# PKU-EPIC/HOTrack

Measured on AMD Instinct MI355X. Metric: HandTrackNet point-cloud frames/sec (N=1024), higher is better.
Workload: dtype f32; 1 GPU; HandTrackNet forward, batch=64 synthetic 1024-pt clouds per GPU (BASELINE configs[1]); per_gpu_batch=64, global_batch=64, npoints=1024, parallelism=dp1 (independent batches, no collective), world_size=1, resident_batches_rotated=5, dead_attention_elided=True, fused_sa_kernels=True, launch=hipGraph replay, batches_in_flight=4, hip_hw_queues=4, sa_compute_units=256, weights=deterministic random init (no checkpoint available offline)

## Files before the change

hotrack_amd/csrc/capi.hip:

```cpp
#include <stdlib.h>

#include "pn2_common.h"
#include "../../include/pn2_ext.h"

namespace pn2 {
static thread_local int g_last_hip_error = 0;
void set_last_hip_error(int e) { g_last_hip_error = e; }

int fps_dispatch(int b, int n, int m, const float *xyz, float *temp, int *idx, hipStream_t st, int force_threads,
                 const int *skip_flags, int nflags, float *radii);
int fps_tie_check(int b, int n, int m, int m1, const float *xyz, const int *idx, const float *radii, int *flags, hipStream_t st);
bool fps_knn_supported(int n, int nq, int k);
bool ball_tie_supported(long b, long n, long m, long m2);
int ball_tie_dispatch(int b, int n, int m, float radius, int nsample, const float *xyz, int *idx, const int *picks, float *new_xyz_out,
                      float *new_xyz_copy, int copy_ld, int m2, const float *radii, int *flags, hipStream_t st, int *counts);
bool three_nn_interp_supported(long b, long n, long m, long c, long ldp, long ldo);
int three_nn_interp_dispatch(int b, int n, int m, int c, const float *unknown, const float *known, const float *points, int ldp,
                             float *out, int ldo, hipStream_t st);
bool three_nn_interp_rows_supported(long b, long n, long m, long c, long ldp, long ldo);
int three_nn_interp_rows_dispatch(int b, int n, int m, int c, const float *unknown, const float *known, const float *points, int ldp,
                                  float *out, int ldo, const int *row_list, const int *row_counts, hipStream_t st);
int fps_knn_dispatch(int b, int n, int m, const float *xyz, int *idx, float *radii, int nq, int k, int k2, const float *query,
                     int *kidx, int *kidx2, hipStream_t st);
int ball_query_dispatch(int b, int n, int m, float radius, int nsample, const float *new_xyz, const float *xyz,
                        int *idx, hipStream_t st, const int *picks, float *new_xyz_out, float *new_xyz_copy, int copy_ld, int *counts);
int three_nn_dispatch(int b, int n, int m, const float *unknown, const float *known, float *dist2, int *idx,
                      hipStream_t st, bool weights);
int interp_pm_dispatch(int b, int c, int m, int n, const float *points, int ldp, const int *idx, const float *weight,
                       float *out, int ldo, hipStream_t st);
int knn_dispatch(int b, int n, int m, int k, const float *unknown, const float *known, float *dist2, int *idx,
                 hipStream_t st, int k2, int *idx2);
int group_fwd_dispatch(int b, int c, int n, int npoints, int nsample, const float *points, const int *idx,
                       float *out, hipStream_t st);
int group_bwd_dispatch(int b, int c, int n, int npoints, int nsample, const float *grad_out, const int *idx,
                       float *grad_points, hipStream_t st);
int interp_fwd_dispatch(int b, int c, int m, int n, const float *points, const int *idx, const float *weight,
                        float *out, hipStream_t st);
int interp_bwd_dispatch(int b, int c, int n, int m, const float *grad_out, const int *idx, const float *weight,
                        float *grad_points, hipStream_t st);
}

using namespace pn2;

#define PN2_REQ(cond, code) \
    do {                    \
        if (!(cond)) return (code); \
    } while (0)

static inline bool fits_int(long v) { return v >= 0 && v <= 2147483647L; }

extern "C" {

int pn2_abi_version(void) { return 4; }

int pn2_last_hip_error(void) { return g_last_hip_error; }

const char *pn2_strerror(int code) {
    switch (code) {
        case PN2_OK: return "ok";
        case PN2_EINVAL: return "invalid dimension or parameter";
        case PN2_ENULL: return "required pointer is NULL";
        case PN2_ERANGE: return "size outside the supported range";
        case PN2_ESCRATCH: return "this size needs the scratch buffer (temp) to be provided";
        case PN2_ELAUNCH: return "HIP kernel launch failed";
        default: return "unknown error";
    }
}

int pn2_furthest_point_sampling(int b, int n, int m, const float *xyz, float *temp, int *idx, void *stream) {
    PN2_REQ(b >= 0 && n >= 1 && m >= 0, PN2_EINVAL);
    if (b == 0 || m == 0) return PN2_OK;
    PN2_REQ(xyz && idx, PN2_ENULL);
    PN2_REQ(b <= 65535 * 32768L, PN2_ERANGE);
    PN2_REQ(fits_int((long)n * 3), PN2_ERANGE);
    int force = 0;
    if (const char *e = getenv("PN2_FPS_THREADS")) force = atoi(e);
    return fps_dispatch(b, n, m, xyz, temp, idx, (hipStream_t)stream, force, nullptr, 0, nullptr);
}

int pn2x_furthest_point_sampling_radii(int b, int n, int m, const float *xyz, int *idx, float *radii, void *stream) {
    PN2_REQ(b >= 0 && n >= 1 && m >= 0, PN2_EINVAL);
    if (b == 0 || m == 0) return PN2_OK;
    PN2_REQ(xyz && idx && radii, PN2_ENULL);
    PN2_REQ(fits_int((long)n * 3), PN2_ERANGE);
    return fps_dispatch(b, n, m, xyz, nullptr, idx, (hipStream_t)stream, 0, nullptr, 0, radii);
}

int pn2x_fps_radii_knn_supported(int n, int nq, int k) { return fps_knn_supported(n, nq, k) ? 1 : 0; }

int pn2x_fps_radii_knn(int b, int n, int m, const float *xyz, int *idx, float *radii, int nq, int k, int k2, const float *query,
                       int *knn_idx, int *knn_idx2, void *stream) {
    PN2_REQ(b >= 0 && n >= 1 && m >= 1 && nq >= 1 && k >= 1 && k2 >= 0 && k2 <= k, PN2_EINVAL);
    if (b == 0) return PN2_OK;
    PN2_REQ(xyz && idx && radii && query && knn_idx && (k2 == 0 || knn_idx2), PN2_ENULL);
    PN2_REQ(m <= n && fits_int((long)n * 3) && fits_int((long)b * nq * k), PN2_ERANGE);
    return fps_knn_dispatch(b, n, m, xyz, idx, radii, nq, k, k2, query, knn_idx, k2 ? knn_idx2 : nullptr, (hipStream_t)stream);
}

int pn2x_fps_prefix_ties(int b, int n, int m1, int m2, const float *xyz, const int *idx1, const float *radii, int *flags, void *stream) {
    PN2_REQ(b >= 0 && n >= 1 && m1 >= 1 && m2 >= 1 && m2 <= m1, PN2_EINVAL);
    if (b == 0) return PN2_OK;
    PN2_REQ(xyz && idx1 && radii && flags, PN2_ENULL);
    PN2_REQ(fits_int((long)n * 3) && b <= 65535, PN2_ERANGE);
    return fps_tie_check(b, n, m2, m1, xyz, idx1, radii, flags, (hipStream_t)stream);
}

int pn2x_fps_prefix_flags(int n) { return n < 1 ? PN2_EINVAL : (n + 63) / 64; }

int pn2x_furthest_point_sampling_prefix(int b, int n, int m, const float *xyz, const int *flags, int nflags, int *idx, void *stream) {
    PN2_REQ(b >= 0 && n >= 1 && m >= 0 && m <= n && nflags >= 1, PN2_EINVAL);
    if (b == 0 || m == 0) return PN2_OK;
    PN2_REQ(xyz && idx && flags, PN2_ENULL);
    PN2_REQ(fits_int((long)n * 3), PN2_ERANGE);
    return fps_dispatch(b, n, m, xyz, nullptr, idx, (hipStream_t)stream, 0, flags, nflags, nullptr);
}

int pn2_ball_query(int b, int n, int m, float radius, int nsample, const float *new_xyz, const float *xyz,
                   int *idx, void *stream) {
    PN2_REQ(b >= 0 && n >= 1 && m >= 0 && nsample >= 1, PN2_EINVAL);
    PN2_REQ(radius == radius, PN2_EINVAL);
    if (b == 0 || m == 0) return PN2_OK;
    PN2_REQ(new_xyz && xyz && idx, PN2_ENULL);
    PN2_REQ(b <= 65535, PN2_ERANGE);
    PN2_REQ(fits_int((long)n * 3) && fits_int((long)m * nsample), PN2_ERANGE);
    if (n >= 4096 && (long)m * n >= (1L << 22) && radius > 0.f) {
        const long words = pn2x_ball_query_grid_scratch_words(b, n);
        if (words > 0 && words < (1L << 30)) {
            StreamScratch own;
            int *scratch = own.acquire((size_t)words + 4, (hipStream_t)stream);
            if (scratch) {
                unsigned *aligned = reinterpret_cast<unsigned *>(((uintptr_t)scratch + 15) & ~(uintptr_t)15);
                const int rc = ball_query_grid_dispatch(b, n, m, radius, nsample, new_xyz, xyz, idx, aligned, (size_t)words, (hipStream_t)stream);
                if (rc != PN2_ERANGE) return rc;
            }
        }
    }
    return ball_query_dispatch(b, n, m, radius, nsample, new_xyz, xyz, idx, (hipStream_t)stream, nullptr, nullptr, nullptr, 0, nullptr);
}

int pn2x_ball_query_picks(int b, int n, int m, float radius, int nsample, const float *xyz, const int *picks, float *new_xyz,
                           int *idx, float *new_xyz_copy, int copy_ld, void *stream) {
    return pn2x_ball_query_picks_counts(b, n, m, radius, nsample, xyz, picks, new_xyz, idx, new_xyz_copy, copy_ld, nullptr, stream);
}

int pn2x_ball_query_picks_counts(int b, int n, int m, float radius, int nsample, const float *xyz, const int *picks, float *new_xyz,
                                  int *idx, float *new_xyz_copy, int copy_ld, int *counts, void *stream) {
    PN2_REQ(!new_xyz_copy || copy_ld >= 3, PN2_EINVAL);
    PN2_REQ(b >= 0 && n >= 1 && m >= 0 && nsample >= 1, PN2_EINVAL);
    PN2_REQ(radius == radius, PN2_EINVAL);
    if (b == 0 || m == 0) return PN2_OK;
    PN2_REQ(xyz && picks && new_xyz && idx, PN2_ENULL);
    PN2_REQ(b <= 65535, PN2_ERANGE);
    PN2_REQ(fits_int((long)n * 3) && fits_int((long)m * nsample), PN2_ERANGE);
    return ball_query_dispatch(b, n, m, radius, nsample, nullptr, xyz, idx, (hipStream_t)stream, picks, new_xyz, new_xyz_copy, copy_ld, counts);
}

int pn2x_ball_query_picks_ties_supported(int b, int n, int m, int m2) { return ball_tie_supported(b, n, m, m2) ? 1 : 0; }

int pn2x_ball_query_picks_ties(int b, int n, int m, float radius, int nsample, const float *xyz, const int *picks, float *new_xyz,
                               int *idx, float *new_xyz_copy, int copy_ld, int m2, const float *radii, int *flags, void *stream) {
    return pn2x_ball_query_picks_ties_counts(b, n, m, radius, nsample, xyz, picks, new_xyz, idx, new_xyz_copy, copy_ld, m2, radii, flags,
                                             nullptr, stream);
}

int pn2x_ball_query_picks_ties_counts(int b, int n, int m, float radius, int nsample, const float *xyz, const int *picks, float *new_xyz,
                                      int *idx, float *new_xyz_copy, int copy_ld, int m2, const float *radii, int *flags, int *counts,
                                      void *stream) {
    PN2_REQ(!new_xyz_copy || copy_ld >= 3, PN2_EINVAL);
    PN2_REQ(b >= 0 && n >= 1 && m >= 1 && nsample >= 1 && m2 >= 1 && m2 <= m, PN2_EINVAL);
    PN2_REQ(radius == radius, PN2_EINVAL);
    if (b == 0) return PN2_OK;
    PN2_REQ(xyz && picks && new_xyz && idx && radii && flags, PN2_ENULL);
    PN2_REQ(b <= 65535 && fits_int((long)n * 3) && fits_int((long)m * nsample), PN2_ERANGE);
    return ball_tie_dispatch(b, n, m, radius, nsample, xyz, idx, picks, new_xyz, new_xyz_copy, copy_ld, m2, radii, flags, (hipStream_t)stream, counts);
}

int pn2_group_points(int b, int c, int n, int npoints, int nsample, const float *points, const int *idx,
                     float *out, void *stream) {
    PN2_REQ(b >= 0 && c >= 0 && n >= 1 && npoints >= 0 && nsample >= 0, PN2_EINVAL);
    if (b == 0 || c == 0 || npoints == 0 || nsample == 0) return PN2_OK;
    PN2_REQ(points && idx && out, PN2_ENULL);
    PN2_REQ(b <= 65535 && fits_int((long)npoints * nsample), PN2_ERANGE);
    return group_fwd_dispatch(b, c, n, npoints, nsample, points, idx, out, (hipStream_t)stream);
}

int pn2_group_points_grad(int b, int c, int n, int npoints, int nsample, const float *grad_out, const int *idx,
                          float *grad_points, void *stream) {
    PN2_REQ(b >= 0 && c >= 0 && n >= 1 && npoints >= 0 && nsample >= 0, PN2_EINVAL);
    if (b == 0 || c == 0 || npoints == 0 || nsample == 0) return PN2_OK;
    PN2_REQ(grad_out && idx && grad_points, PN2_ENULL);
    PN2_REQ(b <= 65535 && c <= 65535 * 16 && fits_int((long)npoints * nsample), PN2_ERANGE);
    return group_bwd_dispatch(b, c, n, npoints, nsample, grad_out, idx, grad_points, (hipStream_t)stream);
}

int pn2_gather_points(int b, int c, int n, int npoints, const float *points, const int *idx, float *out,
                      void *stream) {
    return pn2_group_points(b, c, n, npoints, 1, points, idx, out, stream);
}

int pn2_gather_points_grad(int b, int c, int n, int npoints, const float *grad_out, const int *idx,
                           float *grad_points, void *stream) {
    return pn2_group_points_grad(b, c, n, npoints, 1, grad_out, idx, grad_points, stream);
}

int pn2_knn(int b, int n, int m, int k, const float *unknown, const float *known, float *dist2, int *idx,
            void *stream) {
    PN2_REQ(b >= 0 && n >= 0 && m >= 0, PN2_EINVAL);
    PN2_REQ(k >= 1, PN2_EINVAL);
    PN2_REQ(k <= PN2_KNN_MAX_K, PN2_ERANGE);
    if (b == 0 || n == 0) return PN2_OK;
    PN2_REQ(unknown && dist2 && idx && (known || m == 0), PN2_ENULL);
    PN2_REQ(b <= 65535 && fits_int((long)n * k) && fits_int((long)m * 3), PN2_ERANGE);
    return knn_dispatch(b, n, m, k, unknown, known, dist2, idx, (hipStream_t)stream, 0, nullptr);
}

int pn2x_knn_indices(int b, int n, int m, int k, int k2, const float *unknown, const float *known, int *idx, int *idx2, void *stream) {
    PN2_REQ(b >= 0 && n >= 0 && m >= 1 && k >= 1 && k2 >= 0 && k2 <= k, PN2_EINVAL);
    PN2_REQ(k <= PN2_KNN_MAX_K, PN2_ERANGE);
    if (b == 0 || n == 0) return PN2_OK;
    PN2_REQ(unknown && known && idx && (idx2 || k2 == 0), PN2_ENULL);
    PN2_REQ(b <= 65535 && fits_int((long)n * k) && fits_int((long)m * 3), PN2_ERANGE);
    return knn_dispatch(b, n, m, k, unknown, known, nullptr, idx, (hipStream_t)stream, k2, k2 > 0 ? idx2 : nullptr);
}

int pn2_three_nn(int b, int n, int m, const float *unknown, const float *known, float *dist2, int *idx,
                 void *stream) {
    PN2_REQ(b >= 0 && n >= 0 && m >= 0, PN2_EINVAL);
    if (b == 0 || n == 0) return PN2_OK;
    PN2_REQ(unknown && dist2 && idx && (known || m == 0), PN2_ENULL);
    PN2_REQ(b <= 65535 && fits_int((long)n * 3) && fits_int((long)m * 3), PN2_ERANGE);
    return three_nn_dispatch(b, n, m, unknown, known, dist2, idx, (hipStream_t)stream, false);
}

int pn2_three_interpolate(int b, int c, int m, int n, const float *points, const int *idx, const float *weight,
                          float *out, void *stream) {
    PN2_REQ(b >= 0 && c >= 0 && m >= 1 && n >= 0, PN2_EINVAL);
    if (b == 0 || c == 0 || n == 0) return PN2_OK;
    PN2_REQ(points && idx && weight && out, PN2_ENULL);
    PN2_REQ(b <= 65535 && fits_int((long)n * 3), PN2_ERANGE);
    return interp_fwd_dispatch(b, c, m, n, points, idx, weight, out, (hipStream_t)stream);
}

int pn2_three_interpolate_grad(int b, int c, int n, int m, const float *grad_out, const int *idx,
                               const float *weight, float *grad_points, void *stream) {
    PN2_REQ(b >= 0 && c >= 0 && m >= 1 && n >= 0, PN2_EINVAL);
    if (b == 0 || c == 0 || n == 0) return PN2_OK;
    PN2_REQ(grad_out && idx && weight && grad_points, PN2_ENULL);
    PN2_REQ(b <= 65535 && c <= 65535 * 16 && fits_int((long)n * 3), PN2_ERANGE);
    return interp_bwd_dispatch(b, c, n, m, grad_out, idx, weight, grad_points, (hipStream_t)stream);
}

int pn2x_three_nn_weights(int b, int n, int m, const float *unknown, const float *known, float *weight, int *idx,
                          void *stream) {
    PN2_REQ(b >= 0 && n >= 0 && m >= 3, PN2_EINVAL);
    if (b == 0 || n == 0) return PN2_OK;
    PN2_REQ(unknown && known && weight && idx, PN2_ENULL);
    PN2_REQ(b <= 65535 && fits_int((long)n * 3) && fits_int((long)m * 3), PN2_ERANGE);
    return three_nn_dispatch(b, n, m, unknown, known, weight, idx, (hipStream_t)stream, true);
}

int pn2x_three_nn_interpolate_pm_supported(int b, int n, int m, int c, int ldp, int ldo) {
    return three_nn_interp_supported(b, n, m, c, ldp, ldo) ? 1 : 0;
}

int pn2x_three_nn_interpolate_pm(int b, int n, int m, int c, const float *unknown, const float *known, const float *points, int ldp,
                                 float *out, int ldo, void *stream) {
    PN2_REQ(b >= 0 && n >= 0 && m >= 3 && c >= 1 && ldp >= c && ldo >= c, PN2_EINVAL);
    if (b == 0 || n == 0) return PN2_OK;
    PN2_REQ(unknown && known && points && out, PN2_ENULL);
    PN2_REQ(b <= 65535 && fits_int((long)n * 3) && fits_int((long)m * 3), PN2_ERANGE);
    return three_nn_interp_dispatch(b, n, m, c, unknown, known, points, ldp, out, ldo, (hipStream_t)stream);
}

int pn2x_three_nn_interpolate_pm_rows_supported(int b, int n, int m, int c, int ldp, int ldo) {
    return three_nn_interp_rows_supported(b, n, m, c, ldp, ldo) ? 1 : 0;
}

int pn2x_three_nn_interpolate_pm_rows(int b, int n, int m, int c, const float *unknown, const float *known, const float *points,
                                      int ldp, float *out, int ldo, const int *row_list, const int *row_counts, void *stream) {
    PN2_REQ(b >= 0 && n >= 0 && m >= 3 && c >= 1 && ldp >= c && ldo >= c, PN2_EINVAL);
    if (b == 0 || n == 0) return PN2_OK;
    PN2_REQ(unknown && known && points && out && row_list && row_counts, PN2_ENULL);
    PN2_REQ(b <= 65535 && fits_int((long)n * 3) && fits_int((long)m * 3), PN2_ERANGE);
    return three_nn_interp_rows_dispatch(b, n, m, c, unknown, known, points, ldp, out, ldo, row_list, row_counts, (hipStream_t)stream);
}

int pn2x_three_interpolate_pm(int b, int c, int m, int n, const float *points, int ldp, const int *idx,
                              const float *weight, float *out, int ldo, void *stream) {
    PN2_REQ(b >= 0 && c >= 0 && m >= 1 && n >= 0 && ldp >= c && ldo >= c, PN2_EINVAL);
    if (b == 0 || c == 0 || n == 0) return PN2_OK;
    PN2_REQ(points && idx && weight && out, PN2_ENULL);
    PN2_REQ(fits_int((long)n * 3), PN2_ERANGE);
    return interp_pm_dispatch(b, c, m, n, points, ldp, idx, weight, out, ldo, (hipStream_t)stream);
}

}
```

hotrack_amd/csrc/nn_search.hip:

```cpp
#include "pn2_common.h"
#include "knn_wave.h"

namespace pn2 {

constexpr int kNnTile = 2048;

template <int THREADS, bool WEIGHTS>
__global__ void __launch_bounds__(THREADS)
three_nn_kernel(int n, int m, const float *__restrict__ unknown_all, const float *__restrict__ known_all,
                float *__restrict__ dist2_all, int *__restrict__ idx_all) {
    extern __shared__ __attribute__((aligned(16))) float4 sk[];
    const int b = blockIdx.y;
    const float *__restrict__ known = known_all + (size_t)b * m * 3;
    const int q = blockIdx.x * THREADS + threadIdx.x;
    const bool active = q < n;
    const float *__restrict__ u = unknown_all + ((size_t)b * n + (active ? q : 0)) * 3;
    const float ux = u[0], uy = u[1], uz = u[2];

    float b1 = __builtin_inff(), b2 = __builtin_inff(), b3 = __builtin_inff();
    int i1 = 0, i2 = 0, i3 = 0;

    for (int t0 = 0; t0 < m; t0 += kNnTile) {
        const int tn = (m - t0) < kNnTile ? (m - t0) : kNnTile;
        if (t0 > 0) __syncthreads();
        for (int p = threadIdx.x; p < tn; p += THREADS) {
            const float *src = known + (size_t)3 * (t0 + p);
            sk[p] = make_float4(src[0], src[1], src[2], 0.f);
        }
        __syncthreads();
#pragma unroll 4
        for (int p = 0; p < tn; ++p) {
            const float4 kp = sk[p];
            const float d = sqdist(ux, uy, uz, kp.x, kp.y, kp.z);
            const int k = t0 + p;
            const bool lt1 = d < b1, lt2 = d < b2, lt3 = d < b3;
            b3 = lt2 ? b2 : (lt3 ? d : b3);
            i3 = lt2 ? i2 : (lt3 ? k : i3);
            b2 = lt1 ? b1 : (lt2 ? d : b2);
            i2 = lt1 ? i1 : (lt2 ? k : i2);
            b1 = lt1 ? d : b1;
            i1 = lt1 ? k : i1;
        }
    }
    if (active) {
        float *od = dist2_all + ((size_t)b * n + q) * 3;
        int *oi = idx_all + ((size_t)b * n + q) * 3;
        if constexpr (WEIGHTS) {
            const float r1 = 1.0f / (__builtin_sqrtf(b1) + 1e-8f), r2 = 1.0f / (__builtin_sqrtf(b2) + 1e-8f),
                        r3 = 1.0f / (__builtin_sqrtf(b3) + 1e-8f);
            const float norm = (r1 + r2) + r3;
            od[0] = r1 / norm; od[1] = r2 / norm; od[2] = r3 / norm;
        } else {
            od[0] = b1; od[1] = b2; od[2] = b3;
        }
        oi[0] = i1; oi[1] = i2; oi[2] = i3;
    }
}

template <bool WEIGHTS>
__global__ void __launch_bounds__(256)
three_nn_split_kernel(int n, int m, const float *__restrict__ unknown_all, const float *__restrict__ known_all,
                      float *__restrict__ dist2_all, int *__restrict__ idx_all) {
    extern __shared__ __attribute__((aligned(16))) float4 sk[];
    __shared__ float sd[3][3][64];
    __shared__ int si[3][3][64];
    const int b = blockIdx.y;
    const float *__restrict__ known = known_all + (size_t)b * m * 3;
    const int ql = threadIdx.x & 63, c = threadIdx.x >> 6;
    const int q = blockIdx.x * 64 + ql;
    const bool active = q < n;
    const float *__restrict__ u = unknown_all + ((size_t)b * n + (active ? q : 0)) * 3;
    const float ux = u[0], uy = u[1], uz = u[2];
    for (int p = threadIdx.x; p < m; p += 256) {
        const float *src = known + (size_t)3 * p;
        sk[p] = make_float4(src[0], src[1], src[2], 0.f);
    }
    __syncthreads();
    float b1 = __builtin_inff(), b2 = __builtin_inff(), b3 = __builtin_inff();
    int i1 = 0, i2 = 0, i3 = 0;
    auto insert = [&](float d, int k) {
        const bool lt1 = d < b1, lt2 = d < b2, lt3 = d < b3;
        b3 = lt2 ? b2 : (lt3 ? d : b3);
        i3 = lt2 ? i2 : (lt3 ? k : i3);
        b2 = lt1 ? b1 : (lt2 ? d : b2);
        i2 = lt1 ? i1 : (lt2 ? k : i2);
        b1 = lt1 ? d : b1;
        i1 = lt1 ? k : i1;
    };
    const int len = (m + 3) / 4, p0 = c * len, p1 = min(m, p0 + len);
#pragma unroll 4
    for (int p = p0; p < p1; ++p) {
        const float4 kp = sk[p];
        insert(sqdist(ux, uy, uz, kp.x, kp.y, kp.z), p);
    }
    if (c > 0) {
        sd[c - 1][0][ql] = b1; sd[c - 1][1][ql] = b2; sd[c - 1][2][ql] = b3;
        si[c - 1][0][ql] = i1; si[c - 1][1][ql] = i2; si[c - 1][2][ql] = i3;
    }
    __syncthreads();
    if (c != 0 || !active) return;
#pragma unroll
    for (int cc = 0; cc < 3; ++cc)
#pragma unroll
        for (int e = 0; e < 3; ++e) insert(sd[cc][e][ql], si[cc][e][ql]);
    float *od = dist2_all + ((size_t)b * n + q) * 3;
    int *oi = idx_all + ((size_t)b * n + q) * 3;
    if constexpr (WEIGHTS) {
        const float r1 = 1.0f / (__builtin_sqrtf(b1) + 1e-8f), r2 = 1.0f / (__builtin_sqrtf(b2) + 1e-8f),
                    r3 = 1.0f / (__builtin_sqrtf(b3) + 1e-8f);
        const float norm = (r1 + r2) + r3;
        od[0] = r1 / norm; od[1] = r2 / norm; od[2] = r3 / norm;
    } else {
        od[0] = b1; od[1] = b2; od[2] = b3;
    }
    oi[0] = i1; oi[1] = i2; oi[2] = i3;
}

template <bool ROWS>
__global__ void __launch_bounds__(256)
three_nn_interp_kernel(int n, int m, int c4, const float *__restrict__ unknown_all, const float *__restrict__ known_all,
                       const float *__restrict__ points_all, int ldp, float *__restrict__ out_all, int ldo,
                       const int *__restrict__ row_list, const int *__restrict__ row_counts) {
    extern __shared__ __attribute__((aligned(16))) float4 sk[];
    __shared__ float sd[3][3][64];
    __shared__ int si[3][3][64];
    __shared__ float fw[3][64];
    __shared__ int fi[3][64];
    __shared__ int fq[ROWS ? 64 : 1];
    const int b = blockIdx.y;
    const float *__restrict__ known = known_all + (size_t)b * m * 3;
    const int ql = threadIdx.x & 63, c = threadIdx.x >> 6;
    int q = blockIdx.x * 64 + ql, nq = n;
    if constexpr (ROWS) {
        nq = row_counts[2 * b + 1];
        nq = nq < 0 ? 0 : (nq > n ? n : nq);
        if ((int)blockIdx.x * 64 >= nq) return;
        q = q < nq ? row_list[(size_t)b * n + q] : -1;
        if ((unsigned)q >= (unsigned)n) q = -1;
    }
    const bool active = ROWS ? q >= 0 : q < n;
    const float *__restrict__ u = unknown_all + ((size_t)b * n + (active ? q : 0)) * 3;
    const float ux = u[0], uy = u[1], uz = u[2];
    for (int p = threadIdx.x; p < m; p += 256) {
        const float *src = known + (size_t)3 * p;
        sk[p] = make_float4(src[0], src[1], src[2], 0.f);
    }
    __syncthreads();
    float b1 = __builtin_inff(), b2 = __builtin_inff(), b3 = __builtin_inff();
    int i1 = 0, i2 = 0, i3 = 0;
    auto insert = [&](float d, int k) {
        const bool lt1 = d < b1, lt2 = d < b2, lt3 = d < b3;
        b3 = lt2 ? b2 : (lt3 ? d : b3);
        i3 = lt2 ? i2 : (lt3 ? k : i3);
        b2 = lt1 ? b1 : (lt2 ? d : b2);
        i2 = lt1 ? i1 : (lt2 ? k : i2);
        b1 = lt1 ? d : b1;
        i1 = lt1 ? k : i1;
    };
    const int len = (m + 3) / 4, p0 = c * len, p1 = min(m, p0 + len);
#pragma unroll 4
    for (int p = p0; p < p1; ++p) {
        const float4 kp = sk[p];
        insert(sqdist(ux, uy, uz, kp.x, kp.y, kp.z), p);
    }
    if (c > 0) {
        sd[c - 1][0][ql] = b1; sd[c - 1][1][ql] = b2; sd[c - 1][2][ql] = b3;
        si[c - 1][0][ql] = i1; si[c - 1][1][ql] = i2; si[c - 1][2][ql] = i3;
    }
    __syncthreads();
    if (c == 0) {
#pragma unroll
        for (int cc = 0; cc < 3; ++cc)
#pragma unroll
            for (int e = 0; e < 3; ++e) insert(sd[cc][e][ql], si[cc][e][ql]);
        const float r1 = 1.0f / (__builtin_sqrtf(b1) + 1e-8f), r2 = 1.0f / (__builtin_sqrtf(b2) + 1e-8f),
                    r3 = 1.0f / (__builtin_sqrtf(b3) + 1e-8f);
        const float norm = (r1 + r2) + r3;
        fw[0][ql] = r1 / norm; fw[1][ql] = r2 / norm; fw[2][ql] = r3 / norm;
        fi[0][ql] = i1; fi[1][ql] = i2; fi[2][ql] = i3;
        if constexpr (ROWS) fq[ql] = q;
    }
    __syncthreads();
    const int rows = min(64, nq - (int)blockIdx.x * 64);
    const float *__restrict__ src = points_all + (size_t)b * m * ldp;
    float *__restrict__ dst = out_all + ((size_t)b * n + (ROWS ? (size_t)0 : (size_t)blockIdx.x * 64)) * ldo;
    for (int e = threadIdx.x; e < rows * c4; e += 256) {
        const int r = e / c4, col = e - r * c4;
        const float w0 = fw[0][r], w1 = fw[1][r], w2 = fw[2][r];
        const float4 a0 = *reinterpret_cast<const float4 *>(src + (size_t)fi[0][r] * ldp + 4 * col);
        const float4 a1 = *reinterpret_cast<const float4 *>(src + (size_t)fi[1][r] * ldp + 4 * col);
        const float4 a2 = *reinterpret_cast<const float4 *>(src + (size_t)fi[2][r] * ldp + 4 * col);
        float4 o;
        o.x = __builtin_fmaf(w2, a2.x, __builtin_fmaf(w0, a0.x, w1 * a1.x));
        o.y = __builtin_fmaf(w2, a2.y, __builtin_fmaf(w0, a0.y, w1 * a1.y));
        o.z = __builtin_fmaf(w2, a2.z, __builtin_fmaf(w0, a0.z, w1 * a1.z));
        o.w = __builtin_fmaf(w2, a2.w, __builtin_fmaf(w0, a0.w, w1 * a1.w));
        if constexpr (ROWS) {
            if (fq[r] >= 0) *reinterpret_cast<float4 *>(dst + (size_t)fq[r] * ldo + 4 * col) = o;
        } else {
            *reinterpret_cast<float4 *>(dst + (size_t)r * ldo + 4 * col) = o;
        }
    }
}

bool three_nn_interp_supported(long b, long n, long m, long c, long ldp, long ldo) {
    return b * n >= 16384 && b * n < 256L * 1024 && m >= 16 && m <= kNnTile && c >= 4 && c % 4 == 0 && ldp % 4 == 0 && ldo % 4 == 0;
}

int three_nn_interp_dispatch(int b, int n, int m, int c, const float *unknown, const float *known, const float *points, int ldp,
                             float *out, int ldo, hipStream_t st) {
    if (b == 0 || n == 0) return PN2_OK;
    if (!three_nn_interp_supported(b, n, m, c, ldp, ldo) || (((uintptr_t)points | (uintptr_t)out) % 16) != 0) return PN2_ERANGE;
    dim3 grid((n + 63) / 64, b);
    hipLaunchKernelGGL(three_nn_interp_kernel<false>, grid, dim3(256), (size_t)m * sizeof(float4), st, n, m, c / 4, unknown, known, points,
                       ldp, out, ldo, nullptr, nullptr);
    return check_launch();
}

bool three_nn_interp_rows_supported(long b, long n, long m, long c, long ldp, long ldo) {
    return b <= 65535 && m >= 3 && m <= kNnTile && c >= 4 && c % 4 == 0 && ldp % 4 == 0 && ldo % 4 == 0;
}

int three_nn_interp_rows_dispatch(int b, int n, int m, int c, const float *unknown, const float *known, const float *points, int ldp,
                                  float *out, int ldo, const int *row_list, const int *row_counts, hipStream_t st) {
    if (b == 0 || n == 0) return PN2_OK;
    if (!three_nn_interp_rows_supported(b, n, m, c, ldp, ldo) || (((uintptr_t)points | (uintptr_t)out) % 16) != 0) return PN2_ERANGE;
    dim3 grid((n + 63) / 64, b);
    hipLaunchKernelGGL(three_nn_interp_kernel<true>, grid, dim3(256), (size_t)m * sizeof(float4), st, n, m, c / 4, unknown, known, points,
                       ldp, out, ldo, row_list, row_counts);
    return check_launch();
}

int three_nn_dispatch(int b, int n, int m, const float *unknown, const float *known, float *dist2,
                      int *idx, hipStream_t st, bool weights) {
    if (b == 0 || n == 0) return PN2_OK;
    if ((long)b * n < 256L * 1024 && m >= 16 && m <= kNnTile) {
        dim3 grid((n + 63) / 64, b);
        const size_t lds_split = (size_t)m * sizeof(float4);
        if (weights) hipLaunchKernelGGL((three_nn_split_kernel<true>), grid, dim3(256), lds_split, st, n, m, unknown, known, dist2, idx);
        else hipLaunchKernelGGL((three_nn_split_kernel<false>), grid, dim3(256), lds_split, st, n, m, unknown, known, dist2, idx);
        return check_launch();
    }
    const int tile_cap = m < kNnTile ? m : kNnTile;
    const size_t lds = (size_t)(tile_cap > 0 ? tile_cap : 1) * sizeof(float4);
    if ((long)b * n < 256L * 1024) {
        dim3 grid((n + 63) / 64, b);
        if (weights) hipLaunchKernelGGL((three_nn_kernel<64, true>), grid, dim3(64), lds, st, n, m, unknown, known, dist2, idx);
        else hipLaunchKernelGGL((three_nn_kernel<64, false>), grid, dim3(64), lds, st, n, m, unknown, known, dist2, idx);
    } else {
        dim3 grid((n + 255) / 256, b);
        if (weights) hipLaunchKernelGGL((three_nn_kernel<256, true>), grid, dim3(256), lds, st, n, m, unknown, known, dist2, idx);
        else hipLaunchKernelGGL((three_nn_kernel<256, false>), grid, dim3(256), lds, st, n, m, unknown, known, dist2, idx);
    }
    return check_launch();
}

template <int P>
__global__ void __launch_bounds__(256)
knn_wave_kernel(int n, int m, int k, const float *__restrict__ unknown_all, const float *__restrict__ known_all,
                float *__restrict__ dist2_all, int *__restrict__ idx_all, int k2, int *__restrict__ idx2_all) {
    const int q = blockIdx.x * 4 + (threadIdx.x >> 6);
    if (q >= n) return;
    knn_wave_body<P>(blockIdx.y, q, n, m, k, unknown_all, known_all, dist2_all, idx_all, k2, idx2_all);
}

template <int NS>
__global__ void __launch_bounds__(256)
knn_stream_kernel(int n, int m, int k, const float *__restrict__ unknown_all, const float *__restrict__ known_all,
                  float *__restrict__ dist2_all, int *__restrict__ idx_all, int k2, int *__restrict__ idx2_all) {
    __shared__ unsigned long long lists[4][64 * NS];
    const int b = blockIdx.y;
    const int lane = threadIdx.x & 63, wv = threadIdx.x >> 6;
    const int q = blockIdx.x * 4 + wv;
    if (q >= n) return;
    volatile unsigned long long *L = lists[wv];
    const float *__restrict__ known = known_all + (size_t)b * m * 3;
    const float *__restrict__ u = unknown_all + ((size_t)b * n + q) * 3;
    const float ux = u[0], uy = u[1], uz = u[2];
#pragma unroll
    for (int s = 0; s < NS; ++s) L[lane + 64 * s] = kInfKey;
    unsigned long long kth = kInfKey;
    for (int base = 0; base < m; base += 64) {
        const int c = base + lane;
        const bool in = c < m;
        const float *src = known + (size_t)3 * (in ? c : 0);
        const float d = sqdist(ux, uy, uz, src[0], src[1], src[2]);
        const unsigned long long key = (in && d < __builtin_inff()) ? (((unsigned long long)(unsigned)f2i(d) << 32) | (unsigned)c) : kInfKey;
        uint64_t pass = __ballot(key < kth);
        while (pass) {
            const int l = __builtin_ctzll(pass);
            pass &= pass - 1;
            const unsigned long long kb = ((unsigned long long)(unsigned)__builtin_amdgcn_readlane((int)(unsigned)(key >> 32), l) << 32) |
                                          (unsigned)__builtin_amdgcn_readlane((int)(unsigned)key, l);
            if (!(kb < kth)) continue;
            unsigned long long cur[NS], prev[NS];
#pragma unroll
            for (int s = 0; s < NS; ++s) {
                const int e = lane + 64 * s;
                cur[s] = L[e];
                prev[s] = e > 0 ? L[e - 1] : 0ull;
            }
#pragma unroll
            for (int s = 0; s < NS; ++s) L[lane + 64 * s] = cur[s] < kb ? cur[s] : (prev[s] < kb ? kb : prev[s]);
            kth = L[k - 1];
            kth = ((unsigned long long)(unsigned)__builtin_amdgcn_readfirstlane((int)(unsigned)(kth >> 32)) << 32) |
                  (unsigned)__builtin_amdgcn_readfirstlane((int)(unsigned)kth);
        }
    }
    float *__restrict__ od = dist2_all ? dist2_all + ((size_t)b * n + q) * k : nullptr;
    int *__restrict__ oi = idx_all + ((size_t)b * n + q) * k;
    int *__restrict__ oi2 = idx2_all ? idx2_all + ((size_t)b * n + q) * k2 : nullptr;
#pragma unroll
    for (int s = 0; s < NS; ++s) {
        const int e = lane + 64 * s;
        if (e < k) {
            const unsigned long long v = L[e];
            if (od) od[e] = i2f((int)(unsigned)(v >> 32));
            oi[e] = (int)(unsigned)v;
            if (oi2 && e < k2) oi2[e] = (int)(unsigned)v;
        }
    }
}

int knn_dispatch(int b, int n, int m, int k, const float *unknown, const float *known, float *dist2,
                 int *idx, hipStream_t st, int k2, int *idx2) {
    if (b == 0 || n == 0) return PN2_OK;
    dim3 grid((n + 3) / 4, b);
#define PN2_KNN_CASE(PP)                                                                                    \
    if (m <= 64 * PP) {                                                                                     \
        hipLaunchKernelGGL(knn_wave_kernel<PP>, grid, dim3(256), 0, st, n, m, k, unknown, known, dist2, idx, k2, idx2); \
        return check_launch();                                                                              \
    }
    PN2_KNN_CASE(1) PN2_KNN_CASE(2) PN2_KNN_CASE(4) PN2_KNN_CASE(8) PN2_KNN_CASE(16) PN2_KNN_CASE(32)
#undef PN2_KNN_CASE
    if (k <= 64) hipLaunchKernelGGL(knn_stream_kernel<1>, grid, dim3(256), 0, st, n, m, k, unknown, known, dist2, idx, k2, idx2);
    else if (k <= 128) hipLaunchKernelGGL(knn_stream_kernel<2>, grid, dim3(256), 0, st, n, m, k, unknown, known, dist2, idx, k2, idx2);
    else hipLaunchKernelGGL(knn_stream_kernel<4>, grid, dim3(256), 0, st, n, m, k, unknown, known, dist2, idx, k2, idx2);
    static_assert(PN2_KNN_MAX_K <= 256, "knn_stream_kernel<4> holds 256 list entries");
    return check_launch();
}

}
```

hotrack_amd/csrc/row_chain.hip:

```cpp
#include "pn2_common.h"
#include "mfma_rows.h"
#include "../../include/pn2_ext.h"

namespace pn2 {
namespace rchain {

using mrows::f32x4;
using mrows::init_bias;
using mrows::mm;
using mrows::relu_to_lds;

constexpr int CH = 128, CC = 384, CQ = 512;
constexpr int KX = 144;
constexpr int XQ = 33;
constexpr int LDX = 152, LDH = 136, LDC = 392;
constexpr int MAXB = 1024;
constexpr int GROUP_COST_SMALL = 31, GROUP_COST_LARGE = 20;

struct ChainArgs {
    int B, N, ldx, ldo;
    const float *x;
    const int *list, *counts;
    const float *wa, *ba, *wb, *bb, *wc, *bc, *wq;
    float *out;
};

struct Smem {
    int *rows;
    int *p_small;
    int *p_large;
    float *r1;
    float *r2;
};

constexpr size_t lds_bytes(int clouds) {
    return (size_t)64 * (LDX + LDC) * sizeof(float) + (size_t)(64 + 2 * (clouds + 1) + 512) * sizeof(int);
}

__device__ __forceinline__ int lookup(const ChainArgs &A, const Smem &S, int seq, int e) {
    const int *P = seq ? S.p_large : S.p_small;
    int lo = 0, hi = A.B;
    while (hi - lo > 1) {
        const int mid = (lo + hi) >> 1;
        if (P[mid] <= e) lo = mid; else hi = mid;
    }
    const int off = seq ? (S.p_small[lo + 1] - S.p_small[lo]) : 0;
    return lo * A.N + A.list[(size_t)lo * A.N + off + (e - P[lo])];
}

template <int MT>
__device__ void tile(const ChainArgs &A, const Smem &S, int seq, int e0, int cnt) {
    const int tid = (int)threadIdx.x, lane = tid & 63, w = tid >> 6;
    constexpr int R = MT * 16;
    if (tid < R) S.rows[tid] = tid < cnt ? lookup(A, S, seq, e0 + tid) : -1;
    __syncthreads();
    for (int i = tid; i < R * (KX / 4); i += 256) {
        const int r = i / (KX / 4), q = i - r * (KX / 4);
        const int g = S.rows[r];
        f32x4 v = {0.f, 0.f, 0.f, 0.f};
        if (g >= 0 && q < XQ) {
            v = *reinterpret_cast<const f32x4 *>(A.x + (size_t)g * A.ldx + 4 * q);
            if (q == XQ - 1) v.w = 0.f;
        }
        *reinterpret_cast<f32x4 *>(S.r1 + r * LDX + 4 * q) = v;
    }
    __syncthreads();
    {
        f32x4 acc[2][MT];
        init_bias(acc, A.ba, 2 * w, lane);
        mm<2, MT, KX / 16, LDX>(acc, A.wa + (size_t)(2 * w) * (KX / 16) * 256, S.r1, lane);
        relu_to_lds(acc, S.r2, LDH, 2 * w, lane);
    }
    __syncthreads();
    {
        f32x4 acc[2][MT];
        init_bias(acc, A.bb, 2 * w, lane);
        mm<2, MT, CH / 16, LDH>(acc, A.wb + (size_t)(2 * w) * (CH / 16) * 256, S.r2, lane);
        relu_to_lds(acc, S.r1, LDH, 2 * w, lane);
    }
    __syncthreads();
#pragma unroll 1
    for (int p = 0; p < 2; ++p) {
        const int nt0 = (p * 4 + w) * 3;
        f32x4 acc[3][MT];
        init_bias(acc, A.bc, nt0, lane);
        mm<3, MT, CH / 16, LDH>(acc, A.wc + (size_t)nt0 * (CH / 16) * 256, S.r1, lane);
        relu_to_lds(acc, S.r2, LDC, nt0, lane);
    }
    __syncthreads();
    const int np = seq ? 1 : 2;
#pragma unroll 1
    for (int p = 0; p < np; ++p) {
        const int nt0 = (seq ? 16 : 0) + (p * 4 + w) * 4;
        f32x4 acc[4][MT];
#pragma unroll
        for (int nt = 0; nt < 4; ++nt)
#pragma unroll
            for (int mt = 0; mt < MT; ++mt) acc[nt][mt] = (f32x4){0.f, 0.f, 0.f, 0.f};
        mm<4, MT, CC / 16, LDC>(acc, A.wq + (size_t)nt0 * (CC / 16) * 256, S.r2, lane);
#pragma unroll
        for (int mt = 0; mt < MT; ++mt) {
            const int g = S.rows[mt * 16 + (lane & 15)];
            if (g < 0) continue;
            float *o = A.out + (size_t)g * A.ldo + nt0 * 16 + 4 * (lane >> 4);
#pragma unroll
            for (int nt = 0; nt < 4; ++nt) *reinterpret_cast<f32x4 *>(o + nt * 16) = acc[nt][mt];
        }
    }
    __syncthreads();
}

__device__ void run_rows(const ChainArgs &A, const Smem &S, int seq, int e_lo, int e_hi) {
    for (int e0 = e_lo; e0 < e_hi; e0 += 64) {
        const int cnt = e_hi - e0 < 64 ? e_hi - e0 : 64;
        switch ((cnt + 15) >> 4) {
            case 1: tile<1>(A, S, seq, e0, cnt); break;
            case 2: tile<2>(A, S, seq, e0, cnt); break;
            case 3: tile<3>(A, S, seq, e0, cnt); break;
            default: tile<4>(A, S, seq, e0, cnt); break;
        }
    }
}

__global__ __launch_bounds__(256, 1) void row_chain_kernel(ChainArgs A) {
    extern __shared__ __attribute__((aligned(16))) float smem[];
    const int tid = (int)threadIdx.x;
    Smem S;
    S.r1 = smem;
    S.r2 = smem + 64 * LDX;
    S.rows = reinterpret_cast<int *>(S.r2 + 64 * LDC);
    S.p_small = S.rows + 64;
    S.p_large = S.p_small + (A.B + 1);
    int *scan = S.p_large + (A.B + 1);
    int carry_s = 0, carry_l = 0;
    if (tid == 0) { S.p_small[0] = 0; S.p_large[0] = 0; }
    for (int base = 0; base < A.B; base += 256) {
        const int b = base + tid;
        int cs = 0, cl = 0;
        if (b < A.B) {
            cs = A.counts[2 * b];
            cl = A.counts[2 * b + 1] - cs;
        }
        for (int d = 1; d < 256; d <<= 1) {
            scan[tid] = cs; scan[256 + tid] = cl;
            __syncthreads();
            if (tid >= d) { cs += scan[tid - d]; cl += scan[256 + tid - d]; }
            __syncthreads();
        }
        if (b < A.B) { S.p_small[b + 1] = carry_s + cs; S.p_large[b + 1] = carry_l + cl; }
        scan[tid] = cs; scan[256 + tid] = cl;
        __syncthreads();
        carry_s += scan[255]; carry_l += scan[511];
        __syncthreads();
    }
    const int n_small = carry_s, n_large = carry_l;
    const long g_small = (n_small + 15) / 16, g_large = (n_large + 15) / 16;
    const long total = GROUP_COST_SMALL * g_small + GROUP_COST_LARGE * g_large;
    const long lo = total * blockIdx.x / gridDim.x, hi = total * (blockIdx.x + 1) / gridDim.x;
    auto first_at = [](long c, long cost) { return c <= 0 ? 0L : (c + cost - 1) / cost; };
    long s0 = first_at(lo, GROUP_COST_SMALL), s1 = first_at(hi, GROUP_COST_SMALL);
    s0 = s0 < g_small ? s0 : g_small; s1 = s1 < g_small ? s1 : g_small;
    const long cs_end = GROUP_COST_SMALL * g_small;
    long l0 = first_at(lo - cs_end, GROUP_COST_LARGE), l1 = first_at(hi - cs_end, GROUP_COST_LARGE);
    l0 = l0 < g_large ? l0 : g_large; l1 = l1 < g_large ? l1 : g_large;
    auto clip = [](long e, int n) { return (int)(e < n ? e : n); };
    run_rows(A, S, 0, clip(16 * s0, n_small), clip(16 * s1, n_small));
    run_rows(A, S, 1, clip(16 * l0, n_large), clip(16 * l1, n_large));
}

constexpr int RL_MAXN = 16384;

__global__ __launch_bounds__(256) void row_lists_kernel(int N, int J, int KL, int KS, const int *__restrict__ gi,
                                                        const int *__restrict__ gis, int *__restrict__ list, int *__restrict__ counts) {
    __shared__ unsigned small[RL_MAXN / 32], any[RL_MAXN / 32];
    __shared__ int scan[2][256];
    const int tid = (int)threadIdx.x, b = (int)blockIdx.x;
    const int NW = (N + 31) >> 5;
    for (int i = tid; i < NW; i += 256) { small[i] = 0u; any[i] = 0u; }
    __syncthreads();
    const int *gl = gi + (size_t)b * J * KL;
    for (int i = tid; i < J * KL; i += 256) {
        const int p = gl[i];
        if (gis == nullptr && (i % KL) < KS && (unsigned)p < (unsigned)N) atomicOr(&small[p >> 5], 1u << (p & 31));
        if ((unsigned)p < (unsigned)N) atomicOr(&any[p >> 5], 1u << (p & 31));
    }
    if (gis != nullptr) {
        const int *gs = gis + (size_t)b * J * KS;
        for (int i = tid; i < J * KS; i += 256) {
            const int p = gs[i];
            if ((unsigned)p < (unsigned)N) {
                atomicOr(&small[p >> 5], 1u << (p & 31));
                atomicOr(&any[p >> 5], 1u << (p & 31));
            }
        }
    }
    __syncthreads();
    const int WPT = (NW + 255) >> 8;
    const int w0 = tid * WPT, w1 = w0 + WPT < NW ? w0 + WPT : NW;
    int cs = 0, co = 0;
    for (int i = w0; i < w1; ++i) {
        cs += __builtin_popcount(small[i]);
        co += __builtin_popcount(any[i] & ~small[i]);
    }
    int is = cs, io = co;
    for (int d = 1; d < 256; d <<= 1) {
        scan[0][tid] = is; scan[1][tid] = io;
        __syncthreads();
        if (tid >= d) { is += scan[0][tid - d]; io += scan[1][tid - d]; }
        __syncthreads();
    }
    scan[0][tid] = is; scan[1][tid] = io;
    __syncthreads();
    const int tot_s = scan[0][255], tot_o = scan[1][255];
    int *dst = list + (size_t)b * N;
    int ps = is - cs, po = tot_s + io - co;
    for (int i = w0; i < w1; ++i) {
        unsigned ms = small[i], mo = any[i] & ~small[i];
        while (ms) { const int k = __builtin_ctz(ms); ms &= ms - 1; dst[ps++] = 32 * i + k; }
        while (mo) { const int k = __builtin_ctz(mo); mo &= mo - 1; dst[po++] = 32 * i + k; }
    }
    if (tid == 0) { counts[2 * b] = tot_s; counts[2 * b + 1] = tot_s + tot_o; }
}

}
}

extern "C" int pn2x_row_lists(int b, int n, int j, int k_large, int k_small, const int *gi, const int *gi_small, int *list,
                              int *counts, void *stream) {
    using namespace pn2;
    if (b < 0 || n < 1 || j < 1 || k_large < 1 || k_small < 1 || k_small > k_large) return PN2_EINVAL;
    if (n > rchain::RL_MAXN || (long)j * k_large > (1L << 24)) return PN2_ERANGE;
    if (b == 0) return PN2_OK;
    if (!gi || !list || !counts) return PN2_ENULL;
    hipLaunchKernelGGL(rchain::row_lists_kernel, dim3(b), dim3(256), 0, (hipStream_t)stream, n, j, k_large, k_small, gi, gi_small,
                       list, counts);
    return check_launch();
}

extern "C" int pn2x_row_chain_supported(int c_in, int c_h, int c_conv, int c_q) {
    return (c_in == 128 && c_h == 128 && c_conv == 384 && c_q == 512) ? 1 : 0;
}

extern "C" int pn2x_row_chain(int b, int n, const float *x, int ldx, const int *list, const int *counts, const float *wa,
                              const float *ba, const float *wb, const float *bb, const float *wc, const float *bc, const float *wq,
                              float *out, int ldo, int grid, void *stream) {
    using namespace pn2;
    using namespace pn2::rchain;
    if (b < 0 || n < 1 || ldx < 132 || ldo < CQ || ldx % 4 || ldo % 4 || grid < 0) return PN2_EINVAL;
    if (b > MAXB || (long)b * n >= (1L << 31) / 2) return PN2_ERANGE;
    if (b == 0) return PN2_OK;
    if (!x || !list || !counts || !wa || !ba || !wb || !bb || !wc || !bc || !wq || !out) return PN2_ENULL;
    if (((uintptr_t)x | (uintptr_t)out | (uintptr_t)wa | (uintptr_t)ba | (uintptr_t)wb | (uintptr_t)bb | (uintptr_t)wc |
         (uintptr_t)bc | (uintptr_t)wq) % 16 != 0)
        return PN2_EINVAL;
    ChainArgs a;
    a.B = b; a.N = n; a.ldx = ldx; a.ldo = ldo; a.x = x; a.list = list; a.counts = counts;
    a.wa = wa; a.ba = ba; a.wb = wb; a.bb = bb; a.wc = wc; a.bc = bc; a.wq = wq; a.out = out;
    const size_t lds = lds_bytes(b);
    static_assert(lds_bytes(MAXB) <= 160 * 1024, "row_chain's LDS at MAXB clouds exceeds a compute unit's 160 KB");
    static PerDeviceOnce raised;
    if (raised.first_use())
        (void)hipFuncSetAttribute((const void *)row_chain_kernel, hipFuncAttributeMaxDynamicSharedMemorySize, (int)lds_bytes(MAXB));
    const int cus = num_compute_units();
    if (grid == 0 || grid > cus) grid = cus;
    hipLaunchKernelGGL(row_chain_kernel, dim3(grid), dim3(256), lds, (hipStream_t)stream, a);
    return check_launch();
}
```

hotrack_amd/ext.py:

```python
from __future__ import annotations

import ctypes
import os

import torch

from . import pointnet2_hip as _native

_lib = _native._lib
_vp, _ci = ctypes.c_void_p, ctypes.c_int
_lib.pn2x_kabsch.argtypes = [_ci, _ci, _ci, _vp, _vp, _vp, _vp, _vp]
_lib.pn2x_kabsch.restype = _ci


def kabsch(x: torch.Tensor, y: torch.Tensor):
    x = x.float().contiguous()
    y = y.float().contiguous()
    if x.dim() == 2:
        x = x.unsqueeze(0)
    B, num, _ = y.shape
    xb = x.shape[0]
    if xb not in (1, B) or x.shape[1] != num:
        raise ValueError(f"kabsch: x {tuple(x.shape)} does not match y {tuple(y.shape)}")
    px = _native._ptr(x, "x", torch.float32, xb * num * 3)
    py = _native._ptr(y, "y", torch.float32, B * num * 3)
    R = torch.empty((B, 3, 3), dtype=torch.float32, device=y.device)
    t = torch.empty((B, 3, 1), dtype=torch.float32, device=y.device)
    with torch.cuda.device(y.device):
        _native._check(_lib.pn2x_kabsch(B, xb, num, px, py, R.data_ptr(), t.data_ptr(), _native._stream(y)), "kabsch")
    return R, t


_lib.pn2x_kabsch_backward.argtypes = [_ci, _ci, _ci, _vp, _vp, _vp, _vp, _vp, _vp, _vp]
_lib.pn2x_kabsch_backward.restype = _ci


def kabsch_backward(x: torch.Tensor, y: torch.Tensor, R: torch.Tensor, grad_R, grad_t) -> torch.Tensor:
    x = x.float().contiguous()
    y = y.float().contiguous()
    if x.dim() == 2:
        x = x.unsqueeze(0)
    B, num, _ = y.shape
    f32 = torch.float32
    gR = None if grad_R is None else _native._ptr(grad_R.contiguous(), "grad_R", f32, B * 9)
    gt = None if grad_t is None else _native._ptr(grad_t.contiguous(), "grad_t", f32, B * 3)
    dy = torch.empty_like(y)
    with torch.cuda.device(y.device):
        _native._check(_lib.pn2x_kabsch_backward(B, x.shape[0], num, _native._ptr(x, "x", f32, x.shape[0] * num * 3),
                                                 _native._ptr(y, "y", f32, B * num * 3), _native._ptr(R.contiguous(), "R", f32, B * 9),
                                                 gR, gt, dy.data_ptr(), _native._stream(y)), "kabsch_backward")
    return dy


class KabschFit(torch.autograd.Function):

    @staticmethod
    def forward(ctx, x, y):
        R, t = kabsch(x, y)
        ctx.save_for_backward(x, y, R)
        return R, t

    @staticmethod
    def backward(ctx, grad_R, grad_t):
        x, y, R = ctx.saved_tensors
        return None, kabsch_backward(x, y, R, grad_R, grad_t)


_cl = ctypes.c_long
_lib.pn2x_sa_mlp_max.argtypes = [_ci] * 7 + [_vp, _ci, _vp, _vp, _vp, _vp, _vp, _ci, _vp, _vp, _vp, _vp, _vp, _vp, _cl, _ci, _ci, _vp]
_lib.pn2x_sa_mlp_max.restype = _ci
_lib.pn2x_sa_mlp_max_supported.argtypes = [_ci] * 4
_lib.pn2x_sa_mlp_max_supported.restype = _ci
_lib.pn2x_three_nn_weights.argtypes = [_ci, _ci, _ci, _vp, _vp, _vp, _vp, _vp]
_lib.pn2x_three_nn_weights.restype = _ci
_lib.pn2x_three_interpolate_pm.argtypes = [_ci, _ci, _ci, _ci, _vp, _ci, _vp, _vp, _vp, _ci, _vp]
_lib.pn2x_three_interpolate_pm.restype = _ci
_lib.pn2x_gather_rows.argtypes = [_ci, _ci, _ci, _ci, _vp, _vp, _vp, _vp]
_lib.pn2x_gather_rows.restype = _ci
_lib.pn2x_bias_act_pm.argtypes = [_cl, _ci, _vp, _ci, _vp, _cl, _ci, _vp]
_lib.pn2x_bias_act_pm.restype = _ci


def sa_mlp_max_supported(k: int, c1: int, c2: int, c3: int) -> bool:
    return bool(_lib.pn2x_sa_mlp_max_supported(k, c1, c2, c3))


def _rows(t: torch.Tensor, name: str, cols: int):
    if not t.is_cuda or t.dtype != torch.float32 or t.dim() != 3:
        raise TypeError(f"{name}: expected a 3-D float32 GPU tensor")
    B, R, C = t.shape
    if C < cols or t.stride(2) != 1 or (R > 1 and B > 1 and t.stride(0) != R * t.stride(1)):
        raise ValueError(f"{name}: unsupported layout shape={tuple(t.shape)} strides={t.stride()}")
    return t.data_ptr(), t.stride(1)


def sa_mlp_max(idx: torch.Tensor, w2, b2, w3, b3, *, a1f=None, xyz=None, cxyz=None, wx=None, b1=None, cadd=None,
               out=None, point_major=False) -> torch.Tensor:
    return _sa_mlp_max(idx, w2, b2, w3, b3, None, a1f, xyz, cxyz, wx, b1, cadd, out, point_major)


_lib.pn2x_sa_mlp_max_classes.argtypes = [_ci] * 7 + [_vp, _ci, _vp, _vp, _vp, _vp, _vp, _ci, _vp, _vp, _vp, _vp, _vp, _vp, _vp, _vp, _cl, _ci, _ci, _vp]
_lib.pn2x_sa_mlp_max_classes.restype = _ci
_lib.pn2x_sa_mlp_max_classes_supported.argtypes = [_ci] * 4
_lib.pn2x_sa_mlp_max_classes_supported.restype = _ci
_lib.pn2x_sa_class_lists.argtypes = [_ci, _ci, _ci, _vp, _vp, _vp, _vp]
_lib.pn2x_sa_class_lists.restype = _ci
_lib.pn2x_sa_class_lists2.argtypes = [_ci, _ci, _ci, _vp, _vp, _vp] * 2 + [_vp]
_lib.pn2x_sa_class_lists2.restype = _ci


def sa_mlp_max_classes_supported(k: int, c1: int, c2: int, c3: int) -> bool:
    return bool(_lib.pn2x_sa_mlp_max_classes_supported(k, c1, c2, c3))


def sa_class_partition(counts: torch.Tensor):
    c = counts.reshape(-1)
    ids = torch.arange(c.numel(), dtype=torch.int32, device=c.device)
    masks = (c > 16, (c > 8) & (c <= 16), c <= 8)
    return torch.cat([ids[m] for m in masks]), torch.stack([m.sum() for m in masks]).to(torch.int32)


def _class_lists_args(counts, n, what):
    if not isinstance(counts, torch.Tensor) or counts.dim() != 2 or counts.dtype != torch.int32 or not counts.is_cuda:
        raise TypeError(f"{what}: counts must be a (B,S) int32 GPU tensor")
    if int(n) < 1:
        raise ValueError(f"{what}: n >= 1")
    B, S = counts.shape
    pc = _native._ptr(counts, "counts", torch.int32, B * S)
    lst = torch.empty((B * S, 4), dtype=torch.int32, device=counts.device)
    sizes = torch.empty(3, dtype=torch.int32, device=counts.device)
    return B, S, int(n), pc, lst, sizes


def sa_class_lists(counts: torch.Tensor, n: int):
    B, S, n, pc, lst, sizes = _class_lists_args(counts, n, "sa_class_lists")
    with torch.cuda.device(counts.device):
        _native._check(_native._call(_lib.pn2x_sa_class_lists, "sa_class_lists2_kernel", None, B, S, n, pc, lst.data_ptr(),
                                     sizes.data_ptr(), _native._stream(counts)), "sa_class_lists")
    return lst, sizes


def sa_class_lists_pair(counts_a: torch.Tensor, n_a: int, counts_b: torch.Tensor, n_b: int):
    a = _class_lists_args(counts_a, n_a, "sa_class_lists_pair")
    b = _class_lists_args(counts_b, n_b, "sa_class_lists_pair")
    if counts_a.device != counts_b.device:
        raise ValueError("sa_class_lists_pair: both problems on one device")
    with torch.cuda.device(counts_a.device):
        _native._check(_native._call(_lib.pn2x_sa_class_lists2, "sa_class_lists2_kernel", None, *a[:4], a[4].data_ptr(), a[5].data_ptr(),
                                     *b[:4], b[4].data_ptr(), b[5].data_ptr(), _native._stream(counts_a)), "sa_class_lists_pair")
    return (a[4], a[5]), (b[4], b[5])


def sa_mlp_max_classes(idx: torch.Tensor, classes, w2, b2, w3, b3, *, a1f=None, xyz=None, cxyz=None, wx=None, b1=None, cadd=None,
                       out=None, point_major=False) -> torch.Tensor:
    if not (isinstance(classes, (tuple, list)) and len(classes) == 2):
        raise TypeError("sa_mlp_max_classes: classes must be the (list, sizes) pair of sa_class_lists")
    return _sa_mlp_max(idx, w2, b2, w3, b3, classes, a1f, xyz, cxyz, wx, b1, cadd, out, point_major)


def _sa_mlp_max(idx, w2, b2, w3, b3, classes, a1f, xyz, cxyz, wx, b1, cadd, out, point_major, record=False):
    B, S, K = idx.shape
    C1, C2, C3 = w2.shape[1], w2.shape[0], w3.shape[0]
    f32 = torch.float32
    N = a1f.shape[1] if a1f is not None else xyz.shape[1]
    pa, lda = (None, 0) if a1f is None else _rows(a1f, "a1f", C1)
    pc, ldc = (None, 0) if cadd is None else _rows(cadd, "cadd", C1)
    px = None if xyz is None else _native._ptr(xyz, "xyz", f32, B * N * 3)
    pcx = None if cxyz is None else _native._ptr(cxyz, "cxyz", f32, B * S * 3)
    pwx = None if wx is None else _native._ptr(wx, "wx", f32, C1 * 3)
    pb1 = None if b1 is None else _native._ptr(b1, "b1", f32, C1)
    pi = _native._ptr(idx, "idx", torch.int32, B * S * K)
    pw2, pb2 = _native._ptr(w2, "w2", f32, C2 * C1), _native._ptr(b2, "b2", f32, C2)
    pw3, pb3 = _native._ptr(w3, "w3", f32, C3 * C2), _native._ptr(b3, "b3", f32, C3)
    if out is None:
        out = torch.empty((B, S, C3) if point_major else (B, C3, S), dtype=f32, device=idx.device)
        ob, os_, oc = (S * C3, C3, 1) if point_major else (C3 * S, 1, S)
        po = out.data_ptr()
    else:
        po, ld = _rows(out, "out", C3)
        ob, os_, oc = out.stride(0), ld, 1
    if record:
        return _SaProblem(N, S, K, pa, lda, px, pcx, pwx, pb1, pc, ldc, pi, pw2, pb2, pw3, pb3, po, ob, os_, oc)
    if classes is not None:
        lst, sizes = classes
        pl = _native._ptr(lst, "classes list", torch.int32, B * S * 4)
        ps = _native._ptr(sizes, "classes sizes", torch.int32, 3)
        if lst.device != idx.device or sizes.device != idx.device:
            raise ValueError("sa_mlp_max_classes: classes on another device than idx")
        with torch.cuda.device(idx.device):
            _native._check(_native._call(_lib.pn2x_sa_mlp_max_classes, "sa_mlp_max_classes_kernel", None, B, N, S, K, C1, C2, C3, pa, lda,
                                         px, pcx, pwx, pb1, pc, ldc, pi, pl, ps, pw2, pb2, pw3, pb3, po, ob, os_, oc,
                                         _native._stream(idx)), "sa_mlp_max_classes")
        return out
    with torch.cuda.device(idx.device):
        _native._check(_native._call(_lib.pn2x_sa_mlp_max, "sa_mlp_max_kernel", None, B, N, S, K, C1, C2, C3, pa, lda, px, pcx,
                                     pwx, pb1, pc, ldc, pi, pw2, pb2, pw3, pb3, po, ob, os_, oc, _native._stream(idx)),
                       "sa_mlp_max")
    return out


class _SaProblem(ctypes.Structure):
    _fields_ = [("n", _ci), ("s", _ci), ("k", _ci), ("a1f", _vp), ("a1f_ld", _ci), ("xyz", _vp), ("cxyz", _vp), ("wx", _vp),
                ("b1", _vp), ("cadd", _vp), ("cadd_ld", _ci), ("idx", _vp), ("w2", _vp), ("b2", _vp), ("w3", _vp), ("b3", _vp),
                ("out", _vp), ("out_b", _cl), ("out_s", _ci), ("out_c", _ci)]


_lib.pn2x_sa_mlp_max_pair.argtypes = [_ci] * 4 + [ctypes.POINTER(_SaProblem)] * 2 + [_vp]
_lib.pn2x_sa_mlp_max_pair.restype = _ci
_lib.pn2x_sa_mlp_max_pair_supported.argtypes = [_ci] * 5
_lib.pn2x_sa_mlp_max_pair_supported.restype = _ci


def sa_mlp_max_pair(p0: dict, p1: dict) -> None:
    keys = ("idx", "w2", "b2", "w3", "b3", "a1f", "xyz", "cxyz", "wx", "b1", "cadd", "out")
    a = [{k: p.get(k) for k in keys} for p in (p0, p1)]
    C1, C2, C3 = a[0]["w2"].shape[1], a[0]["w2"].shape[0], a[0]["w3"].shape[0]
    same = all(tuple(a[1][k].shape) == tuple(a[0][k].shape) for k in ("w2", "w3"))
    modes = [(p["a1f"] is not None, p["xyz"] is not None, p["cadd"] is not None) for p in a]
    if not (same and modes[0] == modes[1] and modes[0][0] and modes[0][1]
            and _lib.pn2x_sa_mlp_max_pair_supported(a[0]["idx"].shape[2], a[1]["idx"].shape[2], C1, C2, C3)):
        for p in a:
            sa_mlp_max(p["idx"], p["w2"], p["b2"], p["w3"], p["b3"], a1f=p["a1f"], xyz=p["xyz"], cxyz=p["cxyz"], wx=p["wx"], b1=p["b1"],
                       cadd=p["cadd"], out=p["out"])
        return
    B = a[0]["idx"].shape[0]
    if a[0]["out"] is None or a[1]["out"] is None:
        raise TypeError("sa_mlp_max_pair: out is required")
    q0, q1 = (_sa_mlp_max(classes=None, point_major=False, record=True, **p) for p in a)
    with torch.cuda.device(a[0]["idx"].device):
        _native._check(_native._call(_lib.pn2x_sa_mlp_max_pair, "sa_mlp_max_pair_kernel", None, B, C1, C2, C3, ctypes.byref(q0),
                                     ctypes.byref(q1), _native._stream(a[0]["idx"])), "sa_mlp_max_pair")


_lib.pn2x_mlp2_rows.argtypes = [_cl] + [_ci] * 3 + [_vp, _ci, _vp, _vp, _vp, _vp, _vp, _vp, _ci, _vp]
_lib.pn2x_mlp2_rows.restype = _ci
_lib.pn2x_mlp2_rows_supported.argtypes = [_ci] * 3
_lib.pn2x_mlp2_rows_supported.restype = _ci


_lib.pn2x_sa_set_compute_units.argtypes = [_ci]
_lib.pn2x_sa_set_compute_units.restype = _ci


def sa_set_compute_units(n: int) -> None:
    _native._check(_lib.pn2x_sa_set_compute_units(int(n)), "sa_set_compute_units")


def mlp2_rows_supported(c1: int, c2: int, c3: int) -> bool:
    return bool(_lib.pn2x_mlp2_rows_supported(c1, c2, c3))


def mlp2_rows(x: torch.Tensor, w2, b2, w3, b3, out: torch.Tensor = None, w2e=None) -> torch.Tensor:
    if x.dim() != 2 or not x.is_cuda or x.dtype != torch.float32 or x.stride(1) != 1:
        raise TypeError("mlp2_rows: x must be a 2-D float32 GPU tensor with a contiguous last dimension")
    R = x.shape[0]
    C1, C2, C3 = w2.shape[1], w2.shape[0], w3.shape[0]
    f32 = torch.float32
    ldx = x.stride(0) if R > 1 else x.shape[1]
    if x.shape[1] < C1 + (3 if w2e is not None else 0) or (w2e is not None and ldx < C1 + 4):
        raise ValueError("mlp2_rows: x has too few columns")
    if out is None:
        out = torch.empty((R, C3), dtype=f32, device=x.device)
    if out.dim() != 2 or out.shape[0] != R or out.shape[1] < C3 or out.stride(1) != 1 or out.dtype != f32 or out.device != x.device:
        raise ValueError("mlp2_rows: out must be (rows, >= c3) float32 on the same device")
    if (R > 1 and out.stride(0) % 4) or out.data_ptr() % 16:
        raise ValueError("mlp2_rows: out needs a row stride that is a multiple of 4 floats and a 16-byte aligned first element")
    with torch.cuda.device(x.device):
        _native._check(_native._call(_lib.pn2x_mlp2_rows, "mlp2_rows_kernel", None, R, C1, C2, C3, x.data_ptr(), ldx,
                                     _native._ptr(w2, "w2", f32, C2 * C1), None if w2e is None else _native._ptr(w2e, "w2e", f32, C2 * 3),
                                     _native._ptr(b2, "b2", f32, C2), _native._ptr(w3, "w3", f32, C3 * C2),
                                     _native._ptr(b3, "b3", f32, C3), out.data_ptr(), out.stride(0) if R > 1 else out.shape[1], _native._stream(x)),
                       "mlp2_rows")
    return out


def three_nn_weights(unknown: torch.Tensor, known: torch.Tensor):
    B, n, _ = unknown.shape
    m = known.shape[1]
    f32 = torch.float32
    w = torch.empty((B, n, 3), dtype=f32, device=unknown.device)
    idx = torch.empty((B, n, 3), dtype=torch.int32, device=unknown.device)
    with torch.cuda.device(unknown.device):
        _native._check(_lib.pn2x_three_nn_weights(B, n, m, _native._ptr(unknown, "unknown", f32, B * n * 3),
                                                  _native._ptr(known, "known", f32, B * m * 3), w.data_ptr(), idx.data_ptr(),
                                                  _native._stream(unknown)), "three_nn_weights")
    return w, idx


def three_interpolate_pm(points: torch.Tensor, idx: torch.Tensor, weight: torch.Tensor, out: torch.Tensor) -> torch.Tensor:
    B, M, C = points.shape
    n = idx.shape[1]
    pp, ldp = _rows(points, "points", C)
    po, ldo = _rows(out, "out", C)
    with torch.cuda.device(points.device):
        _native._check(_lib.pn2x_three_interpolate_pm(B, C, M, n, pp, ldp, _native._ptr(idx, "idx", torch.int32, B * n * 3),
                                                      _native._ptr(weight, "weight", torch.float32, B * n * 3), po, ldo,
                                                      _native._stream(points)), "three_interpolate_pm")
    return out


_lib.pn2x_three_nn_interpolate_pm.argtypes = [_ci, _ci, _ci, _ci, _vp, _vp, _vp, _ci, _vp, _ci, _vp]
_lib.pn2x_three_nn_interpolate_pm.restype = _ci
_lib.pn2x_three_nn_interpolate_pm_supported.argtypes = [_ci] * 6
_lib.pn2x_three_nn_interpolate_pm_supported.restype = _ci
_lib.pn2x_three_nn_interpolate_pm_rows.argtypes = [_ci, _ci, _ci, _ci, _vp, _vp, _vp, _ci, _vp, _ci, _vp, _vp, _vp]
_lib.pn2x_three_nn_interpolate_pm_rows.restype = _ci
_lib.pn2x_three_nn_interpolate_pm_rows_supported.argtypes = [_ci] * 6
_lib.pn2x_three_nn_interpolate_pm_rows_supported.restype = _ci


def three_nn_interpolate_pm(unknown: torch.Tensor, known: torch.Tensor, points: torch.Tensor, out: torch.Tensor, rows=None) -> torch.Tensor:
    if rows is not None:
        if not (isinstance(rows, (tuple, list)) and len(rows) == 2 and all(isinstance(t, torch.Tensor) for t in rows)):
            raise TypeError("three_nn_interpolate_pm: rows must be the (list, counts) pair of row_lists")
        if rows[0].dtype != torch.int32 or rows[1].dtype != torch.int32:
            raise TypeError("three_nn_interpolate_pm: rows must be int32 tensors")
        if tuple(rows[0].shape) != tuple(unknown.shape[:2]) or tuple(rows[1].shape) != (unknown.shape[0], 2):
            raise ValueError("three_nn_interpolate_pm: rows must be list (B,n) and counts (B,2)")
    B, n, _ = unknown.shape
    m, C = known.shape[1], points.shape[2]
    pp, ldp = _rows(points, "points", C)
    po, ldo = _rows(out, "out", C)
    f32 = torch.float32
    if rows is not None:
        if not (_lib.pn2x_three_nn_interpolate_pm_rows_supported(B, n, m, C, ldp, ldo) and pp % 16 == 0 and po % 16 == 0):
            raise ValueError("three_nn_interpolate_pm: rows needs 3 <= m <= 2048 known points, C and the row strides multiples of 4 "
                             "and 16-byte aligned points / out")
        if rows[0].device != points.device or rows[1].device != points.device:
            raise ValueError("three_nn_interpolate_pm: rows on another device than points")
        with torch.cuda.device(points.device):
            _native._check(_native._call(_lib.pn2x_three_nn_interpolate_pm_rows, "three_nn_interp_kernel", None, B, n, m, C,
                                         _native._ptr(unknown, "unknown", f32, B * n * 3), _native._ptr(known, "known", f32, B * m * 3),
                                         pp, ldp, po, ldo, _native._ptr(rows[0], "rows list", torch.int32, B * n),
                                         _native._ptr(rows[1], "rows counts", torch.int32, B * 2), _native._stream(points)),
                           "three_nn_interpolate_pm")
        return out
    if _lib.pn2x_three_nn_interpolate_pm_supported(B, n, m, C, ldp, ldo) and pp % 16 == 0 and po % 16 == 0:
        with torch.cuda.device(points.device):
            _native._check(_native._call(_lib.pn2x_three_nn_interpolate_pm, "three_nn_interp_kernel", None, B, n, m, C,
                                         _native._ptr(unknown, "unknown", f32, B * n * 3), _native._ptr(known, "known", f32, B * m * 3),
                                         pp, ldp, po, ldo, _native._stream(points)), "three_nn_interpolate_pm")
        return out
    w, i3 = three_nn_weights(unknown, known)
    return three_interpolate_pm(points, i3, w, out)


def gather_rows(src: torch.Tensor, idx: torch.Tensor) -> torch.Tensor:
    B, N, C = src.shape
    M = idx.shape[1]
    out = torch.empty((B, M, C), dtype=torch.float32, device=src.device)
    with torch.cuda.device(src.device):
        _native._check(_lib.pn2x_gather_rows(B, N, M, C, _native._ptr(src, "src", torch.float32, B * N * C),
                                             _native._ptr(idx, "idx", torch.int32, B * M), out.data_ptr(),
                                             _native._stream(src)), "gather_rows")
    return out


def bias_act_pm_(y: torch.Tensor, bias: torch.Tensor, rows_per_bias: int, relu: bool = True) -> torch.Tensor:
    B, R, C = y.shape
    py, ldy = _rows(y, "y", C)
    with torch.cuda.device(y.device):
        _native._check(_lib.pn2x_bias_act_pm(B * R, C, py, ldy, _native._ptr(bias.contiguous(), "bias", torch.float32, bias.numel()),
                                             rows_per_bias, 1 if relu else 0, _native._stream(y)), "bias_act_pm")
    return y


_lib.pn2x_bias_act.argtypes = [_ci, _ci, _ci, _vp, _vp, _ci, _vp]
_lib.pn2x_bias_act.restype = _ci


def bias_act_(y: torch.Tensor, bias: torch.Tensor, relu: bool = True) -> torch.Tensor:
    B, C, N = y.shape
    py = _native._ptr(y, "y", torch.float32, B * C * N)
    pb = _native._ptr(bias, "bias", torch.float32, C)
    with torch.cuda.device(y.device):
        _native._check(_lib.pn2x_bias_act(B, C, N, py, pb, 1 if relu else 0, _native._stream(y)), "bias_act")
    return y


_lib.pn2x_max_rows.argtypes = [_ci, _ci, _ci, _vp, _vp, _vp]
_lib.pn2x_max_rows.restype = _ci


def max_rows(x: torch.Tensor) -> torch.Tensor:
    B, R, C = x.shape
    out = torch.empty((B, C), dtype=torch.float32, device=x.device)
    with torch.cuda.device(x.device):
        _native._check(_lib.pn2x_max_rows(B, R, C, _native._ptr(x, "x", torch.float32, B * R * C), out.data_ptr(),
                                          _native._stream(x)), "max_rows")
    return out


_lib.pn2x_hand_frame.argtypes = [_ci] * 5 + [_vp] * 4 + [ctypes.c_float] + [_vp] * 5 + [_ci, _vp, _vp]
_lib.pn2x_hand_frame.restype = _ci


def _xyz_cols(t: torch.Tensor, name: str, B: int, R: int):
    if not t.is_cuda or t.dtype != torch.float32 or tuple(t.shape) != (B, R, 3) or t.stride(2) != 1 or \
            (B > 1 and t.stride(0) != R * t.stride(1)):
        raise ValueError(f"{name}: expected a (B,{R},3) float32 column block with uniform row stride, got {tuple(t.shape)} {t.stride()}")
    return t.data_ptr(), t.stride(1)


def hand_frame(palm_template: torch.Tensor, kp: torch.Tensor, palm_idx: torch.Tensor, points: torch.Tensor, scale: float,
               xyz2_copy: torch.Tensor = None, nonfinite: torch.Tensor = None):
    if palm_template.dim() == 2:
        palm_template = palm_template.unsqueeze(0)
    palm_template, kp, points = palm_template.float().contiguous(), kp.float().contiguous(), points.float().contiguous()
    B, N, _ = points.shape
    J = kp.shape[1]
    xb, num = palm_template.shape[0], palm_template.shape[1]
    f32 = torch.float32
    R = torch.empty((B, 3, 3), dtype=f32, device=points.device)
    t = torch.empty((B, 3, 1), dtype=f32, device=points.device)
    xyz2 = torch.empty((B, N, 3), dtype=f32, device=points.device)
    xyz1 = torch.empty((B, J, 3), dtype=f32, device=points.device)
    pc, ldc = (None, 0) if xyz2_copy is None else _xyz_cols(xyz2_copy, "xyz2_copy", B, N)
    with torch.cuda.device(points.device):
        _native._check(_lib.pn2x_hand_frame(B, xb, num, N, J, _native._ptr(palm_template, "palm_template", f32, xb * num * 3),
                                             _native._ptr(kp, "kp", f32, B * J * 3), _native._ptr(palm_idx, "palm_idx", torch.int32, num),
                                             _native._ptr(points, "points", f32, B * N * 3), float(scale), R.data_ptr(), t.data_ptr(),
                                             xyz2.data_ptr(), xyz1.data_ptr(), pc, ldc,
                                             None if nonfinite is None else _native._ptr(nonfinite, "nonfinite", torch.int32, B),
                                             _native._stream(points)), "hand_frame")
    return R, t, xyz2, xyz1


_cf = ctypes.c_float
_lib.pn2x_add_layernorm.argtypes = [_cl, _ci, _vp, _vp, _vp, _vp, _vp, _cf, _vp, _vp, _cf, _vp, _vp]
_lib.pn2x_add_layernorm.restype = _ci
_lib.pn2x_pose_head.argtypes = [_ci, _ci, _ci, _vp, _vp, _vp, _vp, _vp, _vp, _cf, _vp, _vp, _vp, _vp]
_lib.pn2x_pose_head.restype = _ci


def add_layernorm(x: torch.Tensor, ln1, y: torch.Tensor = None, bias: torch.Tensor = None, ln2=None) -> torch.Tensor:
    rows, C = x.shape
    f32 = torch.float32
    px = _native._ptr(x, "x", f32, rows * C)
    py = None if y is None else _native._ptr(y, "y", f32, rows * C)
    pb = None if bias is None else _native._ptr(bias, "bias", f32, C)
    for ln in (ln1, ln2):
        if ln is not None and (tuple(ln.normalized_shape) != (C,) or ln.weight is None or ln.bias is None):
            raise ValueError("add_layernorm: LayerNorm over the last dimension with affine parameters expected")
    g1, b1 = _native._ptr(ln1.weight, "ln1.weight", f32, C), _native._ptr(ln1.bias, "ln1.bias", f32, C)
    g2 = b2 = None
    eps2 = 0.0
    if ln2 is not None:
        g2, b2, eps2 = _native._ptr(ln2.weight, "ln2.weight", f32, C), _native._ptr(ln2.bias, "ln2.bias", f32, C), ln2.eps
    out = torch.empty_like(x)
    with torch.cuda.device(x.device):
        _native._check(_lib.pn2x_add_layernorm(rows, C, px, py, pb, g1, b1, ln1.eps, g2, b2, eps2, out.data_ptr(), _native._stream(x)),
                       "add_layernorm")
    return out


_lib.pn2x_perm_sum_rows.argtypes = [_ci, _ci, _ci, _ci, _vp, _ci, _vp, _vp, _vp]
_lib.pn2x_perm_sum_rows.restype = _ci
_lib.pn2x_add_layernorm_perm.argtypes = [_ci, _ci, _ci, _ci, _vp, _ci, _vp, _vp, _vp, _vp, _cf, _vp, _vp, _cf, _vp, _vp]
_lib.pn2x_add_layernorm_perm.restype = _ci
_lib.pn2x_add_layernorm_perm_any_slots.argtypes = _lib.pn2x_add_layernorm_perm.argtypes
_lib.pn2x_add_layernorm_perm_any_slots.restype = _ci


def _perm_args(z: torch.Tensor, perm: torch.Tensor, c: int, name: str):
    if not z.is_cuda or z.dtype != torch.float32 or z.dim() != 2 or z.stride(1) != 1:
        raise TypeError(f"{name}: z must be 2-D float32 GPU rows with a contiguous last dimension")
    if perm.is_cuda or perm.dtype != torch.int32 or perm.dim() != 2 or not perm.is_contiguous():
        raise TypeError(f"{name}: perm must be a contiguous (J, re) int32 CPU tensor (the library reads it on the host)")
    J, re = perm.shape
    if z.shape[0] % J or z.shape[1] < re * c:
        raise ValueError(f"{name}: z {tuple(z.shape)} does not hold whole groups of {J} tokens with {re} slots of {c} channels")
    return z.shape[0] // J, J, re, z.stride(0)


def perm_sum_rows(z: torch.Tensor, perm: torch.Tensor, c: int) -> torch.Tensor:
    B, J, re, ldz = _perm_args(z, perm, c, "perm_sum_rows")
    out = torch.empty((B, J, c), dtype=torch.float32, device=z.device)
    with torch.cuda.device(z.device):
        _native._check(_lib.pn2x_perm_sum_rows(B, J, re, c, z.data_ptr(), ldz, perm.data_ptr(), out.data_ptr(), _native._stream(z)),
                       "perm_sum_rows")
    return out


def add_layernorm_perm(z: torch.Tensor, perm: torch.Tensor, ln1, bias: torch.Tensor = None, ln2=None, fixed_slots: bool = True) -> torch.Tensor:
    C = int(ln1.normalized_shape[-1])
    f32 = torch.float32
    for ln in (ln1, ln2):
        if ln is not None and (tuple(ln.normalized_shape) != (C,) or ln.weight is None or ln.bias is None):
            raise ValueError("add_layernorm_perm: LayerNorm over the last dimension with affine parameters expected")
    B, J, re, ldz = _perm_args(z, perm, C, "add_layernorm_perm")
    pb = None if bias is None else _native._ptr(bias, "bias", f32, C)
    g1, b1 = _native._ptr(ln1.weight, "ln1.weight", f32, C), _native._ptr(ln1.bias, "ln1.bias", f32, C)
    g2 = b2 = None
    eps2 = 0.0
    if ln2 is not None:
        g2, b2, eps2 = _native._ptr(ln2.weight, "ln2.weight", f32, C), _native._ptr(ln2.bias, "ln2.bias", f32, C), ln2.eps
    out = torch.empty((B * J, C), dtype=f32, device=z.device)
    with torch.cuda.device(z.device):
        args = (B, J, re, C, z.data_ptr(), ldz, perm.data_ptr(), pb, g1, b1, ln1.eps, g2, b2, eps2, out.data_ptr(), _native._stream(z))
        _native._check(_lib.pn2x_add_layernorm_perm(*args) if fixed_slots else _lib.pn2x_add_layernorm_perm_any_slots(*args),
                       "add_layernorm_perm")
    return out


def pose_head(h: torch.Tensor, w: torch.Tensor, bias: torch.Tensor, xyz1: torch.Tensor, R: torch.Tensor, t: torch.Tensor, scale: float,
              nonfinite: torch.Tensor = None):
    B, J, _ = xyz1.shape
    C = h.shape[1]
    f32 = torch.float32
    ptrs = (_native._ptr(h, "h", f32, B * J * C), _native._ptr(w, "w", f32, 3 * C), _native._ptr(bias, "bias", f32, 3),
            _native._ptr(xyz1, "xyz1", f32, B * J * 3), _native._ptr(R, "R", f32, B * 9), _native._ptr(t, "t", f32, B * 3))
    kp_hand = torch.empty((B, J, 3), dtype=f32, device=h.device)
    kp_cam = torch.empty((B, J, 3), dtype=f32, device=h.device)
    with torch.cuda.device(h.device):
        _native._check(_lib.pn2x_pose_head(B, J, C, *ptrs, float(scale), kp_hand.data_ptr(), kp_cam.data_ptr(),
                                            None if nonfinite is None else _native._ptr(nonfinite, "nonfinite", torch.int32, B),
                                            _native._stream(h)), "pose_head")
    return kp_hand, kp_cam


_lib.pn2x_linear_small.argtypes = [_ci, _ci, _ci, _vp, _ci, _vp, _ci, _vp, _ci, _vp, _ci, _vp]
_lib.pn2x_linear_small.restype = _ci
LINEAR_SMALL_MAX_ROWS = 512
LINEAR_SMALL_MAX_K, LINEAR_SMALL_MAX_N = 384, 512


def linear(x: torch.Tensor, w: torch.Tensor, bias: torch.Tensor = None, relu: bool = False) -> torch.Tensor:
    M, K = x.shape
    N = w.shape[0]
    if (M > LINEAR_SMALL_MAX_ROWS or M < 2 or K > LINEAR_SMALL_MAX_K or N > LINEAR_SMALL_MAX_N or not x.is_cuda or x.dtype != torch.float32 or w.dtype != torch.float32 or x.stride(1) != 1
            or w.stride(1) != 1 or (bias is not None and not bias.is_contiguous()) or torch.is_grad_enabled() and (x.requires_grad or w.requires_grad)):
        if relu and bias is not None:
            return torch._addmm_activation(bias, x, w.t())
        y = torch.nn.functional.linear(x, w, bias)
        return torch.relu_(y) if relu else y
    y = torch.empty((M, N), dtype=torch.float32, device=x.device)
    with torch.cuda.device(x.device):
        _native._check(_lib.pn2x_linear_small(M, K, N, x.data_ptr(), x.stride(0), w.data_ptr(), w.stride(0),
                                              None if bias is None else bias.data_ptr(), 1 if relu else 0, y.data_ptr(), N,
                                              _native._stream(x)), "linear_small")
    return y


_lib.pn2x_ln_linear_small.argtypes = [_ci, _ci, _ci, _vp, _vp, _vp, _vp, _vp, _cf, _vp, _vp, _cf, _vp, _vp, _ci, _vp, _ci, _vp, _ci, _vp]
_lib.pn2x_ln_linear_small.restype = _ci
LN_LINEAR_MAX_ROWS = 256


def ln_linear_supported(rows: int, c: int) -> bool:
    return 0 < rows <= LN_LINEAR_MAX_ROWS and c <= 384


def ln_linear(x: torch.Tensor, ln1, w: torch.Tensor, bias: torch.Tensor = None, relu: bool = False, y: torch.Tensor = None,
              ybias: torch.Tensor = None, ln2=None):
    rows, C = x.shape
    N = w.shape[0]
    f32 = torch.float32
    for ln in (ln1, ln2):
        if ln is not None and (tuple(ln.normalized_shape) != (C,) or ln.weight is None or ln.bias is None):
            raise ValueError("ln_linear: LayerNorm over the last dimension with affine parameters expected")
    if x.dtype != f32 or not x.is_cuda or not x.is_contiguous() or w.dtype != f32 or w.stride(1) != 1 or w.shape[1] != C:
        raise TypeError("ln_linear: contiguous float32 GPU rows and a (N, C) float32 weight expected")
    if y is not None and (y.shape != x.shape or not y.is_contiguous() or y.dtype != f32):
        raise TypeError("ln_linear: y must match x")
    xn = torch.empty_like(x)
    out = torch.empty((rows, N), dtype=f32, device=x.device)
    with torch.cuda.device(x.device):
        _native._check(_lib.pn2x_ln_linear_small(
            rows, C, N, x.data_ptr(), None if y is None else y.data_ptr(), None if ybias is None else _native._ptr(ybias, "ybias", f32, C),
            _native._ptr(ln1.weight, "ln1.weight", f32, C), _native._ptr(ln1.bias, "ln1.bias", f32, C), ln1.eps,
            None if ln2 is None else _native._ptr(ln2.weight, "ln2.weight", f32, C), None if ln2 is None else _native._ptr(ln2.bias, "ln2.bias", f32, C),
            0.0 if ln2 is None else ln2.eps, xn.data_ptr(), w.data_ptr(), w.stride(0), None if bias is None else _native._ptr(bias, "bias", f32, N),
            1 if relu else 0, out.data_ptr(), N, _native._stream(x)), "ln_linear_small")
    return xn, out


_lib.pn2x_knn_indices.argtypes = [_ci, _ci, _ci, _ci, _ci, _vp, _vp, _vp, _vp, _vp]
_lib.pn2x_knn_indices.restype = _ci


def knn_indices(k: int, unknown: torch.Tensor, known: torch.Tensor, k2: int = 0):
    B, n, _ = unknown.shape
    m = known.shape[1]
    pu, pk = _native._ptr(unknown, "unknown", torch.float32, B * n * 3), _native._ptr(known, "known", torch.float32, B * m * 3)
    idx = torch.empty((B, n, k), dtype=torch.int32, device=unknown.device)
    idx2 = torch.empty((B, n, k2), dtype=torch.int32, device=unknown.device) if k2 else None
    with torch.cuda.device(unknown.device):
        _native._check(_lib.pn2x_knn_indices(B, n, m, k, k2, pu, pk, idx.data_ptr(), None if idx2 is None else idx2.data_ptr(),
                                             _native._stream(unknown)), "knn_indices")
    return (idx, idx2) if k2 else idx


_lib.pn2x_furthest_point_sampling_radii.argtypes = [_ci, _ci, _ci, _vp, _vp, _vp, _vp]
_lib.pn2x_furthest_point_sampling_radii.restype = _ci
_lib.pn2x_fps_radii_knn.argtypes = [_ci, _ci, _ci, _vp, _vp, _vp, _ci, _ci, _ci, _vp, _vp, _vp, _vp]
_lib.pn2x_fps_radii_knn.restype = _ci
_lib.pn2x_fps_radii_knn_supported.argtypes = [_ci, _ci, _ci]
_lib.pn2x_fps_radii_knn_supported.restype = _ci
_lib.pn2x_fps_prefix_ties.argtypes = [_ci, _ci, _ci, _ci, _vp, _vp, _vp, _vp, _vp]
_lib.pn2x_fps_prefix_ties.restype = _ci
_lib.pn2x_fps_prefix_flags.argtypes = [_ci]
_lib.pn2x_fps_prefix_flags.restype = _ci
_lib.pn2x_furthest_point_sampling_prefix.argtypes = [_ci, _ci, _ci, _vp, _vp, _ci, _vp, _vp]
_lib.pn2x_furthest_point_sampling_prefix.restype = _ci


_lib.pn2x_ball_query_picks.argtypes = [_ci, _ci, _ci, ctypes.c_float, _ci, _vp, _vp, _vp, _vp, _vp, _ci, _vp]
_lib.pn2x_ball_query_picks.restype = _ci
_lib.pn2x_ball_query_picks_counts.argtypes = [_ci, _ci, _ci, ctypes.c_float, _ci, _vp, _vp, _vp, _vp, _vp, _ci, _vp, _vp]
_lib.pn2x_ball_query_picks_counts.restype = _ci


def ball_query_picks(radius: float, nsample: int, xyz: torch.Tensor, picks: torch.Tensor, xyz_copy: torch.Tensor = None,
                     counts: bool = False):
    B, N, _ = xyz.shape
    S = picks.shape[1]
    px = _native._ptr(xyz, "xyz", torch.float32, B * N * 3)
    pp = _native._ptr(picks, "picks", torch.int32, B * S)
    idx = torch.empty((B, S, nsample), dtype=torch.int32, device=xyz.device)
    new_xyz = torch.empty((B, S, 3), dtype=torch.float32, device=xyz.device)
    pc, ldc = (None, 0) if xyz_copy is None else _xyz_cols(xyz_copy, "xyz_copy", B, S)
    with torch.cuda.device(xyz.device):
        if counts:
            cnt = torch.empty((B, S), dtype=torch.int32, device=xyz.device)
            _native._check(_lib.pn2x_ball_query_picks_counts(B, N, S, float(radius), nsample, px, pp, new_xyz.data_ptr(), idx.data_ptr(),
                                                              pc, ldc, cnt.data_ptr(), _native._stream(xyz)), "ball_query_picks")
            return idx, new_xyz, cnt
        _native._check(_lib.pn2x_ball_query_picks(B, N, S, float(radius), nsample, px, pp, new_xyz.data_ptr(), idx.data_ptr(),
                                                   pc, ldc, _native._stream(xyz)), "ball_query_picks")
    return idx, new_xyz


FPS_KNN_COLAUNCH = True
BALL_TIE_COLAUNCH = True
_lib.pn2x_ball_query_picks_ties.argtypes = [_ci, _ci, _ci, ctypes.c_float, _ci, _vp, _vp, _vp, _vp, _vp, _ci, _ci, _vp, _vp, _vp]
_lib.pn2x_ball_query_picks_ties.restype = _ci
_lib.pn2x_ball_query_picks_ties_counts.argtypes = [_ci, _ci, _ci, ctypes.c_float, _ci, _vp, _vp, _vp, _vp, _vp, _ci, _ci, _vp, _vp, _vp, _vp]
_lib.pn2x_ball_query_picks_ties_counts.restype = _ci
_lib.pn2x_ball_query_picks_ties_supported.argtypes = [_ci] * 4
_lib.pn2x_ball_query_picks_ties_supported.restype = _ci


def fps_two_level(xyz: torch.Tensor, m1: int, m2: int, query=None, knn=None, query_counts: bool = False):
    from . import pointnet2_utils as ops
    B, N, _ = xyz.shape
    if not 1 <= m2 <= m1:
        raise ValueError("fps_two_level: need 1 <= m2 <= m1")
    xyz = xyz.contiguous()

    def knn_alone():
        r = knn_indices(knn[1], knn[0], xyz, k2=knn[2])
        return r if knn[2] else (r, None)
    if m2 > 1024 or N > 16384:
        i1 = ops.furthest_point_sample(xyz, m1)
        l1 = gather_rows(xyz, i1)
        i2 = ops.furthest_point_sample(l1, m2)
        if query is not None and query_counts:
            raise ValueError("fps_two_level: query_counts needs m2 <= 1024 and N <= 16384")
        res = (i1, l1, i2) if query is None else (i1, l1, i2, ops.ball_query(query[0], query[1], xyz, l1))
        return res if knn is None else res + (knn_alone(),)
    px = _native._ptr(xyz, "xyz", torch.float32, B * N * 3)
    nf = _lib.pn2x_fps_prefix_flags(N)
    i1 = torch.empty((B, m1), dtype=torch.int32, device=xyz.device)
    radii = torch.empty((B, m1), dtype=torch.float32, device=xyz.device)
    flags = torch.empty((B, nf), dtype=torch.int32, device=xyz.device)
    i2 = torch.empty((B, m2), dtype=torch.int32, device=xyz.device)
    if query_counts and query is None:
        raise ValueError("fps_two_level: query_counts without query")
    cnt1 = torch.empty((B, m1), dtype=torch.int32, device=xyz.device) if query_counts else None
    with torch.cuda.device(xyz.device):
        st = _native._stream(xyz)
        lists = None
        if knn is not None and FPS_KNN_COLAUNCH and _lib.pn2x_fps_radii_knn_supported(N, knn[0].shape[1], knn[1]):
            pts, k, k2 = knn
            nq = pts.shape[1]
            gi = torch.empty((B, nq, k), dtype=torch.int32, device=xyz.device)
            gi2 = torch.empty((B, nq, k2), dtype=torch.int32, device=xyz.device) if k2 else None
            _native._check(_native._call(_lib.pn2x_fps_radii_knn, "fps_knn_kernel", None, B, N, m1, px, i1.data_ptr(), radii.data_ptr(),
                                         nq, k, k2, _native._ptr(pts, "knn points", torch.float32, B * nq * 3), gi.data_ptr(),
                                         None if gi2 is None else gi2.data_ptr(), st), "fps_two_level/1+knn")
            lists = (gi, gi2)
        else:
            _native._check(_native._call(_lib.pn2x_furthest_point_sampling_radii, "fps_kernel", None, B, N, m1, px, i1.data_ptr(),
                                         radii.data_ptr(), st), "fps_two_level/1")
        if query is not None and BALL_TIE_COLAUNCH and _lib.pn2x_ball_query_picks_ties_supported(B, N, m1, m2):
            idx1 = torch.empty((B, m1, query[1]), dtype=torch.int32, device=xyz.device)
            l1 = torch.empty((B, m1, 3), dtype=torch.float32, device=xyz.device)
            if query_counts:
                _native._check(_native._call(_lib.pn2x_ball_query_picks_ties_counts, "ball_tie_kernel", None, B, N, m1, float(query[0]), query[1],
                                             px, i1.data_ptr(), l1.data_ptr(), idx1.data_ptr(), None, 0, m2, radii.data_ptr(),
                                             flags.data_ptr(), cnt1.data_ptr(), st), "fps_two_level/query+ties")
            else:
                _native._check(_native._call(_lib.pn2x_ball_query_picks_ties, "ball_tie_kernel", None, B, N, m1, float(query[0]), query[1], px,
                                             i1.data_ptr(), l1.data_ptr(), idx1.data_ptr(), None, 0, m2, radii.data_ptr(), flags.data_ptr(), st),
                               "fps_two_level/query+ties")
        else:
            if query is None:
                l1 = gather_rows(xyz, i1)
            elif query_counts:
                idx1, l1, cnt1 = ball_query_picks(query[0], query[1], xyz, i1, counts=True)
            else:
                idx1, l1 = ball_query_picks(query[0], query[1], xyz, i1)
            _native._check(_lib.pn2x_fps_prefix_ties(B, N, m1, m2, px, i1.data_ptr(), radii.data_ptr(), flags.data_ptr(), st), "fps_two_level/ties")
        _native._check(_native._call(_lib.pn2x_furthest_point_sampling_prefix, "fps_prefix_kernel", None, B, m1, m2, l1.data_ptr(),
                                     flags.data_ptr(), nf, i2.data_ptr(), st), "fps_two_level/2")
    res = (i1, l1, i2) if query is None else (i1, l1, i2, idx1)
    if query_counts:
        res = res + (cnt1,)
    if knn is None:
        return res
    return res + (lists if lists is not None else knn_alone(),)


_lib.pn2x_hand_losses.argtypes = [_ci, _ci, _vp, _vp, _vp, _vp, _vp, _vp, ctypes.c_float, _vp, _vp, _vp, _vp, _vp]
_lib.pn2x_hand_losses.restype = _ci
_lib.pn2x_hand_losses_backward.argtypes = [_ci, _ci, _vp, ctypes.c_float, _vp, _vp, _vp, _vp, _vp, _vp, _vp]
_lib.pn2x_hand_losses_backward.restype = _ci
HAND_LOSS_NAMES = ("hand_pred_kp_loss", "hand_pred_r_loss", "hand_pred_t_loss", "hand_pred_kp_diff", "hand_init_kp_diff",
                   "hand_init_r_diff", "hand_init_t_diff", "hand_pred_r_diff", "hand_pred_t_diff")


class HandLosses(torch.autograd.Function):

    @staticmethod
    def forward(ctx, pred_hf, init_hf, gt_kp, pred_kp, R, t, scale, palm, weights=None):
        f32 = torch.float32
        B = pred_hf.shape[0]
        ctx.set_materialize_grads(False)
        pred_hf = pred_hf.contiguous()
        palm = palm.contiguous().float()
        if palm.dim() == 2:
            palm = palm.unsqueeze(0)
        args = [x.detach().contiguous().float() for x in (init_hf, gt_kp, pred_kp, R, t)]
        out = torch.empty(10, dtype=f32, device=pred_hf.device)
        saved = torch.empty((B, 87), dtype=f32, device=pred_hf.device)
        wptr = None if weights is None else _native._ptr(weights, "weights", f32, 9)
        with torch.cuda.device(pred_hf.device):
            _native._check(_lib.pn2x_hand_losses(B, palm.shape[0], _native._ptr(pred_hf, "pred_hf", f32, B * 63), _native._ptr(args[0], "init_hf", f32, B * 63),
                                                  _native._ptr(args[1], "gt_kp", f32, B * 63), _native._ptr(args[2], "pred_kp", f32, B * 63),
                                                  _native._ptr(args[3], "R", f32, B * 9), _native._ptr(args[4], "t", f32, B * 3), float(scale),
                                                  _native._ptr(palm, "palm", f32, palm.shape[0] * 18), out.data_ptr(), saved.data_ptr(), wptr,
                                                  _native._stream(pred_hf)), "hand_losses")
        ctx.save_for_backward(pred_hf, palm, saved, *([weights] if weights is not None else []))
        ctx.scale = float(scale)
        ctx.set_materialize_grads(False)
        if weights is None:
            return out[:9]
        return out[:9], out[9]

    @staticmethod
    def backward(ctx, grad, grad_total=None):
        pred_hf, palm, saved = ctx.saved_tensors[:3]
        weights = ctx.saved_tensors[3] if len(ctx.saved_tensors) > 3 else None
        B = pred_hf.shape[0]
        if grad is None and grad_total is None:
            return (None,) * 9
        g3 = None if grad is None else grad[:3].contiguous().float()
        gt = None if grad_total is None else grad_total.contiguous().float()
        d = torch.empty_like(pred_hf)
        with torch.cuda.device(pred_hf.device):
            _native._check(_lib.pn2x_hand_losses_backward(B, palm.shape[0], pred_hf.data_ptr(), ctx.scale, palm.data_ptr(), saved.data_ptr(),
                                                           None if g3 is None else g3.data_ptr(), None if gt is None else gt.data_ptr(),
                                                           None if weights is None else weights.data_ptr(), d.data_ptr(),
                                                           _native._stream(pred_hf)), "hand_losses_backward")
        return d, None, None, None, None, None, None, None, None


_lib.pn2x_copy_multi_max.argtypes = []
_lib.pn2x_copy_multi_max.restype = _ci
_lib.pn2x_copy_multi.argtypes = [_ci, ctypes.POINTER(_vp), ctypes.POINTER(_vp), ctypes.POINTER(ctypes.c_long), _vp]
_lib.pn2x_copy_multi.restype = _ci


def copy_multi(dsts, srcs) -> None:
    n = len(dsts)
    if n == 0:
        return
    cap = int(_lib.pn2x_copy_multi_max())
    dev = dsts[0].device
    for d, s_ in zip(dsts, srcs):
        if (not d.is_cuda or d.device != dev or s_.device != dev or d.dtype != s_.dtype or d.shape != s_.shape
                or not d.is_contiguous() or not s_.is_contiguous()):
            raise ValueError("copy_multi: same-shaped contiguous tensors of one dtype on one GPU")
    with torch.cuda.device(dev):
        for i0 in range(0, n, cap):
            k = min(cap, n - i0)
            D, S, Bn = (_vp * k)(), (_vp * k)(), (ctypes.c_long * k)()
            for j in range(k):
                D[j], S[j], Bn[j] = dsts[i0 + j].data_ptr(), srcs[i0 + j].data_ptr(), dsts[i0 + j].numel() * dsts[i0 + j].element_size()
            _native._check(_lib.pn2x_copy_multi(k, D, S, Bn, _native._stream(dsts[0])), "copy_multi")


_lib.pn2x_row_lists.argtypes = [_ci] * 5 + [_vp] * 5
_lib.pn2x_row_lists.restype = _ci
_lib.pn2x_row_chain_supported.argtypes = [_ci] * 4
_lib.pn2x_row_chain_supported.restype = _ci
_lib.pn2x_row_chain.argtypes = [_ci, _ci, _vp, _ci, _vp, _vp] + [_vp] * 7 + [_vp, _ci, _ci, _vp]
_lib.pn2x_row_chain.restype = _ci
ROW_CHAIN_MAX_B = 1024


def row_lists(gi: torch.Tensor, gi_small, n: int):
    if gi.dim() != 3 or gi.dtype != torch.int32 or not gi.is_cuda:
        raise TypeError("row_lists: gi must be a (B,J,K) int32 GPU tensor")
    gi = gi.contiguous()
    B, J, KL = gi.shape
    if gi_small is not None:
        if gi_small.dim() != 3 or gi_small.shape[:2] != (B, J) or gi_small.dtype != torch.int32 or gi_small.device != gi.device:
            raise ValueError("row_lists: gi_small must be (B,J,K2) int32 on gi's device")
        gi_small = gi_small.contiguous()
    KS = gi_small.shape[2] if gi_small is not None else KL
    lst = torch.empty((B, n), dtype=torch.int32, device=gi.device)
    counts = torch.empty((B, 2), dtype=torch.int32, device=gi.device)
    with torch.cuda.device(gi.device):
        _native._check(_native._call(_lib.pn2x_row_lists, "row_lists_kernel", None, B, n, J, KL, KS, gi.data_ptr(),
                                     None if gi_small is None else gi_small.data_ptr(), lst.data_ptr(), counts.data_ptr(),
                                     _native._stream(gi)), "row_lists")
    return lst, counts


def row_chain_supported(c_in: int, c_h: int, c_conv: int, c_q: int) -> bool:
    return bool(_lib.pn2x_row_chain_supported(c_in, c_h, c_conv, c_q))


def row_chain_pack(W: torch.Tensor) -> torch.Tensor:
    n_out, k = W.shape
    kp = (k + 15) // 16 * 16
    Wp = torch.zeros((n_out, kp), dtype=torch.float32, device=W.device)
    Wp[:, :k] = W
    return Wp.view(n_out // 16, 16, kp // 16, 4, 4).permute(0, 2, 3, 1, 4).contiguous()


def row_chain(x: torch.Tensor, lst: torch.Tensor, counts: torch.Tensor, wa, ba, wb, bb, wc, bc, wq, out: torch.Tensor = None,
              grid: int = 0) -> torch.Tensor:
    if x.dim() != 3 or not x.is_cuda or x.dtype != torch.float32 or x.stride(2) != 1 or x.stride(0) != x.shape[1] * x.stride(1):
        raise TypeError("row_chain: x must be a (B,N,C) float32 GPU tensor with contiguous rows")
    B, N, _ = x.shape
    f32 = torch.float32
    if out is None:
        out = torch.empty((B, N, 512), dtype=f32, device=x.device)
    if out.shape[:2] != (B, N) or out.shape[2] < 512 or out.stride(2) != 1 or out.stride(0) != N * out.stride(1) or out.dtype != f32:
        raise ValueError("row_chain: out must be (B,N,>=512) float32 with contiguous rows")
    if lst.shape != (B, N) or counts.shape != (B, 2) or lst.dtype != torch.int32 or counts.dtype != torch.int32:
        raise ValueError("row_chain: list (B,N) / counts (B,2) int32 from row_lists")
    with torch.cuda.device(x.device):
        _native._check(_native._call(_lib.pn2x_row_chain, "row_chain_kernel", None, B, N, x.data_ptr(), x.stride(1), lst.data_ptr(),
                                     counts.data_ptr(), _native._ptr(wa, "wa", f32, 128 * 144), _native._ptr(ba, "ba", f32, 128),
                                     _native._ptr(wb, "wb", f32, 128 * 128), _native._ptr(bb, "bb", f32, 128),
                                     _native._ptr(wc, "wc", f32, 384 * 128), _native._ptr(bc, "bc", f32, 384),
                                     _native._ptr(wq, "wq", f32, 512 * 384), out.data_ptr(), out.stride(1), int(grid),
                                     _native._stream(x)), "row_chain")
    return out


_lib.pn2x_sa3_chain_supported.argtypes = [_ci] * 5
_lib.pn2x_sa3_chain_supported.restype = _ci
_lib.pn2x_sa3_chain.argtypes = [_ci, _ci, _vp, _ci] + [_vp] * 7 + [_vp]
_lib.pn2x_sa3_chain.restype = _ci
_lib.pn2x_fp3_chain_supported.argtypes = [_ci] * 5
_lib.pn2x_fp3_chain_supported.restype = _ci
_lib.pn2x_fp3_chain.argtypes = [_ci, _ci, _vp, _ci] + [_vp] * 6 + [_vp, _ci, _vp]
_lib.pn2x_fp3_chain.restype = _ci
MID_CHAIN_TILE = 32


def sa3_chain_supported(s: int, c_in: int, c1: int, c2: int, c3: int) -> bool:
    return bool(_lib.pn2x_sa3_chain_supported(s, c_in, c1, c2, c3))


def fp3_chain_supported(s: int, c_l2: int, c_l3: int, c1: int, c2: int) -> bool:
    return bool(_lib.pn2x_fp3_chain_supported(s, c_l2, c_l3, c1, c2))


def _chain_rows(x: torch.Tensor, name: str, min_cols: int):
    if x.dim() != 3 or not x.is_cuda or x.dtype != torch.float32 or x.stride(2) != 1 or x.shape[2] < min_cols or \
            x.stride(0) != x.shape[1] * x.stride(1):
        raise TypeError(f"{name}: expected a (B,S,>={min_cols}) float32 GPU tensor with contiguous rows, got {tuple(x.shape)} {x.stride()}")
    return x.shape[0], x.shape[1]


def sa3_chain(x: torch.Tensor, w1, b1, w2, b2, w3, b3, part: torch.Tensor = None) -> torch.Tensor:
    B, S = _chain_rows(x, "sa3_chain", 132)
    T = MID_CHAIN_TILE
    if S % T:
        raise ValueError(f"sa3_chain: S = {S} is not a multiple of {T}")
    f32 = torch.float32
    if part is None:
        part = torch.empty((B, S // T, 512), dtype=f32, device=x.device)
    if tuple(part.shape) != (B, S // T, 512) or not part.is_contiguous() or part.dtype != f32:
        raise ValueError(f"sa3_chain: part must be a contiguous (B, S/{T}, 512) float32 tensor")
    with torch.cuda.device(x.device):
        _native._check(_native._call(_lib.pn2x_sa3_chain, "sa3_chain_kernel", None, B, S, x.data_ptr(), x.stride(1),
                                     _native._ptr(w1, "w1", f32, 128 * 144), _native._ptr(b1, "b1", f32, 128),
                                     _native._ptr(w2, "w2", f32, 128 * 128), _native._ptr(b2, "b2", f32, 128),
                                     _native._ptr(w3, "w3", f32, 512 * 128), _native._ptr(b3, "b3", f32, 512), part.data_ptr(),
                                     _native._stream(x)), "sa3_chain")
    return part


def fp3_chain(x: torch.Tensor, part: torch.Tensor, wgt, bg, wa, wf, bf, out: torch.Tensor = None) -> torch.Tensor:
    B, S = _chain_rows(x, "fp3_chain", 128)
    T = MID_CHAIN_TILE
    if S % T:
        raise ValueError(f"fp3_chain: S = {S} is not a multiple of {T}")
    f32 = torch.float32
    if out is None:
        out = torch.empty((B, S, 256), dtype=f32, device=x.device)
    _chain_rows(out, "fp3_chain: out", 256)
    if out.shape[:2] != (B, S):
        raise ValueError("fp3_chain: out must be (B,S,>=256)")
    if tuple(part.shape) != (B, S // T, 512) or not part.is_contiguous() or part.dtype != f32:
        raise ValueError(f"fp3_chain: part must be a contiguous (B, S/{T}, 512) float32 tensor")
    if tuple(wgt.shape) != (512, 256):
        raise ValueError("fp3_chain: wgt must be Wg^T, (512, 256)")
    with torch.cuda.device(x.device):
        _native._check(_native._call(_lib.pn2x_fp3_chain, "fp3_chain_kernel", None, B, S, x.data_ptr(), x.stride(1), part.data_ptr(),
                                     _native._ptr(wgt, "wgt", f32, 512 * 256), _native._ptr(bg, "bg", f32, 256),
                                     _native._ptr(wa, "wa", f32, 256 * 128), _native._ptr(wf, "wf", f32, 256 * 256),
                                     _native._ptr(bf, "bf", f32, 256), out.data_ptr(), out.stride(1), _native._stream(x)), "fp3_chain")
    return out


_lib.pn2x_hand_shape_opt_supported.argtypes = [_ci] * 3
_lib.pn2x_hand_shape_opt_supported.restype = _ci
_lib.pn2x_hand_shape_opt.argtypes = [_ci] * 4 + [_vp] * 5 + [ctypes.c_double, ctypes.c_double, _vp, _vp, _vp]
_lib.pn2x_hand_shape_opt.restype = _ci


def hand_shape_opt_supported(p: int, d: int, t: int) -> bool:
    return bool(_lib.pn2x_hand_shape_opt_supported(p, d, t))


def hand_shape_opt(k0: torch.Tensor, k: torch.Tensor, pre: torch.Tensor, targets: torch.Tensor, initial_scale: torch.Tensor,
                   scaling_coefficient2: float, beta: float, iterations: int, out: torch.Tensor = None, trace: bool = False):
    P, D = pre.shape
    T = targets.shape[0]
    f32 = torch.float32
    if tuple(k.shape) != (D, 21, 3) or tuple(k0.shape) != (21, 3) or targets.dim() != 2 or targets.shape[1] != 15:
        raise ValueError(f"hand_shape_opt: k0 {tuple(k0.shape)}, k {tuple(k.shape)}, pre {tuple(pre.shape)}, targets "
                         f"{tuple(targets.shape)} do not fit together")
    if not hand_shape_opt_supported(P, D, T):
        raise ValueError(f"hand_shape_opt: P = {P}, D = {D}, T = {T} outside 1..8192, 1..16, 1..1024")
    if out is None:
        out = (torch.empty if iterations > 0 else torch.zeros)(D, dtype=f32, device=pre.device)
    tr = torch.empty((iterations, 3 + D), dtype=f32, device=pre.device) if trace else None
    with torch.cuda.device(pre.device):
        _native._check(_native._call(_lib.pn2x_hand_shape_opt, "hand_shape_kernel", None, P, D, T, int(iterations),
                                     _native._ptr(k0, "k0", f32, 63), _native._ptr(k, "k", f32, D * 63),
                                     _native._ptr(pre, "pre", f32, P * D), _native._ptr(targets, "targets", f32, T * 15),
                                     _native._ptr(initial_scale, "initial_scale", f32, D), float(scaling_coefficient2), float(beta),
                                     _native._ptr(out, "out", f32, D), None if tr is None else tr.data_ptr(),
                                     _native._stream(pre)), "hand_shape_opt")
        if iterations == 0:
            out.zero_()
    return out, tr


_lib.pn2x_iknet_supported.argtypes = [_ci] * 5
_lib.pn2x_iknet_supported.restype = _ci
_lib.pn2x_iknet_work_floats.argtypes = []
_lib.pn2x_iknet_work_floats.restype = _cl
_lib.pn2x_iknet_forward.argtypes = [_ci, _ci] + [_vp] * 14
_lib.pn2x_iknet_forward.restype = _ci
IKNET_MAX_ROWS = 16


def iknet_supported(m: int, k_in: int = 126, hidden: int = 1024, layers: int = 6, n_out: int = 60) -> bool:
    return bool(_lib.pn2x_iknet_supported(m, k_in, hidden, layers, n_out))


def iknet_forward(kp: torch.Tensor, R: torch.Tensor, t: torch.Tensor, w1, b1, wh, bh, wo, bo, camera: bool = False):
    M = kp.shape[0]
    if not iknet_supported(M):
        raise ValueError(f"iknet_forward: {M} rows outside 1..{IKNET_MAX_ROWS}")
    f32 = torch.float32
    dev = kp.device
    work = torch.empty(int(_lib.pn2x_iknet_work_floats()), dtype=f32, device=dev)
    raw = torch.empty((M, 60), dtype=f32, device=dev)
    theta = torch.empty((M, 45), dtype=f32, device=dev)
    kp_hf = torch.empty((M, 3, 21), dtype=f32, device=dev)
    with torch.cuda.device(dev):
        _native._check(_native._call(_lib.pn2x_iknet_forward, "iknet_forward", None, M, 1 if camera else 0,
                                     _native._ptr(kp, "kp", f32, M * 63), _native._ptr(R, "R", f32, M * 9),
                                     _native._ptr(t, "t", f32, M * 3), _native._ptr(w1, "w1", f32, 1024 * 128),
                                     _native._ptr(b1, "b1", f32, 1024), _native._ptr(wh, "wh", f32, 5 * 1024 * 1024),
                                     _native._ptr(bh, "bh", f32, 5 * 1024), _native._ptr(wo, "wo", f32, 60 * 1024),
                                     _native._ptr(bo, "bo", f32, 60), work.data_ptr(), kp_hf.data_ptr(), raw.data_ptr(),
                                     theta.data_ptr(), _native._stream(kp)), "iknet_forward")
    return raw, theta, kp_hf


_cf, _cd = ctypes.c_float, ctypes.c_double
HAND_POSE_STATE_FLOATS = 90
HAND_POSE_TRACE_FLOATS = 19
HAND_POSE_WEIGHTS = ("sil_loss", "penetrate_sum_loss", "vis_regu_loss", "invis_regu_loss", "temporal_smooth", "attraction_loss")
HAND_POSE_MANO_ENTRIES = ("posedirs", "pose_mean", "kp_vertex", "centre_root")


class _HandPoseSetup(ctypes.Structure):
    _WEIGHTS = ("w_sil", "w_pen", "w_vis", "w_invis", "w_temporal", "w_attr")
    _fields_ = ([(n, _vp) for n in ("parents", "pose_block", "skin_pack", "skin_w", "comps", "pre", "posedirs", "pose_mean", "kp_vertex")] +
                [(n, _ci) for n in ("p", "v", "j", "k", "vol_f16", "res", "centre_root", "reserved")] +
                [(n, _cf) for n in ("theta_scale", "voxel_scale") + _WEIGHTS])


class _HandPoseProblem(ctypes.Structure):
    _fields_ = ([(n, _vp) for n in ("state", "work", "rest_joints", "rest_verts", "pred_kp", "last_kp", "vis_mask", "obj_r", "obj_t",
                                    "vol", "mask", "trace")] +
                [("h", _ci), ("w", _ci), ("fx", _cf), ("fy", _cf), ("cx", _cf), ("cy", _cf), ("active", _ci), ("reserved", _ci)])


_HP_SETUP, _HP_PROBLEM = ctypes.POINTER(_HandPoseSetup), ctypes.POINTER(_HandPoseProblem)
_lib.pn2x_hand_pose_opt_supported.argtypes = [_ci] * 6
_lib.pn2x_hand_pose_opt_supported.restype = _ci
_lib.pn2x_hand_pose_opt_work_floats.argtypes = [_ci]
_lib.pn2x_hand_pose_opt_work_floats.restype = _cl
_lib.pn2x_hand_pose_mano_work_floats.argtypes = [_ci, _ci]
_lib.pn2x_hand_pose_mano_work_floats.restype = _cl
_lib.pn2x_hand_pose_opt_batch_work_floats.argtypes = [_ci, _ci]
_lib.pn2x_hand_pose_opt_batch_work_floats.restype = _cl
_lib.pn2x_hand_pose_energy.argtypes = [_HP_SETUP, _HP_PROBLEM, _vp, _vp, _vp, _vp, _vp]
_lib.pn2x_hand_pose_energy.restype = _ci
_lib.pn2x_hand_pose_opt.argtypes = [_HP_SETUP, _HP_PROBLEM, _vp, _ci, _cd, _cd, _vp]
_lib.pn2x_hand_pose_opt.restype = _ci
_lib.pn2x_hand_pose_problems_fill.argtypes = [_vp, _ci, _HP_PROBLEM, _vp]
_lib.pn2x_hand_pose_problems_fill.restype = _ci
_lib.pn2x_hand_pose_opt_batch.argtypes = [_HP_SETUP, _ci, _ci, _vp, _ci, _cd, _cd, _vp]
_lib.pn2x_hand_pose_opt_batch.restype = _ci
_lib.pn2x_hand_pose_mano_batch_work_floats.argtypes = [_ci, _ci, _ci]
_lib.pn2x_hand_pose_mano_batch_work_floats.restype = _cl
_lib.pn2x_hand_pose_mano_opt_batch.argtypes = [_HP_SETUP, _ci, _ci, _vp, _vp, _ci, _cd, _cd, _vp]
_lib.pn2x_hand_pose_mano_opt_batch.restype = _ci


def hand_pose_opt_supported(p: int, v: int, j: int, k: int, d_pose: int = 10, res: int = 151) -> bool:
    return bool(_lib.pn2x_hand_pose_opt_supported(int(p), int(v), int(j), int(k), int(d_pose), int(res)))


def hand_pose_model(tables: dict, device) -> dict:
    f32, i32 = torch.float32, torch.int32
    idx = tables["skin_idx"].long()
    V, K = idx.shape
    pack = torch.zeros(V, dtype=torch.long)
    for k in range(K):
        pack |= idx[:, k] << (5 * k)
    offs = [int(o) for o in tables["finger_offsets"]]
    for f in range(5):
        pack[tables["tips"][offs[f]:offs[f + 1]].long().unique()] |= 1 << (20 + f)
    m = {"V": V, "K": K, "J": int(tables["parents"].numel()),
         "parents": tables["parents"].to(device, i32).contiguous(), "pose_block": tables["pose_block"].to(device, i32).contiguous(),
         "rest_joints": tables["rest_joints"].to(device, f32).contiguous(), "rest_verts": tables["rest_verts"].to(device, f32).contiguous(),
         "skin_pack": pack.to(device, i32).contiguous(), "skin_w": tables["skin_w"].to(device, f32).contiguous(),
         "comps": tables["comps"].to(device, f32).contiguous(), "fingers_ok": all(offs[f + 1] > offs[f] for f in range(5))}
    m["mano"] = any(k in tables for k in HAND_POSE_MANO_ENTRIES)
    if m["mano"]:
        J = m["J"]
        kpv = tables["kp_vertex"].long() if "kp_vertex" in tables else torch.full((J,), -1, dtype=torch.long)
        owners = [(j, int(v)) for j, v in enumerate(kpv) if int(v) >= 0]
        m["mano_ok"] = len({v for _, v in owners}) == len(owners) and all(0 < j < 32 and v < V for j, v in owners)
        if m["mano_ok"]:
            for j, v in owners:
                pack[v] |= j << 25
            m["skin_pack"] = pack.to(device, i32).contiguous()
        rows = (3 * V + 15) // 16 * 16
        pd = torch.zeros(rows, 136, dtype=f32)
        if "posedirs" in tables:
            pd[:3 * V, :135] = tables["posedirs"].to(f32).reshape(3 * V, 135)
        m["posedirs_pack"] = pd.to(device).contiguous()
        m["pose_mean"] = (tables["pose_mean"].to(f32) if "pose_mean" in tables else torch.zeros(45)).to(device).contiguous()
        m["kp_vertex"] = kpv.to(device, i32).contiguous()
        m["centre_root"] = 1 if tables.get("centre_root", False) else 0
    if "shape_joints" in tables:
        D = tables["shape_joints"].shape[0]
        m["shape_joints"] = tables["shape_joints"].to(device, f32).reshape(D, -1).contiguous()
        m["shape_verts"] = tables["shape_verts"].to(device, f32).reshape(D, -1).contiguous()
    return m


def hand_pose_rest(model: dict, beta: torch.Tensor = None):
    if beta is None or "shape_joints" not in model:
        return model["rest_joints"], model["rest_verts"]
    b = beta.to(model["rest_joints"]).reshape(1, -1)
    return ((model["rest_joints"] + (b @ model["shape_joints"]).view(-1, 3)).contiguous(),
            (model["rest_verts"] + (b @ model["shape_verts"]).view(-1, 3)).contiguous())


def _hand_pose_setup(model, pre, theta_scale, volume, voxel_scale, weights, posedirs=None) -> _HandPoseSetup:
    f32, i32 = torch.float32, torch.int32
    mano = bool(model.get("mano", False))
    if mano and not model.get("mano_ok", False):
        raise ValueError("hand_pose_mano: one vertex serves two keypoints (kp_vertex)")
    V, K, J = model["V"], model["K"], model["J"]
    if pre is not None and (pre.dim() != 2 or pre.shape[1] != 16):
        raise ValueError(f"hand_pose: pre {tuple(pre.shape)} is not (P, 16)")
    P = 0 if pre is None else pre.shape[0]
    if volume.dim() != 3 or len(set(volume.shape)) != 1 or volume.dtype not in (torch.float16, f32):
        raise ValueError(f"hand_pose: volume {tuple(volume.shape)} {volume.dtype} is not a cubic fp16 / fp32 volume")
    res = volume.shape[0]
    if not hand_pose_opt_supported(1 if pre is None else P, V, J, K, 10, res):
        raise ValueError(f"hand_pose: P = {P}, V = {V}, J = {J}, K = {K}, res = {res} outside 1..8192, 1..1024, 21, 1..4, odd <= 1024")
    s = _HandPoseSetup(p=P, v=V, j=J, k=K, vol_f16=1 if volume.dtype == torch.float16 else 0, res=res,
                       theta_scale=float(theta_scale), voxel_scale=float(voxel_scale))
    s.parents, s.pose_block = _native._ptr(model["parents"], "parents", i32, J), _native._ptr(model["pose_block"], "pose_block", i32, J)
    s.skin_pack, s.skin_w = _native._ptr(model["skin_pack"], "skin_pack", i32, V), _native._ptr(model["skin_w"], "skin_w", f32, V * K)
    s.comps, s.pre = _native._ptr(model["comps"], "comps", f32, 45 * 45), None if pre is None else _native._ptr(pre, "pre", f32, P * 16)
    for field, key in zip(_HandPoseSetup._WEIGHTS, HAND_POSE_WEIGHTS) if weights is not None else ():
        setattr(s, field, float(weights[key]))
    if mano:
        s.posedirs = _native._ptr(model["posedirs_pack"] if posedirs is None else posedirs, "posedirs", f32, (3 * V + 15) // 16 * 16 * 136)
        s.pose_mean, s.kp_vertex = _native._ptr(model["pose_mean"], "pose_mean", f32, 45), _native._ptr(model["kp_vertex"], "kp_vertex", i32, J)
        s.centre_root = int(model["centre_root"])
    return s


def _hand_pose_frame(model, state, work, trace, rest, pred_kp, last_kp, vis_mask, obj_r, obj_t, volume, mask, proj) -> _HandPoseProblem:
    f32, u8 = torch.float32, torch.uint8
    V, J = model["V"], model["J"]
    if mask.dim() != 2:
        raise ValueError(f"hand_pose: mask {tuple(mask.shape)} is not (h, w)")
    h, w = mask.shape
    rest_j, rest_v = rest
    r = _HandPoseProblem(state=state, work=work, trace=trace, h=h, w=w, fx=float(proj["fx"]), fy=float(proj["fy"]), cx=float(proj["cx"]),
                         cy=float(proj["cy"]), active=1)
    r.rest_joints, r.rest_verts = _native._ptr(rest_j, "rest_joints", f32, J * 3), _native._ptr(rest_v, "rest_verts", f32, V * 3)
    r.pred_kp = _native._ptr(pred_kp, "pred_kp", f32, J * 3)
    r.last_kp = None if last_kp is None else _native._ptr(last_kp, "last_kp", f32, J * 3)
    r.vis_mask, r.obj_r, r.obj_t = _native._ptr(vis_mask, "vis_mask", u8, J), _native._ptr(obj_r, "obj_r", f32, 9), _native._ptr(obj_t, "obj_t", f32, 3)
    r.vol, r.mask = _native._ptr(volume, "volume", volume.dtype, volume.shape[0] ** 3), _native._ptr(mask, "mask", u8, h * w)
    return r


def hand_pose_mano_workspace(p: int, v: int, device) -> torch.Tensor:
    return torch.empty(int(_lib.pn2x_hand_pose_mano_work_floats(int(p), int(v))), dtype=torch.float32, device=device)


def _hand_pose_single(setup, model, offsets, state, trace, rest, pred_kp, last_kp, vis_mask, obj_r, obj_t, volume, mask, proj):
    f32, dev = torch.float32, model["rest_joints"].device
    work = torch.empty(int(_lib.pn2x_hand_pose_opt_work_floats(setup.p)), dtype=f32, device=dev)
    off_ptr = None
    if model.get("mano", False):
        if offsets is None:
            offsets = hand_pose_mano_workspace(setup.p, setup.v, dev)
        off_ptr = _native._ptr(offsets, "offsets", f32, int(_lib.pn2x_hand_pose_mano_work_floats(setup.p, setup.v)))
    frame = _hand_pose_frame(model, _native._ptr(state, "state", f32, HAND_POSE_STATE_FLOATS), work.data_ptr(),
                             None if trace is None else trace.data_ptr(), rest, pred_kp, last_kp, vis_mask, obj_r, obj_t, volume, mask, proj)
    return frame, off_ptr, (work, offsets)


def hand_pose_energy(model, rest, theta_scale, pre, state, pred_kp, last_kp, vis_mask, obj_r, obj_t, volume, voxel_scale, mask, proj,
                     weights, with_geometry: bool = False, *, offsets: torch.Tensor = None, posedirs: torch.Tensor = None):
    setup = _hand_pose_setup(model, pre, theta_scale, volume, voxel_scale, weights, posedirs)
    frame, off_ptr, keep = _hand_pose_single(setup, model, offsets, state, None, rest, pred_kp, last_kp, vis_mask, obj_r, obj_t, volume, mask, proj)
    f32, dev, P = torch.float32, pre.device, setup.p
    energy = torch.empty(P, dtype=f32, device=dev)
    verts = torch.empty((P, model["V"], 3), dtype=f32, device=dev) if with_geometry else None
# ... 393 lines not shown
```

include/pn2_ext.h:

```cpp
#ifndef PN2_EXT_H
#define PN2_EXT_H

#include "pn2_hip.h"

#ifdef __cplusplus
extern "C" {
#endif

int pn2x_kabsch(int b, int xb, int num, const float *x, const float *y, float *R, float *t, void *stream);
int pn2x_kabsch_backward(int b, int xb, int num, const float *x, const float *y, const float *R, const float *grad_R,
                         const float *grad_t, float *grad_y, void *stream);

int pn2x_hand_frame(int b, int xb, int num, int n, int j, const float *palm_template, const float *kp,
                    const int *palm_idx, const float *points, float scale, float *R, float *t, float *xyz2,
                    float *xyz1, float *xyz2_copy, int copy_ld, int *nonfinite, void *stream);

int pn2x_sa_mlp_max(int b, int n, int s, int k, int c1, int c2, int c3, const float *a1f, int a1f_ld,
                    const float *xyz, const float *cxyz, const float *wx, const float *b1, const float *cadd,
                    int cadd_ld, const int *idx,
                    const float *w2, const float *b2, const float *w3, const float *b3, float *out,
                    long out_b, int out_s, int out_c, void *stream);
int pn2x_sa_mlp_max_supported(int k, int c1, int c2, int c3);

int pn2x_sa_class_lists(int b, int s, int n, const int *counts, int *list, int *sizes, void *stream);
int pn2x_sa_class_lists2(int b0, int s0, int n0, const int *counts0, int *list0, int *sizes0, int b1, int s1, int n1,
                         const int *counts1, int *list1, int *sizes1, void *stream);
int pn2x_sa_mlp_max_classes_supported(int k, int c1, int c2, int c3);
int pn2x_sa_mlp_max_classes(int b, int n, int s, int k, int c1, int c2, int c3, const float *a1f, int a1f_ld,
                            const float *xyz, const float *cxyz, const float *wx, const float *b1, const float *cadd,
                            int cadd_ld, const int *idx, const int *cls_list, const int *cls_sizes,
                            const float *w2, const float *b2, const float *w3, const float *b3, float *out,
                            long out_b, int out_s, int out_c, void *stream);

int pn2x_bias_act(int b, int c, int n, float *y, const float *bias, int relu, void *stream);

int pn2x_three_nn_weights(int b, int n, int m, const float *unknown, const float *known, float *weight, int *idx,
                          void *stream);

int pn2x_three_nn_interpolate_pm_supported(int b, int n, int m, int c, int ldp, int ldo);
int pn2x_three_nn_interpolate_pm(int b, int n, int m, int c, const float *unknown, const float *known, const float *points, int ldp,
                                 float *out, int ldo, void *stream);
int pn2x_three_interpolate_pm(int b, int c, int m, int n, const float *points, int ldp, const int *idx,
                              const float *weight, float *out, int ldo, void *stream);
int pn2x_three_nn_interpolate_pm_rows_supported(int b, int n, int m, int c, int ldp, int ldo);
int pn2x_three_nn_interpolate_pm_rows(int b, int n, int m, int c, const float *unknown, const float *known, const float *points,
                                      int ldp, float *out, int ldo, const int *row_list, const int *row_counts, void *stream);

int pn2x_furthest_point_sampling_radii(int b, int n, int m, const float *xyz, int *idx, float *radii, void *stream);
int pn2x_fps_radii_knn_supported(int n, int nq, int k);
int pn2x_fps_radii_knn(int b, int n, int m, const float *xyz, int *idx, float *radii, int nq, int k, int k2, const float *query,
                       int *knn_idx, int *knn_idx2, void *stream);
int pn2x_fps_prefix_ties(int b, int n, int m1, int m2, const float *xyz, const int *idx1, const float *radii, int *flags, void *stream);
int pn2x_ball_query_picks_ties_supported(int b, int n, int m, int m2);
int pn2x_ball_query_picks_ties(int b, int n, int m, float radius, int nsample, const float *xyz, const int *picks, float *new_xyz,
                               int *idx, float *new_xyz_copy, int copy_ld, int m2, const float *radii, int *flags, void *stream);
int pn2x_fps_prefix_flags(int n);
int pn2x_furthest_point_sampling_prefix(int b, int n, int m, const float *xyz, const int *flags, int nflags, int *idx, void *stream);

int pn2x_knn_indices(int b, int n, int m, int k, int k2, const float *unknown, const float *known, int *idx, int *idx2, void *stream);

int pn2x_ball_query_picks(int b, int n, int m, float radius, int nsample, const float *xyz, const int *picks, float *new_xyz,
                          int *idx, float *new_xyz_copy, int copy_ld, void *stream);
int pn2x_ball_query_picks_counts(int b, int n, int m, float radius, int nsample, const float *xyz, const int *picks, float *new_xyz,
                                 int *idx, float *new_xyz_copy, int copy_ld, int *counts, void *stream);
int pn2x_ball_query_picks_ties_counts(int b, int n, int m, float radius, int nsample, const float *xyz, const int *picks, float *new_xyz,
                                      int *idx, float *new_xyz_copy, int copy_ld, int m2, const float *radii, int *flags, int *counts,
                                      void *stream);

long pn2x_ball_query_grid_scratch_words(int b, int n);
int pn2x_ball_query_grid(int b, int n, int m, float radius, int nsample, const float *new_xyz, const float *xyz, int *idx,
                         void *scratch, long scratch_words, void *stream);

int pn2x_gather_rows(int b, int n, int m, int c, const float *src, const int *idx, float *out, void *stream);

int pn2x_bias_act_pm(long rows, int c, float *y, int ldy, const float *bias, long rows_per_bias, int relu, void *stream);

int pn2x_max_rows(int b, int r, int c, const float *x, float *out, void *stream);

int pn2x_copy_multi_max(void);
int pn2x_copy_multi(int n, void *const *dst, const void *const *src, const long *bytes, void *stream);

int pn2x_add_layernorm(long rows, int c, const float *x, const float *y, const float *bias, const float *g1,
                       const float *b1, float eps1, const float *g2, const float *b2, float eps2, float *out, void *stream);

int pn2x_perm_sum_rows(int b, int j, int re, int c, const float *z, int ldz, const int *perm, float *out, void *stream);
int pn2x_add_layernorm_perm(int b, int j, int re, int c, const float *z, int ldz, const int *perm, const float *bias,
                            const float *g1, const float *b1, float eps1, const float *g2, const float *b2, float eps2,
                            float *out, void *stream);
int pn2x_add_layernorm_perm_any_slots(int b, int j, int re, int c, const float *z, int ldz, const int *perm, const float *bias,
                                      const float *g1, const float *b1, float eps1, const float *g2, const float *b2, float eps2,
                                      float *out, void *stream);

int pn2x_pose_head(int b, int j, int c, const float *h, const float *w, const float *bias, const float *xyz1,
                   const float *R, const float *t, float scale, float *kp_hand, float *kp_cam, const int *nonfinite,
                   void *stream);

typedef struct pn2x_sa_problem {
    int n, s, k;
    const float *a1f;
    int a1f_ld;
    const float *xyz, *cxyz, *wx, *b1, *cadd;
    int cadd_ld;
    const int *idx;
    const float *w2, *b2, *w3, *b3;
    float *out;
    long out_b;
    int out_s, out_c;
} pn2x_sa_problem;
int pn2x_sa_set_compute_units(int n);
int pn2x_mlp2_rows_supported(int c1, int c2, int c3);
int pn2x_mlp2_rows(long rows, int c1, int c2, int c3, const float *x, int ldx, const float *w2, const float *w2e, const float *b2,
                   const float *w3, const float *b3, float *out, int ldo, void *stream);
int pn2x_sa_mlp_max_pair_supported(int k0, int k1, int c1, int c2, int c3);
int pn2x_sa_mlp_max_pair(int b, int c1, int c2, int c3, const pn2x_sa_problem *p0, const pn2x_sa_problem *p1, void *stream);

int pn2x_row_lists(int b, int n, int j, int k_large, int k_small, const int *gi, const int *gi_small, int *list, int *counts,
                   void *stream);
int pn2x_row_chain_supported(int c_in, int c_h, int c_conv, int c_q);
int pn2x_row_chain(int b, int n, const float *x, int ldx, const int *list, const int *counts, const float *wa, const float *ba,
                   const float *wb, const float *bb, const float *wc, const float *bc, const float *wq, float *out, int ldo,
                   int grid, void *stream);

int pn2x_sa3_chain_supported(int s, int c_in, int c1, int c2, int c3);
int pn2x_sa3_chain(int b, int s, const float *x, int ldx, const float *w1, const float *b1, const float *w2, const float *b2,
                   const float *w3, const float *b3, float *part, void *stream);
int pn2x_fp3_chain_supported(int s, int c_l2, int c_l3, int c1, int c2);
int pn2x_fp3_chain(int b, int s, const float *x, int ldx, const float *part, const float *wgt, const float *bg, const float *wa,
                   const float *wf, const float *bf, float *out, int ldo, void *stream);

int pn2x_hand_shape_opt_supported(int p, int d, int t);
int pn2x_hand_shape_opt(int p, int d, int t, int iterations, const float *k0, const float *k, const float *pre,
                        const float *targets, const float *initial_scale, double scaling_coefficient2, double beta, float *out,
                        float *trace, void *stream);

typedef struct pn2x_hand_pose_setup {
    const int *parents, *pose_block, *skin_pack;
    const float *skin_w, *comps, *pre, *posedirs, *pose_mean;
    const int *kp_vertex;
    int p, v, j, k, vol_f16, res, centre_root, reserved;
    float theta_scale, voxel_scale, w_sil, w_pen, w_vis, w_invis, w_temporal, w_attr;
} pn2x_hand_pose_setup;
typedef struct pn2x_hand_pose_problem {
    float *state, *work;
    const float *rest_joints, *rest_verts, *pred_kp, *last_kp;
    const unsigned char *vis_mask;
    const float *obj_r, *obj_t;
    const void *vol;
    const unsigned char *mask;
    float *trace;
    int h, w;
    float fx, fy, cx, cy;
    int active, reserved;
} pn2x_hand_pose_problem;
int pn2x_hand_pose_opt_supported(int p, int v, int j, int k, int d_pose, int res);
long pn2x_hand_pose_opt_work_floats(int p);
long pn2x_hand_pose_mano_work_floats(int p, int v);
long pn2x_hand_pose_opt_batch_work_floats(int p, int s);
int pn2x_hand_pose_energy(const pn2x_hand_pose_setup *setup, const pn2x_hand_pose_problem *frame, float *offsets, float *energy,
                          float *out_verts, float *out_kp, void *stream);
int pn2x_hand_pose_opt(const pn2x_hand_pose_setup *setup, const pn2x_hand_pose_problem *frame, float *offsets, int iterations,
                       double scaling_coefficient2, double beta, void *stream);
int pn2x_hand_pose_problems_fill(pn2x_hand_pose_problem *problems, int s, const pn2x_hand_pose_problem *host, void *stream);
int pn2x_hand_pose_opt_batch(const pn2x_hand_pose_setup *setup, int s, int active, const pn2x_hand_pose_problem *problems,
                             int iterations, double scaling_coefficient2, double beta, void *stream);
long pn2x_hand_pose_mano_batch_work_floats(int p, int v, int s);
int pn2x_hand_pose_mano_opt_batch(const pn2x_hand_pose_setup *setup, int s, int active, const pn2x_hand_pose_problem *problems,
                                  float *offsets, int iterations, double scaling_coefficient2, double beta, void *stream);

int pn2x_iknet_supported(int m, int k_in, int hidden, int layers, int n_out);
long pn2x_iknet_work_floats(void);
int pn2x_iknet_forward(int m, int frame, const float *kp, const float *R, const float *t, const float *w1, const float *b1,
                       const float *wh, const float *bh, const float *wo, const float *bo, float *work, float *kp_hf,
                       float *raw_quat, float *theta, void *stream);

int pn2x_bn_sums_doubles(int c);
int pn2x_bn_stats(long rows, int c, const float *y, int ldy, double *sums, void *stream);
int pn2x_bn_relu_apply(long rows, int c, const float *y, int ldy, const double *sums, const float *gamma, const float *beta,
                       const float *conv_bias, float eps, float momentum, float *running_mean, float *running_var,
                       long long *num_batches_tracked, float *save_mean, float *save_invstd, float *h, int ldh, int relu,
                       void *stream);
int pn2x_bn_relu_bwd(long rows, int c, const float *dh, int ldd, const float *y, int ldy, const float *mean,
                     const float *invstd, const float *gamma, const float *beta, int relu, double *sums, float *dy, int ldo,
                     float *dgamma, float *dbeta, float *dbias, void *stream);
int pn2x_sa_layer1(int b, int n, int s, int k, int c1, const float *a1f, int a1f_ld, const float *xyz, const float *cxyz,
                   const float *wx, int wx_ld, const float *cadd, int cadd_ld, const int *idx, float *out, float *rel_out,
                   void *stream);
typedef struct pn2x_sa_layer1_stats_problem {
    const float *a1f, *wx, *cadd;
    const int *idx;
    float *out, *rel_out;
    double *sums;
    int k, c1, a1f_ld, wx_ld, cadd_ld, reserved;
} pn2x_sa_layer1_stats_problem;
int pn2x_sa_layer1_stats(const pn2x_sa_layer1_stats_problem *problems, int count, int b, int n, int s, const float *xyz,
                         const float *cxyz, void *stream);
int pn2x_scatter_add_rows(int b, int n, int m, int c, const float *dout, int ldo, const int *idx, float *din, int ldi,
                          void *stream);
int pn2x_three_interpolate_pm_grad(int b, int c, int m, int n, const float *dout, int ldo, const int *idx,
                                   const float *weight, float *dpoints, int ldp, void *stream);

int pn2x_inverse_index(int b, int n_dst, int l, const int *idx, int *offsets, int *order, void *stream);
typedef struct pn2x_rows_segment_sum_problem {
    const float *dout;
    const int *offsets, *order;
    const float *weight;
    float *din;
    int m_src, t, c, ldo, ldi, reserved;
} pn2x_rows_segment_sum_problem;
int pn2x_rows_segment_sum(const pn2x_rows_segment_sum_problem *problems, int count, int b, int n_dst, int accumulate, void *stream);

long pn2x_scatter_cm_scratch_ints(int t, int b, int n_dst, int m_src);
int pn2x_scatter_cm(int t, int b, int c, int n_dst, int m_src, const float *grad_out, const int *idx, const float *weight,
                    float *grad_points, int *scratch, long scratch_ints, void *stream);

typedef struct pn2x_bn_relu_max_problem {
    const float *y;
    const double *sums;
    const float *gamma, *beta, *conv_bias;
    float *running_mean, *running_var;
    long long *num_batches_tracked;
    float *save_mean, *save_invstd, *out;
    int *arg;
    long groups;
    int k, c, ldy, ldo;
    float eps, momentum;
} pn2x_bn_relu_max_problem;
int pn2x_bn_relu_max(const pn2x_bn_relu_max_problem *problems, int count, void *stream);
int pn2x_bn_relu_max_bwd(long groups, int k, int c, const float *dout, const int *arg, const float *y, int ldy, const float *mean,
                         const float *invstd, const float *gamma, const float *beta, double *sums, float *dy, int ldo, float *dgamma,
                         float *dbeta, float *dbias, void *stream);

int pn2x_bn_bwd_reduce(long rows, int c, const float *dh, int ldd, const int *arg, int k, const float *y, int ldy, const float *mean,
                       const float *invstd, const float *gamma, const float *beta, int relu, double *sums, float *g_out, int ldg,
                       void *stream);
typedef struct pn2x_bn_bwd_reduce_routed_problem {
    const float *dout;
    const int *arg;
    const float *y, *mean, *invstd, *gamma, *beta;
    double *sums;
    long groups;
    int k, c, ldd, lda, ldy, reserved;
} pn2x_bn_bwd_reduce_routed_problem;
int pn2x_bn_bwd_reduce_routed(const pn2x_bn_bwd_reduce_routed_problem *problems, int count, void *stream);
long pn2x_rows_outer3_scratch_floats(long rows, int c);
int pn2x_rows_outer3(long rows, int c, const float *dy, int ldy, const float *rel, float *out, float *scratch, long scratch_floats,
                     void *stream);
int pn2x_bn_bwd_apply(long rows, int c, const float *g, int ldg, const float *y, int ldy, const float *mean, const float *invstd,
                      const float *gamma, const float *beta, int relu, const double *sums, float *dy, int ldo, float *dgamma,
                      float *dbeta, float *dbias, void *stream);

long pn2x_bn_bwd_apply_rel_scratch_floats(long rows, int c);
typedef struct pn2x_bn_bwd_apply_rel_problem {
    const float *g, *y, *mean, *invstd, *gamma, *beta;
    const double *sums;
    float *dy, *dgamma, *dbeta, *dbias;
    const float *rel;
    float *scratch, *dwx;
    long rows, scratch_floats;
    int c, ldg, ldy, relu, ldo, reserved;
} pn2x_bn_bwd_apply_rel_problem;
int pn2x_bn_bwd_apply_rel(const pn2x_bn_bwd_apply_rel_problem *problems, int count, void *stream);

int pn2x_tg_supported(int c_in, int c_out);
int pn2x_tg_fwd(long rows, int k, int n, const float *x, int ldx, const float *w, int ldw, float *y, int ldy, const double *sums_in,
                const float *gamma, const float *beta, const float *conv_bias, float eps, float momentum, float *running_mean,
                float *running_var, long long *num_batches_tracked, float *save_mean, float *save_invstd, double *sums_out,
                void *stream);
int pn2x_tg_dgrad(long rows, int kd, int n, int gmode, const float *g, int ldg, const int *arg, int kmax, const float *yi, int ldyi,
                  const float *mean_i, const float *invstd_i, const float *gamma_i, const float *beta_i, const double *sums_bwd_i,
                  const float *w, int ldw, const float *yp, int ldyp, const float *mean_p, const float *invstd_p,
                  const float *gamma_p, const float *beta_p, float *gp, int ldgp, double *sums_bwd_p, void *stream);
long pn2x_tg_wgrad_partial_floats(long rows, int n, int k);
int pn2x_tg_wgrad(long rows, int n, int k, int gmode, const float *g, int ldg, const int *arg, int kmax, const float *yi, int ldyi,
                  const float *mean_i, const float *invstd_i, const float *gamma_i, const float *beta_i, const double *sums_bwd_i,
                  const float *yp, int ldyp, const float *mean_p, const float *invstd_p, const float *gamma_p, const float *beta_p,
                  float *partial, long partial_floats, float *dw, float *dgamma, float *dbeta, float *dbias, int *n_partials,
                  void *stream);

int pn2x_hand_losses(int b, int pb, const float *pred_hf, const float *init_hf, const float *gt_kp, const float *pred_kp, const float *R,
                     const float *t, float scale, const float *palm, float *out, float *saved, const float *weights, void *stream);
int pn2x_hand_losses_backward(int b, int pb, const float *pred_hf, float scale, const float *palm, const float *saved, const float *grad3,
                              const float *grad_total, const float *weights, float *d_pred_hf, void *stream);

int pn2x_tail_ln_fwd(long rows, int c, const float *x, const float *y, const float *bias, float p, int site, const long long *seed_in,
                     long long *seed_dev, long long *seed_out, const float *ga, const float *ba, float eps_a, const float *gb,
                     const float *bb, float eps_b, float *out, float *stats, void *stream);
int pn2x_tail_ln_bwd(long rows, int c, const float *x, const float *y, const float *bias, float p, int site, const long long *seed_in,
                     const float *ga, const float *ba, float eps_a, const float *gb, const float *bb, float eps_b, const float *stats,
                     const float *dout, float *dx, float *dy, float *dga, float *dba, float *dgb, float *dbb, float *dbias,
                     void *stream);
int pn2x_tail_relu_drop_fwd(long rows, int c, const float *z, const float *bias, float p, int site, const long long *seed_in,
                            float *out, void *stream);
int pn2x_tail_relu_drop_bwd(long rows, int c, const float *z, const float *bias, float p, int site, const long long *seed_in,
                            const float *dh, float *dz, float *dbias, void *stream);
int pn2x_tail_pose_head_fwd(int b, int j, int c, const float *h, const float *w, const float *bias, const float *xyz1, const float *R,
                            const float *t, const float *scale, int scale_stride, float *kp_hand, float *kp_cam, void *stream);
int pn2x_tail_pose_head_bwd(int b, int j, int c, const float *h, const float *w, const float *g_hand, const float *g_cam, const float *R,
                            const float *scale, int scale_stride, float *dh, float *dw, float *dbias, void *stream);

int pn2x_adam_multi(int n, void *const *p, const void *const *g, void *const *m, void *const *v, void *const *step, const long *numel,
                    double lr, double beta1, double beta2, double eps, double weight_decay, int advance, void *stream);
int pn2x_adam_advance(float *steps, int n, void *stream);
int pn2x_tg_reduce_multi(int count, const float *const *partial, const int *n_partials, const int *numel, float *const *dw,
                         const double *const *sums_bwd, const int *channels, const int *sums_ld, float *const *dgamma,
                         float *const *dbeta, float *const *dbias, void *stream);
typedef struct pn2x_tg_fwd2_problem {
    const float *x, *w;
    float *y;
    const double *sums_in;
    const float *gamma, *beta, *conv_bias;
    float *running_mean, *running_var;
    long long *num_batches_tracked;
    float *save_mean, *save_invstd;
    double *sums_out;
    long rows;
    int k, n, ldx, ldw, ldy;
    float eps, momentum;
    int reserved;
} pn2x_tg_fwd2_problem;
int pn2x_tg_fwd2_supported(int c_in, int c_out);
int pn2x_tg_fwd2_pair_supported(int c_in, int c_out);
int pn2x_tg_fwd2(const pn2x_tg_fwd2_problem *problems, int count, void *stream);

typedef struct pn2x_tg_bwd_slice_problem {
    const float *g;
    const int *arg;
    const float *yi, *mean_i, *invstd_i, *gamma_i, *beta_i;
    const double *sums_bwd_i;
    const float *w, *yp, *mean_p, *invstd_p, *gamma_p, *beta_p;
    float *gp;
    double *sums_bwd_p;
    float *partial, *dw;
    const float *g_add;
    long rows, partial_floats;
    int n, k, gmode, ldg, ldarg, kmax, ldyi, sums_ld, ldw, ldyp, ldgp, ldga, raw_out, reserved;
} pn2x_tg_bwd_slice_problem;
int pn2x_tg_bwd_pair_supported(int c_in, int c_out);
int pn2x_tg_bwd_slice(const pn2x_tg_bwd_slice_problem *problems, int count, int *n_partials, void *stream);
int pn2x_tg_bwd_supported(int c_in, int c_out);
int pn2x_tg_bwd_partials(long rows, int c_out, int c_in);
int pn2x_tg_bwd_set_variant(int v2);

int pn2x_wgrad_multi_max(void);
long pn2x_wgrad_multi_scratch_floats(int count, const int *rows, const int *n, const int *k);
int pn2x_wgrad_multi(int count, const float *const *g, const int *ldg, const float *const *x, const int *ldx, const int *rows,
                     const int *n, const int *k, float *const *dw, const int *lddw, float *scratch, long scratch_floats, void *stream);

int pn2x_linear_small(int m, int k, int n, const float *x, int ldx, const float *w, int ldw, const float *bias, int relu, float *y,
                      int ldy, void *stream);

int pn2x_ln_linear_small(int m, int k, int n, const float *xa, const float *ya, const float *ybias, const float *g1, const float *b1,
                         float eps1, const float *g2, const float *b2, float eps2, float *xout, const float *w, int ldw,
                         const float *bias, int relu, float *y, int ldy, void *stream);

long pn2x_posed_chamfer_partial_floats(int n, int m, int t);
int pn2x_posed_chamfer(int n, int m, int t, const float *a, const float *b, const float *ra, const float *ta, const float *rb,
                       const float *tb, float *partial, long partial_floats, float *out, void *stream);
int pn2x_obj_pose_metrics(int t, const float *gt_r, const float *gt_t, const float *pred_r, const float *pred_t, int axis,
                          int up_and_down_sym, float *out, void *stream);

int pn2x_hand_seq_metrics(int f, int s, int j, int mode, const float *pred_hf, const float *init_hf, const float *gt_kp,
                          const float *pred_kp, const float *rc, const float *tc, const float *scale, const float *palm,
                          const int *seq_off, const float *pose_r, const float *pose_t, const float *gt_r, const float *gt_t,
                          const float *theta, const float *theta_gt, float *rows, float *seq, void *stream);

int pn2x_hand_interaction_metrics(const pn2x_hand_pose_setup *model, int f, int s, int g, const float *global_r, const float *global_t,
                                  const float *theta, const float *obj_r, const float *obj_t, const float *pred_kp,
                                  const float *rest_joints, const float *rest_verts, const int *rest_of, const void *const *vols,
                                  const int *seq_off, float contact_threshold, float *rows, float *seq, float *out_verts,
                                  float *out_kp, void *stream);

struct pn2x_depth_frame {
    const void *depth;
    const unsigned char *seg;
    const float *intrinsics;
    const float *centre[2];
    float *clouds;
    int *counts;
    unsigned char *background;
    int *work;
    double depth_scale;
    int b, h, w, hs, ws, c, cap, depth_u16, flip_yz, reserved;
    int channel[2], value[2];
    float radius[2];
};
typedef struct pn2x_depth_frame pn2x_depth_frame;
int pn2x_depth_frame_supported(int h, int w, int hs, int ws, int c, int cap);
long pn2x_depth_frame_work_ints(int b, int h, int w);
int pn2x_depth_frame_clouds(const pn2x_depth_frame *frames, void *stream);

#define PN2X_CLOUD_NORMALS_MAX_B 65535
#define PN2X_CLOUD_NORMALS_MAX_N 2048
#define PN2X_CLOUD_NORMALS_MAX_K 64
void pn2x_cloud_normals_limits(int *max_b, int *max_n, int *max_k);
int pn2x_cloud_normals(int b, int n, int k, int orient, const float *points, const unsigned char *valid, const float *viewpoint,
                       float *normals, float *variation, void *stream);

#ifdef __cplusplus
}
#endif
#endif
```

network/models/fast_eval.py:

```python
from __future__ import annotations

import torch
import torch.nn.functional as F



def _lin_relu(x2d: torch.Tensor, W: torch.Tensor, b: torch.Tensor) -> torch.Tensor:
    from hotrack_amd import ext
    return ext.linear(x2d, W, b, relu=True)


def _lin(x2d: torch.Tensor, W: torch.Tensor, b: torch.Tensor = None) -> torch.Tensor:
    from hotrack_amd import ext
    return ext.linear(x2d, W, b)


class FastEval:
    MAX_POINTS = 16384
    fold_rearrange = True
    fold_r2 = True

    def __init__(self, net):
        self.net = net
        self._shapes_seen = set()
        self._key = None
        self.P = None
        self._consts = {}
        self._idents = {}
        self.row_chain = True
        self.sa_classes = True

    def _palm_idx(self, device):
        key = ("palm", str(device))
        if key not in self._consts:
            self._consts[key] = torch.tensor([0, 1, 5, 9, 13, 17], dtype=torch.int32, device=device)
        return self._consts[key]

    def _scale(self, device):
        key = ("scale", str(device))
        if key not in self._consts:
            self._consts[key] = 0.2 * torch.ones(1, dtype=torch.float32, device=device)
        return self._consts[key]

    def _versions(self):
        return tuple((t._version, t.data_ptr(), t.device) for t in list(self.net.parameters()) + list(self.net.buffers()))

    @staticmethod
    def supported(net) -> bool:
        from hotrack_amd import ext
        bh = net.bhand
        if net.handframe != "kp" or not net.elide_dead_attention:
            return False

        def scales_ok(mod, n_scales):
            if len(mod.conv_blocks) != n_scales or len(mod.nsample_list) != n_scales:
                return False
            for convs, K in zip(mod.conv_blocks, mod.nsample_list):
                if len(convs) != 3 or not ext.sa_mlp_max_supported(int(K), *(int(c.weight.shape[0]) for c in convs)):
                    return False
            return True

        if not (scales_ok(bh.sa1, 1) and scales_ok(bh.sa2, 1) and scales_ok(net.q1, 2) and scales_ok(net.q2, 2)):
            return False
        if getattr(bh.sa1, "knn", False) or getattr(bh.sa2, "knn", False) or not (net.q1.knn and net.q2.knn):
            return False
        if bh.in_dim != 0 or not bh.sa3.group_all:
            return False
        if list(net.q1.nsample_list) != list(net.q2.nsample_list):
            return False
        w = [tuple(int(c.weight.shape[0]) for c in convs) for mod in (net.q1, net.q2) for convs in mod.conv_blocks]
        return len(set(w)) == 1

    def prepare(self, force: bool = False):
        key = self._versions()
        if not force and self._key == key:
            return self.P
        with torch.no_grad():
            ts = [t for t in list(self.net.parameters()) + list(self.net.buffers()) if t.is_floating_point()]
            self.finite_weights = bool(torch.stack([torch.isfinite(t).all() for t in ts]).all().item()) if ts else True
        if not self.finite_weights:
            self.P, self._key = None, key
            return None
        from hotrack_amd import gemm_tuning
        from hotrack_amd.fused import fold_conv_bn as fold
        gemm_tuning.enable()
        net, bh = self.net, self.net.bhand
        P = {}

        def msg(mod, i):
            return [fold(c, n) for c, n in zip(mod.conv_blocks[i], mod.bn_blocks[i])]

        (W1, b1), l2, l3 = msg(bh.sa1, 0)
        P["sa1"] = dict(wx=W1.contiguous(), b1=b1, l2=l2, l3=l3)
        (W1, b1), l2, l3 = msg(bh.sa2, 0)
        D = W1.shape[1] - 3
        P["sa2"] = dict(w1f=W1[:, :D].contiguous(), wx=W1[:, D:].contiguous(), b1=b1, l2=l2, l3=l3)
        sa3 = [fold(c, n) for c, n in zip(bh.sa3.mlp_convs, bh.sa3.mlp_bns)]
        W = sa3[0][0]
        sa3[0] = (torch.cat([W[:, 3:], W[:, :3]], dim=1).contiguous(), sa3[0][1])
        P["sa3"] = sa3
        fp3 = [fold(c, n) for c, n in zip(bh.fp3.mlp_convs, bh.fp3.mlp_bns)]
        c_l2 = bh.sa2.out_channel
        P["fp3"] = dict(wa=fp3[0][0][:, :c_l2].contiguous(), wb=fp3[0][0][:, c_l2:].contiguous(), b=fp3[0][1], rest=fp3[1:])
        P["fp2"] = [fold(c, n) for c, n in zip(bh.fp2.mlp_convs, bh.fp2.mlp_bns)]
        fp1 = [fold(c, n) for c, n in zip(bh.fp1.mlp_convs, bh.fp1.mlp_bns)]
        W = fp1[0][0]
        fp1[0] = (torch.cat([W[:, 3:], W[:, :3]], dim=1).contiguous(), fp1[0][1])
        P["fp1"] = fp1
        import os
        from hotrack_amd import ext
        P["fp1_fused"] = None
        c_in = fp1[0][0].shape[1] - 3
        if os.environ.get("HOTRACK_MLP2", "1") != "0" and len(fp1) == 2 and c_in == P["fp2"][-1][0].shape[0] and ext.mlp2_rows_supported(c_in, fp1[0][0].shape[0], fp1[1][0].shape[0]):
            P["fp1_fused"] = dict(w2=fp1[0][0][:, :c_in].contiguous(), w2e=fp1[0][0][:, c_in:].contiguous(), b2=fp1[0][1],
                                  w3=fp1[1][0].contiguous(), b3=fp1[1][1])
        P["conv1"] = fold(bh.conv1, bh.bn1)
        C = bh.out_dim
        wq, q = [], {}
        for name, mod in (("q1", net.q1), ("q2", net.q2)):
            for i in range(2):
                (W1, b1), l2, l3 = msg(mod, i)
                wq.append(W1[:, :C])
                q[(name, i)] = dict(wx=W1[:, C:C + 3].contiguous(), b1=b1, l2=l2, l3=l3, K=mod.nsample_list[i],
                                    wc=W1[:, C + 3:] if W1.shape[1] > C + 3 else None)
        P["q"] = q
        Ks = [q[("q1", i)]["K"] for i in range(2)]
        i_s = Ks.index(min(Ks))
        P["wq_order"] = (i_s, 1 - i_s)
        P["wq"] = torch.cat([torch.cat([wq[i], wq[2 + i]], dim=0) for i in P["wq_order"]], dim=0)
        P["row_chain"] = None
        Wc = P["conv1"][0]
        if (len(fp1) == 2 and c_in == P["fp2"][-1][0].shape[0] and Ks[0] != Ks[1] and fp1[0][0].shape[1] == c_in + 3
                and ext.row_chain_supported(c_in, fp1[0][0].shape[0], Wc.shape[0], 4 * wq[0].shape[0])
                and fp1[1][0].shape == (c_in, c_in) and Wc.shape[1] == c_in and C == Wc.shape[0]):
            P["row_chain"] = dict(wa=ext.row_chain_pack(fp1[0][0]), ba=fp1[0][1].contiguous(),
                                  wb=ext.row_chain_pack(fp1[1][0]), bb=fp1[1][1].contiguous(),
                                  wc=ext.row_chain_pack(Wc), bc=P["conv1"][1].contiguous(), wq=ext.row_chain_pack(P["wq"]))
        P["mid_chain"] = None
        S2 = bh.sa2.npoint
        pf = P["fp3"]
        if (len(sa3) == 3 and len(pf["rest"]) == 1 and sa3[0][0].shape[1] == c_l2 + 3
                and ext.sa3_chain_supported(S2, c_l2, sa3[0][0].shape[0], sa3[1][0].shape[0], sa3[2][0].shape[0])
                and sa3[1][0].shape[1] == sa3[0][0].shape[0] and sa3[2][0].shape[1] == sa3[1][0].shape[0]
                and ext.fp3_chain_supported(S2, pf["wa"].shape[1], pf["wb"].shape[1], pf["wa"].shape[0], pf["rest"][0][0].shape[0])
                and pf["wb"].shape[1] == sa3[2][0].shape[0] and pf["rest"][0][0].shape[1] == pf["wa"].shape[0]):
            P["mid_chain"] = dict(sa3=[t for W, b in sa3 for t in (ext.row_chain_pack(W), b.contiguous())],
                                  wgt=pf["wb"].t().contiguous(), bg=pf["b"].contiguous(), wa=ext.row_chain_pack(pf["wa"]),
                                  wf=ext.row_chain_pack(pf["rest"][0][0]), bf=pf["rest"][0][1].contiguous())
        P["wc2"] = torch.cat([q[("q2", 0)]["wc"], q[("q2", 1)]["wc"]], dim=0).contiguous()
        P["head_w"] = net.final_mlp[2].weight.detach().squeeze(-1).contiguous()
        P["r1"] = (net.r1.linear.weight.detach().squeeze(-1), net.r1.linear.bias.detach(), net.r1._perm.t().contiguous())
        P["r2"] = (net.r2.linear.weight.detach().squeeze(-1), net.r2.linear.bias.detach(), net.r2._perm.t().contiguous())
        Wr1, br1, perm1 = P["r1"]
        Wr2, _, perm2 = P["r2"]
        re1, re2 = perm1.shape[1], perm2.shape[1]
        wc2 = P["wc2"].double()
        P["r1c"] = torch.cat([wc2 @ w for w in Wr1.double().chunk(re1, dim=1)], dim=0).float().contiguous()
        cb = (wc2 @ br1.double()).float()
        c1 = q[("q2", 0)]["b1"].shape[0]
        for i in range(2):
            q[("q2", i)]["b1r"] = (q[("q2", i)]["b1"] + cb[i * c1:(i + 1) * c1]).contiguous()
        P["r2s"] = torch.cat(Wr2.chunk(re2, dim=1), dim=0).contiguous()
        P["perm_host"] = (perm1.to("cpu", torch.int32).contiguous(), perm2.to("cpu", torch.int32).contiguous())
        self.P, self._key = P, key
        return P

    def _large_batch(self, B, N) -> bool:
        from hotrack_amd import ext
        return self.row_chain and B * N >= 32768 and B <= ext.ROW_CHAIN_MAX_B

    def _perm_idx(self, perm, B):
        key = ("perm", B, str(perm.device))
        if key not in self._idents:
            self._idents[key] = perm.reshape(1, -1).to(torch.int32).expand(B, -1).contiguous()
        return self._idents[key]

    @staticmethod
    def _q_scales(ext, name, plan, q, xyz1, c1q, a_col, cadd, out, c_q, b1="b1"):
        probs = []
        for i, (idx, a, nb_xyz) in enumerate(plan):
            p = q[(name, i)]
            probs.append(dict(idx=idx, w2=p["l2"][0], b2=p["l2"][1], w3=p["l3"][0], b3=p["l3"][1], a1f=a[:, :, a_col:a_col + c1q],
                              xyz=nb_xyz, cxyz=xyz1, wx=p["wx"], b1=p[b1],
                              cadd=None if cadd is None else cadd[:, :, i * c1q:(i + 1) * c1q], out=out[:, :, i * c_q:(i + 1) * c_q]))
        if len(probs) == 2:
            ext.sa_mlp_max_pair(*probs)
        else:
            for p in probs:
                ext.sa_mlp_max(p.pop("idx"), p.pop("w2"), p.pop("b2"), p.pop("w3"), p.pop("b3"), **p)

    def forward(self, input, flag_dict):
        from hotrack_amd import gemm_tuning
        shape = tuple(input["hand_points"].shape[:2])
        first = shape not in self._shapes_seen
        self._shapes_seen.add(shape)
        with gemm_tuning.scope(tune=first):
            return self._forward(input, flag_dict)

    def _forward(self, input, flag_dict):
        G = self._geometry(input, flag_dict)
        return None if G is None else self._dense(G, flag_dict)

    def _geometry(self, input, flag_dict):
        from hotrack_amd import ext
        net = self.net
        P = self.prepare()
        if P is None:
            return None
        dev = net.device
        if flag_dict["track_flag"]:
            palm = input["pred_palm_template"]
        else:
            palm = input["gt_hand_pose"]["palm_template"]
        palm = palm.to(dev).float()
        kp = input["jittered_hand_kp"].to(dev).float()
        pts = input["hand_points"].to(dev).float()
        B, N, _ = pts.shape
        J = kp.shape[1]
        f32 = dict(dtype=torch.float32, device=pts.device)

        if net.handframe != "kp":
            raise NotImplementedError("fast path covers handframe='kp' (HandTrackNet's configuration)")
        if kp.shape[1] != 21:
            raise NotImplementedError("fast path covers the 21-keypoint hand")
        palm_idx = self._palm_idx(pts.device)
        c_i = P["fp2"][-1][0].shape[0]
        fp1_in = torch.empty((B, N, c_i + 4), **f32)
        nonfinite = torch.empty(B, dtype=torch.int32, device=pts.device)
        R, t, xyz2, xyz1 = ext.hand_frame(palm.contiguous(), kp.contiguous(), palm_idx, pts.contiguous(), 0.2,
                                          xyz2_copy=fp1_in[:, :, c_i:c_i + 3], nonfinite=nonfinite)
        scale = self._scale(pts.device)
        canon = {"scale": scale, "rotation": R, "translation": t}
        tt = t.transpose(1, 2)

        bh = net.bhand
        p = P["sa1"]
        S1, K1 = bh.sa1.npoint, bh.sa1.nsample_list[0]
        qK = [P["q"][("q1", i)]["K"] for i in range(2)]
        knn_req = (xyz1, max(qK), min(qK) if min(qK) < max(qK) else 0)
        classes = self.sa_classes and self._large_batch(B, N) and all(
            ext.sa_mlp_max_classes_supported(int(m.nsample_list[0]), *(int(c.weight.shape[0]) for c in m.conv_blocks[0]))
            for m in (bh.sa1, bh.sa2))
        cnt1 = None
        if classes:
            _, l1_xyz, i_l2, idx1, cnt1, knn_lists = ext.fps_two_level(xyz2, S1, bh.sa2.npoint, query=(bh.sa1.radius_list[0], K1),
                                                                       knn=knn_req, query_counts=True)
        else:
            _, l1_xyz, i_l2, idx1, knn_lists = ext.fps_two_level(xyz2, S1, bh.sa2.npoint, query=(bh.sa1.radius_list[0], K1), knn=knn_req)
        return dict(cnt1=cnt1, P=P, pts=pts, B=B, N=N, J=J, c_i=c_i, fp1_in=fp1_in, nonfinite=nonfinite, R=R, t=t, xyz2=xyz2, xyz1=xyz1,
                    canon=canon, S1=S1, K1=K1, l1_xyz=l1_xyz, i_l2=i_l2, idx1=idx1, knn_lists=knn_lists)

    def _dense(self, G, flag_dict):
        from hotrack_amd import ext
        from hotrack_amd import pointnet2_utils as ops
        net, bh = self.net, self.net.bhand
        P, pts, B, N, J, c_i, fp1_in, nonfinite = G["P"], G["pts"], G["B"], G["N"], G["J"], G["c_i"], G["fp1_in"], G["nonfinite"]
        R, t, xyz2, xyz1, canon, S1, K1 = G["R"], G["t"], G["xyz2"], G["xyz1"], G["canon"], G["S1"], G["K1"]
        l1_xyz, i_l2, idx1, knn_lists = G["l1_xyz"], G["i_l2"], G["idx1"], G["knn_lists"]
        f32 = dict(dtype=torch.float32, device=pts.device)
        dev = net.device
        p = P["sa1"]
        c_l1 = p["l3"][0].shape[0]
        fp2_w = P["fp2"][0][0].shape[1]
        fp2_in = torch.empty((B, S1, fp2_w), **f32)
        l1_feat = fp2_in[:, :, :c_l1]
        cnt1 = G["cnt1"]
        p2 = P["sa2"]
        S2, K2 = bh.sa2.npoint, bh.sa2.nsample_list[0]
        c_l2 = p2["l3"][0].shape[0]
        sa3_in = torch.empty((B, S2, c_l2 + 4), **f32)
        if cnt1 is not None:
            idx2, l2_xyz, cnt2 = ext.ball_query_picks(bh.sa2.radius_list[0], K2, l1_xyz, i_l2, xyz_copy=sa3_in[:, :, c_l2:c_l2 + 3], counts=True)
            cls1, cls2 = ext.sa_class_lists_pair(cnt1, N, cnt2, S1)
            ext.sa_mlp_max_classes(idx1, cls1, *p["l2"], *p["l3"], xyz=xyz2, cxyz=l1_xyz, wx=p["wx"], b1=p["b1"], out=l1_feat)
        else:
            ext.sa_mlp_max(idx1, *p["l2"], *p["l3"], xyz=xyz2, cxyz=l1_xyz, wx=p["wx"], b1=p["b1"], out=l1_feat)
            idx2, l2_xyz = ext.ball_query_picks(bh.sa2.radius_list[0], K2, l1_xyz, i_l2, xyz_copy=sa3_in[:, :, c_l2:c_l2 + 3])

        p = p2
        a1f = _lin(l1_feat.reshape(B * S1, c_l1), p["w1f"]).view(B, S1, -1)
        l2_feat = sa3_in[:, :, :c_l2]
        if cnt1 is not None:
            ext.sa_mlp_max_classes(idx2, cls2, *p["l2"], *p["l3"], a1f=a1f, xyz=l1_xyz, cxyz=l2_xyz, wx=p["wx"], b1=p["b1"], out=l2_feat)
        else:
            ext.sa_mlp_max(idx2, *p["l2"], *p["l3"], a1f=a1f, xyz=l1_xyz, cxyz=l2_xyz, wx=p["wx"], b1=p["b1"], out=l2_feat)

        large = self._large_batch(B, N)
        mc = P["mid_chain"]
        if large and mc is not None:
            part = ext.sa3_chain(sa3_in, *mc["sa3"])
            l2_out = ext.fp3_chain(sa3_in, part, mc["wgt"], mc["bg"], mc["wa"], mc["wf"], mc["bf"])
        else:
            x = sa3_in.view(B * S2, c_l2 + 4)[:, :c_l2 + 3]
            for W, b in P["sa3"]:
                x = _lin_relu(x, W, b)
            l3 = ext.max_rows(x.view(B, S2, -1))

            p = P["fp3"]
            g = _lin(l3, p["wb"], p["b"])
            if B == 1:
                h = _lin_relu(sa3_in.view(S2, c_l2 + 4)[:, :c_l2], p["wa"], g.view(-1)).view(B, S2, -1)
            else:
                h = _lin(sa3_in.view(B * S2, c_l2 + 4)[:, :c_l2], p["wa"]).view(B, S2, -1)
                ext.bias_act_pm_(h, g, rows_per_bias=S2, relu=True)
            x = h.view(B * S2, -1)
            for W, b in p["rest"]:
                x = _lin_relu(x, W, b)
            l2_out = x.view(B, S2, -1)

        ext.three_nn_interpolate_pm(l1_xyz, l2_xyz, l2_out, fp2_in[:, :, c_l1:])
        x = fp2_in.view(B * S1, fp2_w)
        for W, b in P["fp2"]:
            x = _lin_relu(x, W, b)
        l1_out = x.view(B, S1, -1)

        assert c_i == l1_out.shape[2]
        q = P["q"]
        Ks = [q[("q1", i)]["K"] for i in range(2)]
        kmin, kmax = min(Ks), max(Ks)
        gi, gi_small = knn_lists
        c_q = q[("q1", 0)]["l3"][0].shape[0]
        c1q = q[("q1", 0)]["l2"][0].shape[1]
        rc = P["row_chain"]
        if large and rc is not None and gi_small is not None:
            lst, counts = ext.row_lists(gi, gi_small, N)
            ext.three_nn_interpolate_pm(xyz2, l1_xyz, l1_out, fp1_in[:, :, :c_i], rows=(lst, counts))
            a_all = torch.empty((B, N, 4 * c1q), **f32)
            ext.row_chain(fp1_in, lst, counts, rc["wa"], rc["ba"], rc["wb"], rc["bb"], rc["wc"], rc["bc"], rc["wq"], out=a_all)
        else:
            ext.three_nn_interpolate_pm(xyz2, l1_xyz, l1_out, fp1_in[:, :, :c_i])
            f = P["fp1_fused"]
            if f is not None:
                x = ext.mlp2_rows(fp1_in.view(B * N, c_i + 4), f["w2"], f["b2"], f["w3"], f["b3"], w2e=f["w2e"])
            else:
                x = fp1_in.view(B * N, c_i + 4)[:, :c_i + 3]
                for W, b in P["fp1"]:
                    x = _lin_relu(x, W, b)
            src2 = _lin_relu(x, *P["conv1"])
            a_all = _lin(src2, P["wq"]).view(B, N, -1)
        plan = []
        for i, K in enumerate(Ks):
            j = P["wq_order"].index(i)
            idx = gi if K == kmax else (gi_small if K == kmin and gi_small is not None else gi[:, :, :K].contiguous())
            plan.append((idx, a_all[:, :, 2 * c1q * j:2 * c1q * (j + 1)], xyz2))
        f11 = torch.empty((B, J, 2 * c_q), **f32)
        self._q_scales(ext, "q1", plan, q, xyz1, c1q, 0, None, f11, c_q)
        fold = self.fold_rearrange
        f13 = torch.empty((B, J, 2 * c_q), **f32)
        if fold:
            cadd = ext.perm_sum_rows(_lin(f11.view(B * J, -1), P["r1c"]), P["perm_host"][0], 2 * c1q)
            self._q_scales(ext, "q2", plan, q, xyz1, c1q, c1q, cadd, f13, c_q, b1="b1r")
        else:
            Wr, br, perm = P["r1"]
            f12 = _lin(ext.gather_rows(f11, self._perm_idx(perm, B)).view(B * J, -1), Wr, br)
            cadd = _lin(f12, P["wc2"]).view(B, J, -1)
            self._q_scales(ext, "q2", plan, q, xyz1, c1q, c1q, cadd, f13, c_q)
        Wr, br, perm = P["r2"]
        small = ext.ln_linear_supported(B * J, Wr.shape[0])
        fold2 = fold and self.fold_r2 and not small
        if fold2:
            z14 = _lin(f13.view(B * J, -1), P["r2s"])
        else:
            f14 = _lin(ext.gather_rows(f13, self._perm_idx(perm, B)).view(B * J, -1), Wr, br)

        s11, c11, c3 = net.transt.s11, net.transt.c11, net.c3
        wf, bf = net.final_mlp[0].weight.squeeze(-1), net.final_mlp[0].bias
        if small:
            x, hdn = ext.ln_linear(f14, s11.norm1, c11.linear1.weight, c11.linear1.bias, relu=True, ln2=c11.norm1)
            y = _lin(hdn, c11.linear2.weight)
            x, hdn = ext.ln_linear(x, c11.norm2, c3.linear1.weight, c3.linear1.bias, relu=True, y=y, ybias=c11.linear2.bias, ln2=c3.norm1)
            y = _lin(hdn, c3.linear2.weight)
            x, hdn = ext.ln_linear(x, c3.norm2, wf, bf, relu=True, y=y, ybias=c3.linear2.bias)
        else:
            if fold2:
                x = ext.add_layernorm_perm(z14, P["perm_host"][1], s11.norm1, bias=br, ln2=c11.norm1)
            else:
                x = ext.add_layernorm(f14, s11.norm1, ln2=c11.norm1)
            for blk, nxt in ((c11, c3.norm1), (c3, None)):
                hdn = _lin_relu(x, blk.linear1.weight, blk.linear1.bias)
                x = ext.add_layernorm(x, blk.norm2, y=_lin(hdn, blk.linear2.weight), bias=blk.linear2.bias, ln2=nxt)
            hdn = _lin_relu(x, wf, bf)
        pred_hf, pred_kp = ext.pose_head(hdn, P["head_w"], net.final_mlp[2].bias, xyz1, R, t, 0.2, nonfinite=nonfinite)

        ret = {"canon_pose": canon}
        ret["pred_kp_handframe"] = pred_hf.transpose(1, 2)
        ret["init_kp_handframe"] = xyz1.transpose(1, 2)
        ret["points_handframe"] = xyz2.transpose(1, 2)
        ret["pred_kp"] = pred_kp
        if flag_dict.get("IKNet_flag", False):
            d4, _ = ops.knn(4, ret["pred_kp"].contiguous(), pts.contiguous())
            d4 = d4.mean(dim=-1)
            d4[:, 0] -= 0.01
            d4[:, 1] -= 0.01
            ret["pred_kp_vis_mask"] = (d4 < 0.02).bool()
        return ret
```

Measured before the change: 101,200 frames/s.

## Fold fp1 first linear layer through three-NN interpolation into coarse level

Because interpolation is linear, the first fp1 layer's feature part is applied to the S1 coarse points before interpolation. The interpolate kernel then adds the xyz contribution and bias, applies ReLU, and writes h1 directly. A new row_chain3 kernel starts from h1 and skips the first matmul stage. This moves a per-point 132→128 GEMM onto S1 (fewer) points, at the cost of an extra small GEMM launch and an epilogue in the interpolation kernel.

```diff
diff --git a/hotrack_amd/csrc/capi.hip b/hotrack_amd/csrc/capi.hip
--- a/hotrack_amd/csrc/capi.hip
+++ b/hotrack_amd/csrc/capi.hip
@@ -20,6 +20,10 @@
 bool three_nn_interp_rows_supported(long b, long n, long m, long c, long ldp, long ldo);
 int three_nn_interp_rows_dispatch(int b, int n, int m, int c, const float *unknown, const float *known, const float *points, int ldp,
                                   float *out, int ldo, const int *row_list, const int *row_counts, hipStream_t st);
+bool three_nn_interp_rows_act_supported(long b, long n, long m, long c, long ldp, long ldo);
+int three_nn_interp_rows_act_dispatch(int b, int n, int m, int c, const float *unknown, const float *known, const float *points, int ldp,
+                                      float *out, int ldo, const int *row_list, const int *row_counts, const float *wx,
+                                      const float *bias, int relu, hipStream_t st);
 int fps_knn_dispatch(int b, int n, int m, const float *xyz, int *idx, float *radii, int nq, int k, int k2, const float *query,
                      int *kidx, int *kidx2, hipStream_t st);
 int ball_query_dispatch(int b, int n, int m, float radius, int nsample, const float *new_xyz, const float *xyz,
@@ -285,6 +289,22 @@
     return three_nn_interp_rows_dispatch(b, n, m, c, unknown, known, points, ldp, out, ldo, row_list, row_counts, (hipStream_t)stream);
 }
 
+int pn2x_three_nn_interpolate_pm_rows_act_supported(int b, int n, int m, int c, int ldp, int ldo) {
+    return three_nn_interp_rows_act_supported(b, n, m, c, ldp, ldo) ? 1 : 0;
+}
+
+int pn2x_three_nn_interpolate_pm_rows_act(int b, int n, int m, int c, const float *unknown, const float *known, const float *points,
+                                          int ldp, float *out, int ldo, const int *row_list, const int *row_counts, const float *wx,
+                                          const float *bias, int relu, void *stream) {
+    PN2_REQ(b >= 0 && n >= 0 && m >= 3 && c >= 1 && ldp >= c && ldo >= c, PN2_EINVAL);
+    if (b == 0 || n == 0) return PN2_OK;
+    PN2_REQ(unknown && known && points && out && wx && bias, PN2_ENULL);
+    PN2_REQ((row_list == nullptr) == (row_counts == nullptr), PN2_ENULL);
+    PN2_REQ(b <= 65535 && fits_int((long)n * 3) && fits_int((long)m * 3), PN2_ERANGE);
+    return three_nn_interp_rows_act_dispatch(b, n, m, c, unknown, known, points, ldp, out, ldo, row_list, row_counts, wx, bias, relu,
+                                             (hipStream_t)stream);
+}
+
 int pn2x_three_interpolate_pm(int b, int c, int m, int n, const float *points, int ldp, const int *idx,
                               const float *weight, float *out, int ldo, void *stream) {
     PN2_REQ(b >= 0 && c >= 0 && m >= 1 && n >= 0 && ldp >= c && ldo >= c, PN2_EINVAL);
diff --git a/hotrack_amd/csrc/nn_search.hip b/hotrack_amd/csrc/nn_search.hip
--- a/hotrack_amd/csrc/nn_search.hip
+++ b/hotrack_amd/csrc/nn_search.hip
@@ -116,17 +116,23 @@
     oi[0] = i1; oi[1] = i2; oi[2] = i3;
 }
 
-template <bool ROWS>
-__global__ void __launch_bounds__(256)
-three_nn_interp_kernel(int n, int m, int c4, const float *__restrict__ unknown_all, const float *__restrict__ known_all,
-                       const float *__restrict__ points_all, int ldp, float *__restrict__ out_all, int ldo,
-                       const int *__restrict__ row_list, const int *__restrict__ row_counts) {
+struct InterpEpilogue {
+    const float *wx, *bias;
+    int relu;
+};
+
+template <bool ROWS, bool EPI>
+__device__ __forceinline__ void
+three_nn_interp_body(int n, int m, int c4, const float *__restrict__ unknown_all, const float *__restrict__ known_all,
+                     const float *__restrict__ points_all, int ldp, float *__restrict__ out_all, int ldo,
+                     const int *__restrict__ row_list, const int *__restrict__ row_counts, const InterpEpilogue ep) {
     extern __shared__ __attribute__((aligned(16))) float4 sk[];
     __shared__ float sd[3][3][64];
     __shared__ int si[3][3][64];
     __shared__ float fw[3][64];
     __shared__ int fi[3][64];
     __shared__ int fq[ROWS ? 64 : 1];
+    __shared__ float fx[EPI ? 3 : 1][EPI ? 64 : 4];
     const int b = blockIdx.y;
     const float *__restrict__ known = known_all + (size_t)b * m * 3;
     const int ql = threadIdx.x & 63, c = threadIdx.x >> 6;
@@ -144,6 +150,17 @@
     for (int p = threadIdx.x; p < m; p += 256) {
         const float *src = known + (size_t)3 * p;
         sk[p] = make_float4(src[0], src[1], src[2], 0.f);
+    }
+    float4 *swx = sk + m, *sb = swx + 3 * c4;
+    if constexpr (EPI) {
+        for (int i = threadIdx.x; i < c4; i += 256) {
+            const float4 *w = reinterpret_cast<const float4 *>(ep.wx) + 3 * i;
+            const float4 v0 = w[0], v1 = w[1], v2 = w[2], bv = reinterpret_cast<const float4 *>(ep.bias)[i];
+            swx[i] = make_float4(v0.x, v0.w, v1.z, v2.y);
+            swx[c4 + i] = make_float4(v0.y, v1.x, v1.w, v2.z);
+            swx[2 * c4 + i] = make_float4(v0.z, v1.y, v2.x, v2.w);
+            sb[i] = bv;
+        }
     }
     __syncthreads();
     float b1 = __builtin_inff(), b2 = __builtin_inff(), b3 = __builtin_inff();
@@ -179,6 +196,7 @@
         fw[0][ql] = r1 / norm; fw[1][ql] = r2 / norm; fw[2][ql] = r3 / norm;
         fi[0][ql] = i1; fi[1][ql] = i2; fi[2][ql] = i3;
         if constexpr (ROWS) fq[ql] = q;
+        if constexpr (EPI) { fx[0][ql] = ux; fx[1][ql] = uy; fx[2][ql] = uz; }
     }
     __syncthreads();
     const int rows = min(64, nq - (int)blockIdx.x * 64);
@@ -195,12 +213,40 @@
         o.y = __builtin_fmaf(w2, a2.y, __builtin_fmaf(w0, a0.y, w1 * a1.y));
         o.z = __builtin_fmaf(w2, a2.z, __builtin_fmaf(w0, a0.z, w1 * a1.z));
         o.w = __builtin_fmaf(w2, a2.w, __builtin_fmaf(w0, a0.w, w1 * a1.w));
+        if constexpr (EPI) {
+            const float x = fx[0][r], y = fx[1][r], z = fx[2][r];
+            const float4 cx = swx[col], cy = swx[c4 + col], cz = swx[2 * c4 + col], bv = sb[col];
+            o.x = __builtin_fmaf(cz.x, z, __builtin_fmaf(cy.x, y, __builtin_fmaf(cx.x, x, o.x))) + bv.x;
+            o.y = __builtin_fmaf(cz.y, z, __builtin_fmaf(cy.y, y, __builtin_fmaf(cx.y, x, o.y))) + bv.y;
+            o.z = __builtin_fmaf(cz.z, z, __builtin_fmaf(cy.z, y, __builtin_fmaf(cx.z, x, o.z))) + bv.z;
+            o.w = __builtin_fmaf(cz.w, z, __builtin_fmaf(cy.w, y, __builtin_fmaf(cx.w, x, o.w))) + bv.w;
+            const bool act = ep.relu != 0;
+            o.x = act ? fmaxf(o.x, 0.f) : o.x; o.y = act ? fmaxf(o.y, 0.f) : o.y;
+            o.z = act ? fmaxf(o.z, 0.f) : o.z; o.w = act ? fmaxf(o.w, 0.f) : o.w;
+        }
         if constexpr (ROWS) {
             if (fq[r] >= 0) *reinterpret_cast<float4 *>(dst + (size_t)fq[r] * ldo + 4 * col) = o;
         } else {
             *reinterpret_cast<float4 *>(dst + (size_t)r * ldo + 4 * col) = o;
         }
     }
+}
+
+template <bool ROWS>
+__global__ void __launch_bounds__(256)
+three_nn_interp_kernel(int n, int m, int c4, const float *__restrict__ unknown_all, const float *__restrict__ known_all,
+                       const float *__restrict__ points_all, int ldp, float *__restrict__ out_all, int ldo,
+                       const int *__restrict__ row_list, const int *__restrict__ row_counts) {
+    three_nn_interp_body<ROWS, false>(n, m, c4, unknown_all, known_all, points_all, ldp, out_all, ldo, row_list, row_counts,
+                                      InterpEpilogue{nullptr, nullptr, 0});
+}
+
+template <bool ROWS>
+__global__ void __launch_bounds__(256)
+three_nn_interp_act_kernel(int n, int m, int c4, const float *__restrict__ unknown_all, const float *__restrict__ known_all,
+                           const float *__restrict__ points_all, int ldp, float *__restrict__ out_all, int ldo,
+                           const int *__restrict__ row_list, const int *__restrict__ row_counts, InterpEpilogue ep) {
+    three_nn_interp_body<ROWS, true>(n, m, c4, unknown_all, known_all, points_all, ldp, out_all, ldo, row_list, row_counts, ep);
 }
 
 bool three_nn_interp_supported(long b, long n, long m, long c, long ldp, long ldo) {
@@ -228,6 +274,28 @@
     dim3 grid((n + 63) / 64, b);
     hipLaunchKernelGGL(three_nn_interp_kernel<true>, grid, dim3(256), (size_t)m * sizeof(float4), st, n, m, c / 4, unknown, known, points,
                        ldp, out, ldo, row_list, row_counts);
+    return check_launch();
+}
+
+bool three_nn_interp_rows_act_supported(long b, long n, long m, long c, long ldp, long ldo) {
+    return three_nn_interp_rows_supported(b, n, m, c, ldp, ldo) && c <= 1024;
+}
+
+int three_nn_interp_rows_act_dispatch(int b, int n, int m, int c, const float *unknown, const float *known, const float *points, int ldp,
+                                      float *out, int ldo, const int *row_list, const int *row_counts, const float *wx,
+                                      const float *bias, int relu, hipStream_t st) {
+    if (b == 0 || n == 0) return PN2_OK;
+    if (!three_nn_interp_rows_act_supported(b, n, m, c, ldp, ldo)) return PN2_ERANGE;
+    if ((((uintptr_t)points | (uintptr_t)out | (uintptr_t)wx | (uintptr_t)bias) % 16) != 0) return PN2_ERANGE;
+    dim3 grid((n + 63) / 64, b);
+    const size_t lds = ((size_t)m + (size_t)c) * sizeof(float4);
+    const InterpEpilogue ep{wx, bias, relu ? 1 : 0};
+    if (row_list)
+        hipLaunchKernelGGL(three_nn_interp_act_kernel<true>, grid, dim3(256), lds, st, n, m, c / 4, unknown, known, points, ldp, out, ldo,
+                           row_list, row_counts, ep);
+    else
+        hipLaunchKernelGGL(three_nn_interp_act_kernel<false>, grid, dim3(256), lds, st, n, m, c / 4, unknown, known, points, ldp, out, ldo,
+                           nullptr, nullptr, ep);
     return check_launch();
 }
 
diff --git a/hotrack_amd/csrc/row_chain.hip b/hotrack_amd/csrc/row_chain.hip
--- a/hotrack_amd/csrc/row_chain.hip
+++ b/hotrack_amd/csrc/row_chain.hip
@@ -48,24 +48,31 @@
     return lo * A.N + A.list[(size_t)lo * A.N + off + (e - P[lo])];
 }
 
-template <int MT>
+template <int MT, bool H1IN>
 __device__ void tile(const ChainArgs &A, const Smem &S, int seq, int e0, int cnt) {
     const int tid = (int)threadIdx.x, lane = tid & 63, w = tid >> 6;
     constexpr int R = MT * 16;
     if (tid < R) S.rows[tid] = tid < cnt ? lookup(A, S, seq, e0 + tid) : -1;
     __syncthreads();
-    for (int i = tid; i < R * (KX / 4); i += 256) {
-        const int r = i / (KX / 4), q = i - r * (KX / 4);
-        const int g = S.rows[r];
-        f32x4 v = {0.f, 0.f, 0.f, 0.f};
-        if (g >= 0 && q < XQ) {
-            v = *reinterpret_cast<const f32x4 *>(A.x + (size_t)g * A.ldx + 4 * q);
-            if (q == XQ - 1) v.w = 0.f;
-        }
-        *reinterpret_cast<f32x4 *>(S.r1 + r * LDX + 4 * q) = v;
-    }
-    __syncthreads();
-    {
+    if constexpr (H1IN) {
+        for (int i = tid; i < R * (CH / 4); i += 256) {
+            const int r = i / (CH / 4), q = i - r * (CH / 4);
+            const int g = S.rows[r];
+            const f32x4 v = *reinterpret_cast<const f32x4 *>(A.x + (size_t)(g < 0 ? 0 : g) * A.ldx + 4 * q);
+            *reinterpret_cast<f32x4 *>(S.r2 + r * LDH + 4 * q) = g < 0 ? (f32x4){0.f, 0.f, 0.f, 0.f} : v;
+        }
+    } else {
+        for (int i = tid; i < R * (KX / 4); i += 256) {
+            const int r = i / (KX / 4), q = i - r * (KX / 4);
+            const int g = S.rows[r];
+            f32x4 v = {0.f, 0.f, 0.f, 0.f};
+            if (g >= 0 && q < XQ) {
+                v = *reinterpret_cast<const f32x4 *>(A.x + (size_t)g * A.ldx + 4 * q);
+                if (q == XQ - 1) v.w = 0.f;
+            }
+            *reinterpret_cast<f32x4 *>(S.r1 + r * LDX + 4 * q) = v;
+        }
+        __syncthreads();
         f32x4 acc[2][MT];
         init_bias(acc, A.ba, 2 * w, lane);
         mm<2, MT, KX / 16, LDX>(acc, A.wa + (size_t)(2 * w) * (KX / 16) * 256, S.r1, lane);
@@ -110,19 +117,21 @@
     __syncthreads();
 }
 
+template <bool H1IN>
 __device__ void run_rows(const ChainArgs &A, const Smem &S, int seq, int e_lo, int e_hi) {
     for (int e0 = e_lo; e0 < e_hi; e0 += 64) {
         const int cnt = e_hi - e0 < 64 ? e_hi - e0 : 64;
         switch ((cnt + 15) >> 4) {
-            case 1: tile<1>(A, S, seq, e0, cnt); break;
-            case 2: tile<2>(A, S, seq, e0, cnt); break;
-            case 3: tile<3>(A, S, seq, e0, cnt); break;
-            default: tile<4>(A, S, seq, e0, cnt); break;
-        }
-    }
-}
-
-__global__ __launch_bounds__(256, 1) void row_chain_kernel(ChainArgs A) {
+            case 1: tile<1, H1IN>(A, S, seq, e0, cnt); break;
+            case 2: tile<2, H1IN>(A, S, seq, e0, cnt); break;
+            case 3: tile<3, H1IN>(A, S, seq, e0, cnt); break;
+            default: tile<4, H1IN>(A, S, seq, e0, cnt); break;
+        }
+    }
+}
+
+template <bool H1IN>
+__device__ __forceinline__ void chain(const ChainArgs &A) {
     extern __shared__ __attribute__((aligned(16))) float smem[];
     const int tid = (int)threadIdx.x;
     Smem S;
@@ -164,9 +173,13 @@
     long l0 = first_at(lo - cs_end, GROUP_COST_LARGE), l1 = first_at(hi - cs_end, GROUP_COST_LARGE);
     l0 = l0 < g_large ? l0 : g_large; l1 = l1 < g_large ? l1 : g_large;
     auto clip = [](long e, int n) { return (int)(e < n ? e : n); };
-    run_rows(A, S, 0, clip(16 * s0, n_small), clip(16 * s1, n_small));
-    run_rows(A, S, 1, clip(16 * l0, n_large), clip(16 * l1, n_large));
-}
+    run_rows<H1IN>(A, S, 0, clip(16 * s0, n_small), clip(16 * s1, n_small));
+    run_rows<H1IN>(A, S, 1, clip(16 * l0, n_large), clip(16 * l1, n_large));
+}
+
+__global__ __launch_bounds__(256, 1) void row_chain_kernel(ChainArgs A) { chain<false>(A); }
+
+__global__ __launch_bounds__(256, 1) void row_chain3_kernel(ChainArgs A) { chain<true>(A); }
 
 constexpr int RL_MAXN = 16384;
 
@@ -241,15 +254,16 @@
     return (c_in == 128 && c_h == 128 && c_conv == 384 && c_q == 512) ? 1 : 0;
 }
 
-extern "C" int pn2x_row_chain(int b, int n, const float *x, int ldx, const int *list, const int *counts, const float *wa,
-                              const float *ba, const float *wb, const float *bb, const float *wc, const float *bc, const float *wq,
-                              float *out, int ldo, int grid, void *stream) {
+static int launch_chain(void (*kernel)(pn2::rchain::ChainArgs), pn2::PerDeviceOnce &raised, bool h1in, int b, int n, const float *x,
+                        int ldx, const int *list, const int *counts, const float *wa, const float *ba, const float *wb,
+                        const float *bb, const float *wc, const float *bc, const float *wq, float *out, int ldo, int grid,
+                        void *stream) {
     using namespace pn2;
     using namespace pn2::rchain;
-    if (b < 0 || n < 1 || ldx < 132 || ldo < CQ || ldx % 4 || ldo % 4 || grid < 0) return PN2_EINVAL;
+    if (b < 0 || n < 1 || ldx < (h1in ? CH : 132) || ldo < CQ || ldx % 4 || ldo % 4 || grid < 0) return PN2_EINVAL;
     if (b > MAXB || (long)b * n >= (1L << 31) / 2) return PN2_ERANGE;
     if (b == 0) return PN2_OK;
-    if (!x || !list || !counts || !wa || !ba || !wb || !bb || !wc || !bc || !wq || !out) return PN2_ENULL;
+    if (!x || !list || !counts || (!h1in && (!wa || !ba)) || !wb || !bb || !wc || !bc || !wq || !out) return PN2_ENULL;
     if (((uintptr_t)x | (uintptr_t)out | (uintptr_t)wa | (uintptr_t)ba | (uintptr_t)wb | (uintptr_t)bb | (uintptr_t)wc |
          (uintptr_t)bc | (uintptr_t)wq) % 16 != 0)
         return PN2_EINVAL;
@@ -258,11 +272,30 @@
     a.wa = wa; a.ba = ba; a.wb = wb; a.bb = bb; a.wc = wc; a.bc = bc; a.wq = wq; a.out = out;
     const size_t lds = lds_bytes(b);
     static_assert(lds_bytes(MAXB) <= 160 * 1024, "row_chain's LDS at MAXB clouds exceeds a compute unit's 160 KB");
-    static PerDeviceOnce raised;
     if (raised.first_use())
-        (void)hipFuncSetAttribute((const void *)row_chain_kernel, hipFuncAttributeMaxDynamicSharedMemorySize, (int)lds_bytes(MAXB));
+        (void)hipFuncSetAttribute((const void *)kernel, hipFuncAttributeMaxDynamicSharedMemorySize, (int)lds_bytes(MAXB));
     const int cus = num_compute_units();
     if (grid == 0 || grid > cus) grid = cus;
-    hipLaunchKernelGGL(row_chain_kernel, dim3(grid), dim3(256), lds, (hipStream_t)stream, a);
+    hipLaunchKernelGGL(kernel, dim3(grid), dim3(256), lds, (hipStream_t)stream, a);
     return check_launch();
 }
+
+extern "C" int pn2x_row_chain(int b, int n, const float *x, int ldx, const int *list, const int *counts, const float *wa,
+                              const float *ba, const float *wb, const float *bb, const float *wc, const float *bc, const float *wq,
+                              float *out, int ldo, int grid, void *stream) {
+    static pn2::PerDeviceOnce raised;
+    return launch_chain(pn2::rchain::row_chain_kernel, raised, false, b, n, x, ldx, list, counts, wa, ba, wb, bb, wc, bc, wq, out, ldo,
+                        grid, stream);
+}
+
+extern "C" int pn2x_row_chain3_supported(int c_h, int c_conv, int c_q) {
+    return (c_h == 128 && c_conv == 384 && c_q == 512) ? 1 : 0;
+}
+
+extern "C" int pn2x_row_chain3(int b, int n, const float *h1, int ldh, const int *list, const int *counts, const float *wb,
+                               const float *bb, const float *wc, const float *bc, const float *wq, float *out, int ldo, int grid,
+                               void *stream) {
+    static pn2::PerDeviceOnce raised;
+    return launch_chain(pn2::rchain::row_chain3_kernel, raised, true, b, n, h1, ldh, list, counts, nullptr, nullptr, wb, bb,
+                        wc, bc, wq, out, ldo, grid, stream);
+}
diff --git a/hotrack_amd/ext.py b/hotrack_amd/ext.py
--- a/hotrack_amd/ext.py
+++ b/hotrack_amd/ext.py
@@ -307,9 +307,16 @@
 _lib.pn2x_three_nn_interpolate_pm_rows.restype = _ci
 _lib.pn2x_three_nn_interpolate_pm_rows_supported.argtypes = [_ci] * 6
 _lib.pn2x_three_nn_interpolate_pm_rows_supported.restype = _ci
-
-
-def three_nn_interpolate_pm(unknown: torch.Tensor, known: torch.Tensor, points: torch.Tensor, out: torch.Tensor, rows=None) -> torch.Tensor:
+_lib.pn2x_three_nn_interpolate_pm_rows_act.argtypes = [_ci, _ci, _ci, _ci, _vp, _vp, _vp, _ci, _vp, _ci, _vp, _vp, _vp, _vp, _ci, _vp]
+_lib.pn2x_three_nn_interpolate_pm_rows_act.restype = _ci
+_lib.pn2x_three_nn_interpolate_pm_rows_act_supported.argtypes = [_ci] * 6
+_lib.pn2x_three_nn_interpolate_pm_rows_act_supported.restype = _ci
+
+
+def three_nn_interpolate_pm(unknown: torch.Tensor, known: torch.Tensor, points: torch.Tensor, out: torch.Tensor, rows=None,
+                            wx: torch.Tensor = None, bias: torch.Tensor = None, relu: bool = False) -> torch.Tensor:
+    if (wx is None) != (bias is None) or (wx is None and relu):
+        raise ValueError("three_nn_interpolate_pm: wx, bias (and relu) come together")
     if rows is not None:
         if not (isinstance(rows, (tuple, list)) and len(rows) == 2 and all(isinstance(t, torch.Tensor) for t in rows)):
             raise TypeError("three_nn_interpolate_pm: rows must be the (list, counts) pair of row_lists")
@@ -322,12 +329,26 @@
     pp, ldp = _rows(points, "points", C)
     po, ldo = _rows(out, "out", C)
     f32 = torch.float32
-    if rows is not None:
+    if rows is not None or wx is not None:
         if not (_lib.pn2x_three_nn_interpolate_pm_rows_supported(B, n, m, C, ldp, ldo) and pp % 16 == 0 and po % 16 == 0):
-            raise ValueError("three_nn_interpolate_pm: rows needs 3 <= m <= 2048 known points, C and the row strides multiples of 4 "
-                             "and 16-byte aligned points / out")
-        if rows[0].device != points.device or rows[1].device != points.device:
+            raise ValueError("three_nn_interpolate_pm: rows / wx need 3 <= m <= 2048 known points, C and the row strides multiples "
+                             "of 4 and 16-byte aligned points / out")
+        if rows is not None and (rows[0].device != points.device or rows[1].device != points.device):
             raise ValueError("three_nn_interpolate_pm: rows on another device than points")
+        if wx is not None:
+            if not _lib.pn2x_three_nn_interpolate_pm_rows_act_supported(B, n, m, C, ldp, ldo):
+                raise ValueError("three_nn_interpolate_pm: the wx / bias epilogue covers C <= 1024")
+            pw, pb = _native._ptr(wx, "wx", f32, C * 3), _native._ptr(bias, "bias", f32, C)
+            if tuple(wx.shape) != (C, 3) or tuple(bias.shape) != (C,) or pw % 16 or pb % 16:
+                raise ValueError("three_nn_interpolate_pm: wx must be (C,3) and bias (C,), both 16-byte aligned")
+            pl = None if rows is None else _native._ptr(rows[0], "rows list", torch.int32, B * n)
+            pc = None if rows is None else _native._ptr(rows[1], "rows counts", torch.int32, B * 2)
+            with torch.cuda.device(points.device):
+                _native._check(_native._call(_lib.pn2x_three_nn_interpolate_pm_rows_act, "three_nn_interp_act_kernel", None, B, n, m, C,
+                                             _native._ptr(unknown, "unknown", f32, B * n * 3), _native._ptr(known, "known", f32, B * m * 3),
+                                             pp, ldp, po, ldo, pl, pc, pw, pb, 1 if relu else 0, _native._stream(points)),
+                               "three_nn_interpolate_pm")
+            return out
         with torch.cuda.device(points.device):
             _native._check(_native._call(_lib.pn2x_three_nn_interpolate_pm_rows, "three_nn_interp_kernel", None, B, n, m, C,
                                          _native._ptr(unknown, "unknown", f32, B * n * 3), _native._ptr(known, "known", f32, B * m * 3),
@@ -797,6 +818,10 @@
 _lib.pn2x_row_chain_supported.restype = _ci
 _lib.pn2x_row_chain.argtypes = [_ci, _ci, _vp, _ci, _vp, _vp] + [_vp] * 7 + [_vp, _ci, _ci, _vp]
 _lib.pn2x_row_chain.restype = _ci
+_lib.pn2x_row_chain3_supported.argtypes = [_ci] * 3
+_lib.pn2x_row_chain3_supported.restype = _ci
+_lib.pn2x_row_chain3.argtypes = [_ci, _ci, _vp, _ci, _vp, _vp] + [_vp] * 5 + [_vp, _ci, _ci, _vp]
+_lib.pn2x_row_chain3.restype = _ci
 ROW_CHAIN_MAX_B = 1024
 
 
@@ -835,6 +860,10 @@
               grid: int = 0) -> torch.Tensor:
     if x.dim() != 3 or not x.is_cuda or x.dtype != torch.float32 or x.stride(2) != 1 or x.stride(0) != x.shape[1] * x.stride(1):
         raise TypeError("row_chain: x must be a (B,N,C) float32 GPU tensor with contiguous rows")
+    if (wa is None) != (ba is None):
+        raise ValueError("row_chain: wa and ba come together")
+    if wa is None and x.shape[2] < 128:
+        raise ValueError("row_chain: without wa / ba the rows of x hold h1, 128 floats")
     B, N, _ = x.shape
     f32 = torch.float32
     if out is None:
@@ -843,6 +872,14 @@
         raise ValueError("row_chain: out must be (B,N,>=512) float32 with contiguous rows")
     if lst.shape != (B, N) or counts.shape != (B, 2) or lst.dtype != torch.int32 or counts.dtype != torch.int32:
         raise ValueError("row_chain: list (B,N) / counts (B,2) int32 from row_lists")
+    if wa is None:
+        with torch.cuda.device(x.device):
+            _native._check(_native._call(_lib.pn2x_row_chain3, "row_chain3_kernel", None, B, N, x.data_ptr(), x.stride(1), lst.data_ptr(),
+                                         counts.data_ptr(), _native._ptr(wb, "wb", f32, 128 * 128), _native._ptr(bb, "bb", f32, 128),
+                                         _native._ptr(wc, "wc", f32, 384 * 128), _native._ptr(bc, "bc", f32, 384),
+                                         _native._ptr(wq, "wq", f32, 512 * 384), out.data_ptr(), out.stride(1), int(grid),
+                                         _native._stream(x)), "row_chain")
+        return out
     with torch.cuda.device(x.device):
         _native._check(_native._call(_lib.pn2x_row_chain, "row_chain_kernel", None, B, N, x.data_ptr(), x.stride(1), lst.data_ptr(),
                                      counts.data_ptr(), _native._ptr(wa, "wa", f32, 128 * 144), _native._ptr(ba, "ba", f32, 128),
@@ -851,6 +888,15 @@
                                      _native._ptr(wq, "wq", f32, 512 * 384), out.data_ptr(), out.stride(1), int(grid),
                                      _native._stream(x)), "row_chain")
     return out
+
+
+def row_chain3_supported(c_h: int, c_conv: int, c_q: int) -> bool:
+    return bool(_lib.pn2x_row_chain3_supported(c_h, c_conv, c_q))
+
+
+def row_chain3(h1: torch.Tensor, lst: torch.Tensor, counts: torch.Tensor, wb, bb, wc, bc, wq, out: torch.Tensor = None,
+               grid: int = 0) -> torch.Tensor:
+    return row_chain(h1, lst, counts, None, None, wb, bb, wc, bc, wq, out=out, grid=grid)
 
 
 _lib.pn2x_sa3_chain_supported.argtypes = [_ci] * 5
diff --git a/include/pn2_ext.h b/include/pn2_ext.h
--- a/include/pn2_ext.h
+++ b/include/pn2_ext.h
@@ -45,6 +45,10 @@
 int pn2x_three_nn_interpolate_pm_rows_supported(int b, int n, int m, int c, int ldp, int ldo);
 int pn2x_three_nn_interpolate_pm_rows(int b, int n, int m, int c, const float *unknown, const float *known, const float *points,
                                       int ldp, float *out, int ldo, const int *row_list, const int *row_counts, void *stream);
+int pn2x_three_nn_interpolate_pm_rows_act_supported(int b, int n, int m, int c, int ldp, int ldo);
+int pn2x_three_nn_interpolate_pm_rows_act(int b, int n, int m, int c, const float *unknown, const float *known, const float *points,
+                                          int ldp, float *out, int ldo, const int *row_list, const int *row_counts, const float *wx,
+                                          const float *bias, int relu, void *stream);
 
 int pn2x_furthest_point_sampling_radii(int b, int n, int m, const float *xyz, int *idx, float *radii, void *stream);
 int pn2x_fps_radii_knn_supported(int n, int nq, int k);
@@ -120,6 +124,9 @@
 int pn2x_row_chain(int b, int n, const float *x, int ldx, const int *list, const int *counts, const float *wa, const float *ba,
                    const float *wb, const float *bb, const float *wc, const float *bc, const float *wq, float *out, int ldo,
                    int grid, void *stream);
+int pn2x_row_chain3_supported(int c_h, int c_conv, int c_q);
+int pn2x_row_chain3(int b, int n, const float *h1, int ldh, const int *list, const int *counts, const float *wb, const float *bb,
+                    const float *wc, const float *bc, const float *wq, float *out, int ldo, int grid, void *stream);
 
 int pn2x_sa3_chain_supported(int s, int c_in, int c1, int c2, int c3);
 int pn2x_sa3_chain(int b, int s, const float *x, int ldx, const float *w1, const float *b1, const float *w2, const float *b2,
diff --git a/network/models/fast_eval.py b/network/models/fast_eval.py
--- a/network/models/fast_eval.py
+++ b/network/models/fast_eval.py
@@ -19,6 +19,7 @@
     MAX_POINTS = 16384
     fold_rearrange = True
     fold_r2 = True
+    fold_interp = True
 
     def __init__(self, net):
         self.net = net
@@ -136,6 +137,10 @@
             P["row_chain"] = dict(wa=ext.row_chain_pack(fp1[0][0]), ba=fp1[0][1].contiguous(),
                                   wb=ext.row_chain_pack(fp1[1][0]), bb=fp1[1][1].contiguous(),
                                   wc=ext.row_chain_pack(Wc), bc=P["conv1"][1].contiguous(), wq=ext.row_chain_pack(P["wq"]))
+        P["fold_interp"] = None
+        if P["row_chain"] is not None and ext.row_chain3_supported(fp1[0][0].shape[0], Wc.shape[0], 4 * wq[0].shape[0]):
+            P["fold_interp"] = dict(wa_f=fp1[0][0][:, :c_in].contiguous(), wa_x=fp1[0][0][:, c_in:].contiguous(),
+                                    ba=P["row_chain"]["ba"])
         P["mid_chain"] = None
         S2 = bh.sa2.npoint
         pf = P["fp3"]
@@ -225,10 +230,11 @@
             raise NotImplementedError("fast path covers the 21-keypoint hand")
         palm_idx = self._palm_idx(pts.device)
         c_i = P["fp2"][-1][0].shape[0]
-        fp1_in = torch.empty((B, N, c_i + 4), **f32)
+        folded = self.fold_interp and self._large_batch(B, N) and P["fold_interp"] is not None
+        fp1_in = torch.empty((B, N, P["fold_interp"]["wa_f"].shape[0] if folded else c_i + 4), **f32)
         nonfinite = torch.empty(B, dtype=torch.int32, device=pts.device)
         R, t, xyz2, xyz1 = ext.hand_frame(palm.contiguous(), kp.contiguous(), palm_idx, pts.contiguous(), 0.2,
-                                          xyz2_copy=fp1_in[:, :, c_i:c_i + 3], nonfinite=nonfinite)
+                                          xyz2_copy=None if folded else fp1_in[:, :, c_i:c_i + 3], nonfinite=nonfinite)
         scale = self._scale(pts.device)
         canon = {"scale": scale, "rotation": R, "translation": t}
         tt = t.transpose(1, 2)
@@ -247,7 +253,7 @@
                                                                        knn=knn_req, query_counts=True)
         else:
             _, l1_xyz, i_l2, idx1, knn_lists = ext.fps_two_level(xyz2, S1, bh.sa2.npoint, query=(bh.sa1.radius_list[0], K1), knn=knn_req)
-        return dict(cnt1=cnt1, P=P, pts=pts, B=B, N=N, J=J, c_i=c_i, fp1_in=fp1_in, nonfinite=nonfinite, R=R, t=t, xyz2=xyz2, xyz1=xyz1,
+        return dict(folded=folded, cnt1=cnt1, P=P, pts=pts, B=B, N=N, J=J, c_i=c_i, fp1_in=fp1_in, nonfinite=nonfinite, R=R, t=t, xyz2=xyz2, xyz1=xyz1,
                     canon=canon, S1=S1, K1=K1, l1_xyz=l1_xyz, i_l2=i_l2, idx1=idx1, knn_lists=knn_lists)
 
     def _dense(self, G, flag_dict):
@@ -324,10 +330,17 @@
         rc = P["row_chain"]
         if large and rc is not None and gi_small is not None:
             lst, counts = ext.row_lists(gi, gi_small, N)
-            ext.three_nn_interpolate_pm(xyz2, l1_xyz, l1_out, fp1_in[:, :, :c_i], rows=(lst, counts))
             a_all = torch.empty((B, N, 4 * c1q), **f32)
-            ext.row_chain(fp1_in, lst, counts, rc["wa"], rc["ba"], rc["wb"], rc["bb"], rc["wc"], rc["bc"], rc["wq"], out=a_all)
-        else:
+            if G["folded"]:
+                fi = P["fold_interp"]
+                p1 = _lin(l1_out.view(B * S1, c_i), fi["wa_f"]).view(B, S1, -1)
+                ext.three_nn_interpolate_pm(xyz2, l1_xyz, p1, fp1_in, rows=(lst, counts), wx=fi["wa_x"], bias=fi["ba"], relu=True)
+                ext.row_chain3(fp1_in, lst, counts, rc["wb"], rc["bb"], rc["wc"], rc["bc"], rc["wq"], out=a_all)
+            else:
+                ext.three_nn_interpolate_pm(xyz2, l1_xyz, l1_out, fp1_in[:, :, :c_i], rows=(lst, counts))
+                ext.row_chain(fp1_in, lst, counts, rc["wa"], rc["ba"], rc["wb"], rc["bb"], rc["wc"], rc["bc"], rc["wq"], out=a_all)
+        else:
+            assert not G["folded"]
             ext.three_nn_interpolate_pm(xyz2, l1_xyz, l1_out, fp1_in[:, :, :c_i])
             f = P["fp1_fused"]
             if f is not None:
```

After: 103,000 frames/s, median of 6. +1.8%, better.
